# aluo-x/3D_SLN

Hardware: AMD Instinct MI355X
Metric: scene-graph VAE steps/sec + 256² diff-render fps, 1/2/4/8 MI355X (higher is better)
Workload: dtype f32; 1 GPU; BASELINE configs[1]: batch=64 scene graphs x (32 objects, 64 triples) per GPU, Sg2ScVAE train step at train.py defaults (embedding_dim=64, 5+5 GraphTripleConv, BatchNorm); O=2048, T=4096, hipgraph=True, distinct_batches_cycled=4, eps=N(0,1) drawn on the device inside the step, parallelism=dp1

## Files before the change

### 3d_sln_amd/_lib.py

```python
from __future__ import annotations

import ctypes as C
import os

HERE = os.path.dirname(os.path.abspath(__file__))
LIB_PATH = os.path.join(HERE, "libsln_hip.so")

SLN_E = {-1: "SLN_E_BADARG", -2: "SLN_E_UNSUPPORTED", -3: "SLN_E_STATE", -4: "SLN_E_NOGPU", -5: "SLN_E_NOMEM", -6: "SLN_E_CAPTURE"}

c_f32p = C.c_void_p
c_i64p = C.c_void_p


class SlnError(RuntimeError):
    pass


class SlnVaeConfig(C.Structure):
    _fields_ = [(n, C.c_int) for n in (
        "embedding_dim", "gconv_num_layers", "recurrent", "batch_norm", "decoder_cat", "use_ae",
        "box_dim", "n_angle", "num_objs", "num_preds", "num_attrs", "no_attr")]


class SlnVaeUnit(C.Structure):
# ... 143 lines not shown


class SlnDraw3D(C.Structure):
    _fields_ = [(n, C.c_void_p) for n in ("faces_xyz", "face_index", "depth", "face_label", "chosen", "K", "light_cam", "albedo")] + \
               [(n, C.c_int32) for n in ("R", "V", "F", "S", "k", "shadows")] + \
               [(n, C.c_float) for n in ("ambient", "intensity", "min_dist", "bias")] + [("background", C.c_float * 3)]


SIGNATURES = {
    "sln_version": (C.c_int, []),
    "sln_build_arch": (C.c_char_p, []),
    "sln_device_ok": (C.c_int, []),
    "sln_vae_num_units": (C.c_int, [C.POINTER(SlnVaeConfig)]),
    "sln_vae_create": (C.c_int, [C.POINTER(SlnVaeConfig), C.POINTER(C.c_void_p)]),
    "sln_vae_destroy": (None, [C.c_void_p]),
    "sln_vae_workspace_bytes": (C.c_int64, [C.c_void_p, C.c_int, C.c_int]),
    "sln_vae_bind": (C.c_int, [C.c_void_p, C.POINTER(SlnVaeTensors), C.c_void_p, C.c_int64, C.c_int, C.c_int]),
    "sln_vae_set_batch": (C.c_int, [C.c_void_p, C.POINTER(SlnVaeBatch), C.c_void_p]),
    "sln_vae_check_batch": (C.c_int, [C.c_void_p, C.c_void_p]),
    "sln_vae_encoder": (C.c_int, [C.c_void_p, c_f32p, c_f32p, C.c_int, C.c_void_p]),
    "sln_vae_decoder": (C.c_int, [C.c_void_p, c_f32p, c_f32p, c_f32p, C.c_int, C.c_void_p]),
    "sln_vae_forward": (C.c_int, [C.c_void_p, c_f32p, c_f32p, c_f32p, c_f32p, c_f32p, c_f32p, C.c_int, C.c_void_p]),
    "sln_vae_loss": (C.c_int, [C.c_void_p, c_f32p, c_f32p, c_f32p, c_f32p, C.c_float, c_f32p, C.c_int, C.c_void_p]),
    "sln_vae_decoder_backward": (C.c_int, [C.c_void_p, c_f32p, c_f32p, c_f32p, C.c_void_p]),
    "sln_vae_encoder_backward": (C.c_int, [C.c_void_p, c_f32p, c_f32p, C.c_void_p]),
    "sln_vae_backward": (C.c_int, [C.c_void_p, C.c_void_p]),
    "sln_vae_params_changed": (C.c_int, [C.c_void_p]),
    "sln_vae_zero_grad": (C.c_int, [C.c_void_p, C.c_void_p]),
    "sln_vae_adam_step": (C.c_int, [C.c_void_p, C.c_float, C.c_void_p]),
    "sln_vae_adam_reset": (C.c_int, [C.c_void_p, C.c_int64, C.c_void_p]),
    "sln_vae_adam_get_step": (C.c_int, [C.c_void_p, C.POINTER(C.c_int64), C.c_void_p]),
    "sln_vae_set_grad_guard": (C.c_int, [C.c_void_p, c_f32p]),
    "sln_vae_seed": (C.c_int, [C.c_void_p, C.c_uint64, C.c_uint64, C.c_void_p]),
    "sln_vae_last_eps": (C.c_int, [C.c_void_p, c_f32p, C.c_void_p]),
    "sln_vae_randn": (C.c_int, [C.c_void_p, c_f32p, C.c_int64, C.c_void_p]),
    "sln_layout_heatmap": (C.c_int, [c_f32p, C.c_int64, C.c_int, C.c_int, C.c_int, C.c_int, c_f32p, C.c_void_p]),
    "sln_vae_set_training": (C.c_int, [C.c_void_p, C.c_int]),
    "sln_vae_set_gemm_precision": (C.c_int, [C.c_void_p, C.c_int]),
    "sln_vae_train_step": (C.c_int, [C.c_void_p, c_f32p, C.c_float, C.c_float, c_f32p, C.c_int, C.c_int, C.c_void_p]),
    "sln_vae_group_create": (C.c_int, [C.POINTER(C.c_void_p), C.c_int, C.POINTER(SlnVaeGroupIO), C.POINTER(C.c_void_p)]),
    "sln_vae_group_decoder": (C.c_int, [C.c_void_p, C.c_void_p]),
    "sln_vae_group_decoder_backward": (C.c_int, [C.c_void_p, C.c_void_p]),
    "sln_vae_group_launches": (C.c_int, [C.c_void_p, C.POINTER(C.c_int), C.POINTER(C.c_int), C.POINTER(C.c_int)]),
    "sln_vae_group_transposes": (C.c_int64, [C.c_void_p]),
    "sln_vae_group_fused_params": (C.c_int, [C.c_void_p, C.POINTER(C.c_void_p), C.POINTER(C.c_int64), C.c_int]),
    "sln_vae_group_destroy": (None, [C.c_void_p]),
    "sln_debug_side_stream": (C.c_int, [C.c_void_p, C.POINTER(C.c_int), C.POINTER(C.c_int)]),
    "sln_side_stream_prepare": (C.c_int, [C.c_void_p]),
    "sln_side_stream_forget": (C.c_int, [C.c_void_p]),
    "sln_prof_enable": (C.c_int, [C.c_int]),
    "sln_set_deterministic": (C.c_int, [C.c_int]),
    "sln_get_deterministic": (C.c_int, []),
    "sln_debug_tn_plan": (C.c_int, [C.c_void_p, C.c_void_p, C.c_void_p, C.c_int, C.c_void_p, C.c_void_p, C.c_int]),
    "sln_prof_read": (C.c_int, [C.c_void_p, C.c_void_p, C.c_void_p, C.c_int]),
    "sln_vae_tap": (C.c_int64, [C.c_void_p, C.c_int, C.c_int, c_f32p, C.c_void_p]),
    "sln_gconv_workspace_bytes": (C.c_int64, [C.c_int, C.c_int, C.c_int, C.c_int, C.c_int, C.c_int]),
    "sln_gconv_forward": (C.c_int, [C.c_int, C.c_int, C.c_int, C.c_int, C.c_int, C.c_int, C.POINTER(SlnVaeUnit), c_f32p, c_f32p,
                                    C.c_void_p, C.c_int, C.c_int, C.c_int, C.c_void_p, C.c_int64, c_f32p, c_f32p, C.c_void_p]),
    "sln_gconv_net_create": (C.c_int, [C.c_int, C.c_int, C.c_int, C.c_int, C.c_int, C.c_int, C.POINTER(C.c_void_p)]),
    "sln_gconv_net_set_edges": (C.c_int, [C.c_void_p, C.c_void_p, C.c_int, C.c_int, C.c_void_p]),
    "sln_gconv_net_forward": (C.c_int, [C.c_void_p, c_f32p, c_f32p, c_f32p, c_f32p, C.c_int, C.c_void_p]),
    "sln_gconv_net_backward": (C.c_int, [C.c_void_p, c_f32p, c_f32p, c_f32p, c_f32p, C.c_void_p]),
    "sln_linear_forward": (C.c_int, [c_f32p, C.c_int, C.c_int, c_f32p, c_f32p, c_f32p, C.c_int, C.c_void_p,
                                     C.c_int, C.c_void_p]),
    "sln_linear_wgrad": (C.c_int, [c_f32p, c_f32p, C.c_int, C.c_int, C.c_int, c_f32p, c_f32p, C.c_void_p]),
    "sln_debug_gemm_nt": (C.c_int, [C.POINTER(SlnDbgGemmNT), C.c_int, C.POINTER(C.c_int), C.c_void_p]),
    "sln_debug_gemm_tn": (C.c_int, [C.POINTER(SlnDbgGemmTN), C.c_int, C.c_int, C.c_void_p]),
    "sln_debug_gemm_nt_route": (C.c_int, [C.POINTER(SlnDbgGemmNT), C.POINTER(SlnDbgNTRoute)]),
    "sln_debug_gemm_nt_half": (C.c_int, [C.POINTER(SlnDbgGemmNT), C.c_int, C.c_void_p]),
    "sln_debug_gemm_nt_half_takes": (C.c_int, [C.POINTER(SlnDbgGemmNT)]),
    "sln_debug_gemm_sizes": (C.c_int, [C.POINTER(C.c_int), C.c_int]),
    "sln_debug_vae_csr": (C.c_int, [c_i64p, C.c_int, C.c_int, C.c_int, C.POINTER(SlnDbgCsr), C.c_void_p, C.c_void_p]),
    "sln_debug_vae_edge": (C.c_int, [C.POINTER(SlnDbgEdge), C.c_int, C.c_int, C.POINTER(C.c_int), C.c_void_p]),
    "sln_debug_vae_loss": (C.c_int, [C.POINTER(SlnDbgLoss), C.c_void_p]),
    "sln_debug_vae_tables": (C.c_int, [C.c_int, C.c_void_p, C.c_int, C.c_int, C.c_float, C.c_int, C.c_int, C.c_int, C.c_void_p]),
    "sln_debug_vae_embed": (C.c_int, [C.POINTER(SlnDbgEmbed), C.c_int, C.c_int, C.POINTER(C.c_int), C.c_void_p]),
    "sln_debug_vae_opt": (C.c_int, [C.POINTER(SlnDbgOpt), C.c_void_p]),
    "sln_debug_vae_sizes": (C.c_int, [C.POINTER(C.c_int), C.c_int]),
    "sln_debug_vae_leaf_launches": (C.c_int64, [C.c_void_p]),
    "sln_debug_vae_half_launches": (C.c_int64, [C.c_void_p]),
    "sln_project_faces": (C.c_int, [c_f32p, C.c_void_p, c_f32p, c_f32p, c_f32p, C.c_int, C.c_int, C.c_int, C.c_float, C.c_float, c_f32p, C.c_void_p]),
    "sln_project_faces_backward": (C.c_int, [c_f32p, C.c_void_p, c_f32p, c_f32p, c_f32p, C.c_int, C.c_int, C.c_int, C.c_float, C.c_float, c_f32p,
                                             c_f32p, C.c_void_p]),
    "sln_raster_workspace_bytes": (C.c_int64, [C.c_int, C.c_int]),
    "sln_raster_forward": (C.c_int, [c_f32p, C.c_int, C.c_int, C.c_int, C.c_float, C.c_float, C.c_void_p, C.c_void_p,
                                     c_f32p, c_f32p, C.c_void_p]),
    "sln_raster_forward_dual": (C.c_int, [c_f32p, C.c_int, C.c_int, C.c_int, C.c_float, C.c_float, C.c_float, C.c_void_p,
                                          C.c_void_p, c_f32p, c_f32p, C.c_void_p, c_f32p, c_f32p, C.c_void_p]),
    "sln_raster_texture_sample": (C.c_int, [c_f32p, c_f32p, C.c_void_p, c_f32p, c_f32p, C.c_int, C.c_int, C.c_int, C.c_int,
                                            C.c_float, c_f32p, C.c_void_p]),
    "sln_raster_backward_depth": (C.c_int, [c_f32p, C.c_void_p, c_f32p, c_f32p, c_f32p, C.c_int, C.c_int, C.c_int, c_f32p,
                                            C.c_void_p]),
    "sln_raster_backward_rgb": (C.c_int, [c_f32p, C.c_void_p, c_f32p, c_f32p, C.c_int, C.c_int, C.c_int, C.c_int, C.c_float,
                                          c_f32p, C.c_void_p]),
    "sln_raster_texture_sample_chw": (C.c_int, [c_f32p, c_f32p, C.c_void_p, c_f32p, c_f32p, C.c_int, C.c_int, C.c_int, C.c_int, C.c_int,
                                                C.c_float, C.c_float, c_f32p, C.c_void_p]),
    "sln_raster_backward_rgb_multi": (C.c_int, [c_f32p, C.c_void_p, C.c_void_p, C.c_void_p, C.c_int, C.c_int, C.c_int, C.c_int, C.c_float,
                                                C.c_void_p, c_f32p, C.c_void_p]),
    "sln_scene_workspace_bytes": (C.c_int64, [C.c_int, C.c_int, C.c_int]),
    "sln_scene_forward": (C.c_int, [c_f32p, C.c_void_p, C.c_int, C.c_int, C.c_int, C.c_int, C.c_void_p, C.c_void_p,
                                    C.c_float, C.c_float, C.c_float, C.c_float, C.c_void_p, c_f32p, C.c_void_p]),
    "sln_scene_forward_live": (C.c_int, [c_f32p, C.c_void_p, C.c_int, C.c_int, C.c_int, C.c_int, C.c_void_p, C.c_void_p,
                                         C.c_float, C.c_float, C.c_float, C.c_float, C.c_void_p, c_f32p, C.c_void_p, C.c_void_p, C.c_void_p]),
    "sln_spade_prepare": (C.c_int, [C.c_void_p]),
    "sln_spade_release": (C.c_int, [C.c_void_p, C.c_int]),
    "sln_spade_conv": (C.c_int, [c_f32p, C.c_int, C.c_int, C.c_int, C.c_int, c_f32p, c_f32p, C.c_int, C.c_int, C.c_int, C.c_int,
                                 C.c_float, c_f32p, C.c_void_p]),
    "sln_spade_modulate": (C.c_int, [c_f32p, C.c_int, C.c_int, C.c_int, C.c_int, c_f32p, c_f32p, C.c_int, C.c_int, c_f32p, c_f32p,
                                     C.c_int, C.c_float, c_f32p, C.c_void_p]),
    "sln_layernorm_stats": (C.c_int, [c_f32p, C.c_int, C.c_int64, C.c_float, C.c_void_p, c_f32p, C.c_void_p]),
    "sln_spade_apply": (C.c_int, [c_f32p, c_f32p, C.c_int, C.c_int, C.c_int, C.c_int, C.c_int, c_f32p, C.c_int, C.c_float, c_f32p, C.c_void_p]),
    "sln_spade_apply_up": (C.c_int, [c_f32p, C.c_int, c_f32p, C.c_int, C.c_int, C.c_int, C.c_int, C.c_int, c_f32p, C.c_int, C.c_float, c_f32p,
                                     C.c_void_p]),
    "sln_resize": (C.c_int, [c_f32p, C.c_int, C.c_int, C.c_int, C.c_int, C.c_int, C.c_int, c_f32p, C.c_void_p]),
    "sln_spade_depth_concat": (C.c_int, [c_f32p, C.c_int, C.c_int, C.c_int, C.c_int, c_f32p, c_f32p, C.c_int, c_f32p, C.c_int, C.c_void_p]),
    "sln_se_scale_add": (C.c_int, [c_f32p, c_f32p, C.c_int, C.c_int, C.c_int64, c_f32p, c_f32p, c_f32p, c_f32p, C.c_void_p]),
    "sln_spade_conv_sums": (C.c_int, [c_f32p, C.c_int, C.c_int, C.c_int, C.c_int, c_f32p, c_f32p, C.c_int, C.c_int, C.c_int, C.c_int,
                                      C.c_float, c_f32p, C.c_void_p, C.c_void_p, C.c_void_p]),
    "sln_spade_modulate_up": (C.c_int, [c_f32p, C.c_int, C.c_int, C.c_int, C.c_int, c_f32p, c_f32p, C.c_int, C.c_int, c_f32p, C.c_int,
                                        c_f32p, C.c_int, C.c_float, c_f32p, C.c_void_p]),
    "sln_layernorm_finalize": (C.c_int, [C.c_void_p, C.c_int, C.c_int64, C.c_int, C.c_float, c_f32p, C.c_void_p]),
    "sln_spade_conv_f16": (C.c_int, [c_f32p, C.c_int, C.c_int, C.c_int, C.c_int, C.c_void_p, C.c_void_p, c_f32p, C.c_int, C.c_int, C.c_int,
                                     C.c_int, C.c_float, c_f32p, C.c_void_p]),
    "sln_spade_conv_sums_f16": (C.c_int, [c_f32p, C.c_int, C.c_int, C.c_int, C.c_int, C.c_void_p, C.c_void_p, c_f32p, C.c_int, C.c_int,
                                          C.c_int, C.c_int, C.c_float, c_f32p, C.c_void_p, C.c_void_p, C.c_void_p]),
    "sln_spade_modulate_f16": (C.c_int, [c_f32p, C.c_int, C.c_int, C.c_int, C.c_int, C.c_void_p, C.c_void_p, c_f32p, C.c_int, C.c_int,
                                         c_f32p, c_f32p, C.c_int, C.c_float, c_f32p, C.c_void_p]),
    "sln_spade_modulate_up_f16": (C.c_int, [c_f32p, C.c_int, C.c_int, C.c_int, C.c_int, C.c_void_p, C.c_void_p, c_f32p, C.c_int, C.c_int,
                                            c_f32p, C.c_int, c_f32p, C.c_int, C.c_float, c_f32p, C.c_void_p]),
    "sln_block_tail": (C.c_int, [c_f32p, C.c_int, c_f32p, C.c_int, C.c_int, C.c_int, C.c_int, C.c_void_p, c_f32p, c_f32p, c_f32p,
                                 C.c_int, c_f32p, C.c_void_p, C.c_int, C.c_float, c_f32p, C.c_void_p]),
    "sln_upsample2x": (C.c_int, [c_f32p, C.c_int, C.c_int, C.c_int, C.c_int, c_f32p, C.c_void_p]),
    "sln_conv_img_tanh": (C.c_int, [c_f32p, C.c_int, C.c_int, C.c_int, C.c_int, c_f32p, c_f32p, C.c_int, c_f32p, C.c_void_p]),
# ... 120 lines not shown
```

### 3d_sln_amd/csrc/gemm_bodies.h

```cpp
#pragma once
#include "sln_common.h"
#include "sln_gemm.h"
#include "sln_prof.h"

#include <cstdlib>
#include <cstring>
#include <type_traits>
namespace {


#ifndef SLN_TRACE
#define SLN_TRACE(i)
#endif
#ifndef SLN_TRACEH
#define SLN_TRACEH(i)
#endif

#ifndef SLN_NT_SCHED
#define SLN_NT_SCHED 1
#endif
#ifndef SLN_TN_SCHED
#define SLN_TN_SCHED 1
#endif
#ifndef SLN_TN_ABL
// ... 1267 lines not shown
      for (int r = 0; r < 16; ++r) dst[r * 64] = tn_acc_read(acc[1][r]);
    } else {
#pragma unroll
      for (int r = 0; r < 16; ++r) dst[r * 64] = tn_acc_read(acc[0][r]);
    }
  }
  __syncthreads();
  {
    const float* src = red + ((wave ^ 2) * 16) * 64 + lane;
    const float sc = a.sgd_step != nullptr ? -a.sgd_step[0] : 1.f;
    const int k = k0 + 32 * wc + lrow;
    float* dcol = a.dW + min(k, a.Kin - 1);
    const bool kv = k < a.Kin;
    if (wr == 0) {
#pragma unroll
      for (int r = 0; r < 16; ++r) {
        const float v = (tn_acc_read(acc[0][r]) + src[r * 64]) * sc;
        const int n = n0 + 2 * ((r & 3) + 8 * (r >> 2) + 4 * lk);
        if (kv && n < a.Nout) sln_gatomic_add(dcol + (size_t)n * a.lddw, v);
      }
    } else {
#pragma unroll
      for (int r = 0; r < 16; ++r) {
        const float v = (src[r * 64] + tn_acc_read(acc[1][r])) * sc;
        const int n = n0 + 2 * ((r & 3) + 8 * (r >> 2) + 4 * lk) + 1;
        if (kv && n < a.Nout) sln_gatomic_add(dcol + (size_t)n * a.lddw, v);
      }
    }
  }

  if (a.db != nullptr && (bx % tiles_k) == 0) {
#pragma unroll
    for (int off = TPRA; off < 64; off <<= 1) {
      dbacc.x += __shfl_xor(dbacc.x, off, 64); dbacc.y += __shfl_xor(dbacc.y, off, 64);
      dbacc.z += __shfl_xor(dbacc.z, off, 64); dbacc.w += __shfl_xor(dbacc.w, off, 64);
    }
    __syncthreads();
    float4* dbs = reinterpret_cast<float4*>(red);
    if (lane < TPRA) dbs[wave * TPRA + lane] = dbacc;
    __syncthreads();
    if (tid < TPRA) {
      const float4 p0 = dbs[tid], p1 = dbs[TPRA + tid], p2 = dbs[2 * TPRA + tid], p3 = dbs[3 * TPRA + tid];
      const int n = n0 + 4 * tid;
      const float sb = a.sgd_step != nullptr ? -a.sgd_step[0] : 1.f;
      if (n + 0 < a.Nout) sln_gatomic_add(a.db + n + 0, (((p0.x + p1.x) + p2.x) + p3.x) * sb);
      if (n + 1 < a.Nout) sln_gatomic_add(a.db + n + 1, (((p0.y + p1.y) + p2.y) + p3.y) * sb);
      if (n + 2 < a.Nout) sln_gatomic_add(a.db + n + 2, (((p0.z + p1.z) + p2.z) + p3.z) * sb);
      if (n + 3 < a.Nout) sln_gatomic_add(a.db + n + 3, (((p0.w + p1.w) + p2.w) + p3.w) * sb);
    }
  }
}


inline bool tn_gathers(const GemmTNArgs& a) {
  bool g = false;
  for (int s = 0; s < a.X.nseg; ++s) g |= a.X.seg[s].which != 0;
  return g;
}

inline bool tn_supported(const GemmTNArgs& a) {
  for (int s = 0; s < a.G.nseg; ++s) if (a.G.seg[s].which != 0) return false;
  return true;
}

inline size_t nt_smem_bytes(int K, int BM, int BN, int WM) {
  const int kpad = (K + 31) & ~31;
  return (size_t)sln_crows(kpad + 4) * 16 + (size_t)2 * (BM + BN) * (BK + 4) * 4 + (size_t)BN * 16 + (size_t)WM * BN * 16;
}

inline size_t tn_smem_bytes(int BM, int BN) { return (size_t)(BM + BN) * 16 + (size_t)2 * BK * (BM + TN_PAD + BN + TN_PAD) * 4; }

inline int nt_heuristic_tile(const GemmNTArgs& a) {
  static const int forced = std::getenv("SLN_NT_TILE") ? std::atoi(std::getenv("SLN_NT_TILE")) : -1;
  (void)a;
  return forced >= 0 ? forced : 0;
}

inline bool nt_big_shape(const GemmNTArgs& a) {
  return (long)sln_cdiv(a.M, 128) * sln_cdiv(a.N, 64) >= 384;
}

inline bool nt_unaligned(const GemmNTArgs& a) {
  for (int s = 0; s + 1 < a.A.nseg; ++s) if (a.A.seg[s].len % BK) return true;
  return false;
}

inline int nt_amode(const GemmNTArgs& a) {
  bool x2 = false;
  for (int s = 0; s < a.A.nseg; ++s) x2 |= a.A.seg[s].x2 != nullptr;
  bool ident = !x2;
  for (int s = 0; s < a.A.nseg; ++s) ident = ident && a.A.seg[s].coef == SLN_COEF_IDENT;
  return x2 ? 1 : (ident ? 2 : 0);
}

inline bool tn_prepare(GemmTNArgs& a) {
  bool x2 = false;
  for (int s = 0; s < a.G.nseg; ++s) x2 |= a.G.seg[s].x2 != nullptr;
  if (a.rows_per_block <= 0) {
    static const int target = std::getenv("SLN_TN_TARGET") ? std::atoi(std::getenv("SLN_TN_TARGET")) : 768;
    static const int minrows = std::getenv("SLN_TN_MINROWS") ? std::atoi(std::getenv("SLN_TN_MINROWS")) : 256;
    const int tiles = sln_cdiv(a.Nout, 64) * sln_cdiv(a.Kin, 64);
    int chunks = sln_cdiv(target, tiles);
    int rpb = sln_cdiv(sln_cdiv(a.R, chunks), BK) * BK;
    a.rows_per_block = rpb < minrows ? minrows : rpb;
  }
  return x2;
// ... 4 lines not shown
```

### 3d_sln_amd/csrc/gemm_f32.hip

```cpp
#include <cstdio>
#include <cstdlib>
#include <algorithm>
#include <vector>
#include "gemm_bodies.h"
#include "vae_multi.h"
namespace {
constexpr bool nt_coef_helpers(int amode, int epi) { return amode != 2 || epi == EPI_MASK; }
template <int BM, int BN, int AMODE, int EPI>
constexpr bool nt_helpers() { return BM == 64 && BN == 64 && nt_coef_helpers(AMODE, EPI); }
template <int BM, int BN, int WM, int WN, int AMODE, int EPI, int MULTI>
__global__ __launch_bounds__((nt_helpers<BM, BN, AMODE, EPI>() ? 512 : 256)) void gemm_nt_kernel(const GemmNTArgs a) {
  extern __shared__ __attribute__((aligned(16))) char smem[];
  gemm_nt_body<BM, BN, WM, WN, AMODE, EPI, MULTI, nt_helpers<BM, BN, AMODE, EPI>()>(a, blockIdx.x, ((a.M + BM - 1) / BM) * ((a.N + BN - 1) / BN), smem);
}

template <int AMODE, int EPI>
constexpr bool nt_helpers2() { return nt_coef_helpers(AMODE, EPI); }
template <int J, int AMODE, int EPI>
__global__ __launch_bounds__((nt_helpers2<AMODE, EPI>() ? 512 : 256)) void gemm_nt16_kernel(const GemmNTArgs a) {
  extern __shared__ __attribute__((aligned(16))) char smem[];
  gemm_nt_body16<J, AMODE, EPI, nt_helpers2<AMODE, EPI>()>(a, blockIdx.x, ((a.M + 63) / 64) * ((a.N + 32 * J - 1) / (32 * J)), smem);
}

template <int AMODE, int EPI, int NSEG = 1>
// ... 67 lines not shown
  SLN_CHECK_LAUNCH();
  return 0;
}

template <int AMODE, int EPI>
int launch_nt_route(const GemmNTArgs& a, const NtRoute& rt, hipStream_t st) {
  switch (rt.body) {
    case NT_BODY_SMALL: return launch_nt_small<AMODE, EPI>(a, rt, st);
    case NT_BODY_SMALL3: return launch_nt_small<AMODE, EPI, 3>(a, rt, st);
    case NT_BODY_16J3: return launch_nt16<3, AMODE, EPI>(a, rt, st);
    case NT_BODY_16J5: return launch_nt16<5, AMODE, EPI>(a, rt, st);
    case NT_BODY_128x64: return launch_nt<128, 64, 2, 2, AMODE, EPI>(a, rt, st);
    case NT_BODY_128: return launch_nt<128, 128, 2, 2, AMODE, EPI>(a, rt, st);
    case NT_BODY_64: return launch_nt<64, 64, 2, 2, AMODE, EPI>(a, rt, st);
    default: return -1;
  }
}

NtRoute nt_route(const GemmNTArgs& a, int epi, int tile) {
  static const bool no_small = std::getenv("SLN_NO_SMALL_NT") != nullptr;
  NtRoute r;
  r.amode = nt_amode(a); r.multi = 0;
  if (tile < 0 && !no_small && nt_wants_small(a)) r.body = NT_BODY_SMALL;
  else if (tile < 0 && !no_small && nt_wants_small3(a)) { r.body = NT_BODY_SMALL3; r.multi = 1; }
  else {
    const int J16 = tile < 0 ? nt16_pick(a) : 0;
    if (J16 == 3) r.body = NT_BODY_16J3;
    else if (J16 == 5) r.body = NT_BODY_16J5;
    else {
      if (tile < 0) tile = nt_heuristic_tile(a);
      const bool unaligned = a.A.nseg > 1 && nt_unaligned(a);
      if (unaligned) tile = 0;
      r.body = tile == 1 ? NT_BODY_128x64 : (tile == 2 ? NT_BODY_128 : NT_BODY_64);
      r.multi = a.A.nseg > 1 ? (unaligned ? 2 : 1) : 0;
    }
  }
  const bool big = r.body == NT_BODY_128x64 || r.body == NT_BODY_128;
  r.threads = !big && nt_coef_helpers(r.amode, epi) ? 512 : 256;
  return r;
}

template <int BM, int BN, int WM, int WN, bool G_X2, bool XG>
__global__ __launch_bounds__(256) void gemm_tn_kernel(const GemmTNArgs a) {
  extern __shared__ __attribute__((aligned(16))) char smem[];
  gemm_tn_body<BM, BN, WM, WN, G_X2, XG>(a, blockIdx.x, blockIdx.y, smem);
}

template <bool G_X2, bool XG>
__global__ __launch_bounds__(256) void gemm_tn_multi_kernel(const GemmTNArgs* __restrict__ probs, const TnMultiMeta* __restrict__ meta) {
  extern __shared__ __attribute__((aligned(16))) char smem[];
  const TnMultiItem it = meta->item[blockIdx.x];
  if (it.prob < 0) return;
  gemm_tn_body<64, 64, 2, 2, G_X2, XG>(probs[it.prob], it.tile, it.chunk, smem);
}

template <int BM, int BN, int WM, int WN, bool G_X2>
int launch_tn(const GemmTNArgs& a, hipStream_t st) {
  const size_t smem = tn_smem_bytes(BM, BN);
  const int gx = sln_cdiv(a.Nout, BM) * sln_cdiv(a.Kin, BN);
  const int gy = sln_cdiv(a.R, a.rows_per_block);
  if (gx <= 0 || gy <= 0) return 0;
  if (!tn_supported(a)) return -1;
  if (tn_gathers(a)) hipLaunchKernelGGL((gemm_tn_kernel<BM, BN, WM, WN, G_X2, true>), dim3(gx, gy), dim3(256), smem, st, a);
  else hipLaunchKernelGGL((gemm_tn_kernel<BM, BN, WM, WN, G_X2, false>), dim3(gx, gy), dim3(256), smem, st, a);
  SLN_CHECK_LAUNCH();
  return 0;
}

}

template <int BM, int BN, int WM, int WN>
static int init_nt_tile() {
  hipError_t e = hipSuccess;
#define SLN_SET(X2, EPI)                                                                                          \
  if (e == hipSuccess)                                                                                            \
    e = hipFuncSetAttribute(reinterpret_cast<const void*>(&gemm_nt_kernel<BM, BN, WM, WN, X2, EPI, 0>),           \
                            hipFuncAttributeMaxDynamicSharedMemorySize, 160 * 1024);                              \
  if (e == hipSuccess)                                                                                            \
    e = hipFuncSetAttribute(reinterpret_cast<const void*>(&gemm_nt_kernel<BM, BN, WM, WN, X2, EPI, 1>),           \
                            hipFuncAttributeMaxDynamicSharedMemorySize, 160 * 1024);                              \
  if (e == hipSuccess && BM == 64 && BN == 64)                                                                    \
    e = hipFuncSetAttribute(reinterpret_cast<const void*>(&gemm_nt_kernel<64, 64, WM, WN, X2, EPI, 2>),           \
                            hipFuncAttributeMaxDynamicSharedMemorySize, 160 * 1024);
  SLN_SET(0, EPI_PLAIN) SLN_SET(0, EPI_STATS) SLN_SET(0, EPI_MASK)
  SLN_SET(1, EPI_PLAIN) SLN_SET(1, EPI_STATS) SLN_SET(1, EPI_MASK)
  SLN_SET(2, EPI_PLAIN) SLN_SET(2, EPI_STATS) SLN_SET(2, EPI_MASK)
#undef SLN_SET
  return (int)e;
}

int sln_gemm_group_init();
int sln_gemm_init() {
  static bool done = false;
  if (done) return 0;
  int r = init_nt_tile<64, 64, 2, 2>();
#define SLN_SET_S(AM, EPI)                                                                                        \
  if (!r) r = (int)hipFuncSetAttribute(reinterpret_cast<const void*>(&gemm_nt_small_kernel<AM, EPI, 1>),         \
                                       hipFuncAttributeMaxDynamicSharedMemorySize, 160 * 1024);                  \
  if (!r) r = (int)hipFuncSetAttribute(reinterpret_cast<const void*>(&gemm_nt_small_kernel<AM, EPI, 3>),         \
                                       hipFuncAttributeMaxDynamicSharedMemorySize, 160 * 1024);
  SLN_SET_S(0, EPI_PLAIN) SLN_SET_S(0, EPI_STATS) SLN_SET_S(0, EPI_MASK) SLN_SET_S(1, EPI_PLAIN) SLN_SET_S(1, EPI_STATS)
  SLN_SET_S(1, EPI_MASK) SLN_SET_S(2, EPI_PLAIN) SLN_SET_S(2, EPI_STATS) SLN_SET_S(2, EPI_MASK)
#undef SLN_SET_S
#define SLN_SET_16(J, AM, EPI)                                                                                    \
  if (!r) r = (int)hipFuncSetAttribute(reinterpret_cast<const void*>(&gemm_nt16_kernel<J, AM, EPI>),             \
                                       hipFuncAttributeMaxDynamicSharedMemorySize, 160 * 1024);
#define SLN_SET_16J(J)                                                                                            \
  SLN_SET_16(J, 0, EPI_PLAIN) SLN_SET_16(J, 0, EPI_STATS) SLN_SET_16(J, 0, EPI_MASK) SLN_SET_16(J, 1, EPI_PLAIN) SLN_SET_16(J, 1, EPI_STATS) \
  SLN_SET_16(J, 1, EPI_MASK) SLN_SET_16(J, 2, EPI_PLAIN) SLN_SET_16(J, 2, EPI_STATS) SLN_SET_16(J, 2, EPI_MASK)
  SLN_SET_16J(3) SLN_SET_16J(5)
#undef SLN_SET_16J
#undef SLN_SET_16
  if (!r) r = init_nt_tile<128, 64, 2, 2>();
  if (!r) r = init_nt_tile<128, 128, 2, 2>();
#define SLN_SET_TN(X2, XG)                                                                                        \
  if (!r) r = (int)hipFuncSetAttribute(reinterpret_cast<const void*>(&gemm_tn_kernel<64, 64, 2, 2, X2, XG>),     \
                                       hipFuncAttributeMaxDynamicSharedMemorySize, 160 * 1024);
  SLN_SET_TN(true, true) SLN_SET_TN(true, false) SLN_SET_TN(false, true) SLN_SET_TN(false, false)
#undef SLN_SET_TN
#define SLN_SET_TNM(X2, XG)                                                                                       \
  if (!r) r = (int)hipFuncSetAttribute(reinterpret_cast<const void*>(&gemm_tn_multi_kernel<X2, XG>),             \
                                       hipFuncAttributeMaxDynamicSharedMemorySize, 160 * 1024);
  SLN_SET_TNM(true, true) SLN_SET_TNM(true, false) SLN_SET_TNM(false, true) SLN_SET_TNM(false, false)
#undef SLN_SET_TNM
  if (!r) r = sln_gemm_group_init();
  done = r == 0;
  return r;
}




int sln_launch_gemm_nt(const GemmNTArgs& a, int epi, int tile, hipStream_t st) {
  SlnProfScope prof(SLN_FAM_GEMM_NT, 2.0 * a.M * a.N * a.K, st);
  const NtRoute rt = nt_route(a, epi, tile);
  static const bool nt_log = std::getenv("SLN_NT_LOG") != nullptr;
  if (nt_log) std::fprintf(stderr, "NTLOG M=%d N=%d K=%d amode=%d epi=%d nseg=%d\n", a.M, a.N, a.K, rt.amode, epi, a.A.nseg);
#define SLN_DISPATCH(AM)                                                              \
  if (rt.amode == AM) {                                                               \
    if (epi == EPI_MASK) return launch_nt_route<AM, EPI_MASK>(a, rt, st);             \
    if (epi == EPI_STATS) return launch_nt_route<AM, EPI_STATS>(a, rt, st);           \
    return launch_nt_route<AM, EPI_PLAIN>(a, rt, st);                                 \
  }
  SLN_DISPATCH(0) SLN_DISPATCH(1) SLN_DISPATCH(2)
#undef SLN_DISPATCH
  return -1;
}

int sln_plan_nt_small(const GemmNTArgs& a, int epi, int* tiles) {
  static const bool no_small = std::getenv("SLN_NO_SMALL_NT") != nullptr;
  if (no_small || a.M <= 0 || a.N <= 0) return -1;
  int nseg = 0;
  const int amode = nt_amode(a);
  if (amode == 1 || epi == EPI_STATS) return -1;
  if (nt_wants_small(a)) nseg = 1;
  else if (nt_wants_small3(a)) nseg = 3;
  if (nseg) { *tiles = sln_cdiv(a.M, 32) * sln_cdiv(a.N, 32); return amode * 16 + epi * 4 + nseg; }
  if (nt_big_shape(a)) return -1;
  *tiles = sln_cdiv(a.M, 64) * sln_cdiv(a.N, 64);
  return 1000 + amode * 16 + epi * 4 + (a.A.nseg > 1 ? (nt_unaligned(a) ? 2 : 1) : 0);
}

template <int AMODE, int EPI, int NSEG>
static int launch_nt_small_multi(const GemmNTArgs* tab, const int* tiles, int R, int max_tiles, size_t smem, hipStream_t st) {
  static bool raised = false;
  if (smem > 48 * 1024 && !raised) {
    hipError_t e = hipFuncSetAttribute(reinterpret_cast<const void*>(&gemm_nt_small_multi_kernel<AMODE, EPI, NSEG>),
                                       hipFuncAttributeMaxDynamicSharedMemorySize, 160 * 1024);
    if (e != hipSuccess) return (int)e;
    raised = true;
  }
  hipLaunchKernelGGL((gemm_nt_small_multi_kernel<AMODE, EPI, NSEG>), dim3(max_tiles, R), dim3(nt_helpers2<AMODE, EPI>() ? 512 : 256), smem, st, tab, tiles);
  SLN_CHECK_LAUNCH();
  return 0;
}

template <int AMODE, int EPI, int MULTI>
static int launch_nt64_multi(const GemmNTArgs* tab, const int* tiles, int R, int max_tiles, size_t smem, hipStream_t st) {
  static bool raised = false;
  if (smem > 48 * 1024 && !raised) {
    hipError_t e = hipFuncSetAttribute(reinterpret_cast<const void*>(&gemm_nt64_multi_kernel<AMODE, EPI, MULTI>),
                                       hipFuncAttributeMaxDynamicSharedMemorySize, 160 * 1024);
    if (e != hipSuccess) return (int)e;
    raised = true;
  }
  hipLaunchKernelGGL((gemm_nt64_multi_kernel<AMODE, EPI, MULTI>), dim3(max_tiles, R), dim3(nt_helpers<64, 64, AMODE, EPI>() ? 512 : 256), smem, st, tab, tiles);
  SLN_CHECK_LAUNCH();
  return 0;
}

int sln_launch_gemm_nt_small_multi(const GemmNTArgs* tab, const int* tiles_dev, int R, int key, int max_tiles, int max_K, double flops,
                                   hipStream_t st) {
  if (R <= 0 || max_tiles <= 0) return 0;
  SlnProfScope prof(SLN_FAM_GEMM_NT, flops, st);
  if (key >= 1000) {
    const size_t smem64 = nt_smem_bytes(max_K, 64, 64, 2);
    const int am = (key - 1000) / 16, ep = ((key - 1000) / 4) % 4, mu = (key - 1000) % 4;
#define SLN_NT64M(AM, EP, MU) if (am == AM && ep == EP && mu == MU) return launch_nt64_multi<AM, EP, MU>(tab, tiles_dev, R, max_tiles, smem64, st);
    SLN_NT64M(0, EPI_PLAIN, 0) SLN_NT64M(0, EPI_PLAIN, 1) SLN_NT64M(0, EPI_PLAIN, 2) SLN_NT64M(0, EPI_MASK, 0) SLN_NT64M(0, EPI_MASK, 1) SLN_NT64M(0, EPI_MASK, 2)
    SLN_NT64M(2, EPI_PLAIN, 0) SLN_NT64M(2, EPI_PLAIN, 1) SLN_NT64M(2, EPI_PLAIN, 2) SLN_NT64M(2, EPI_MASK, 0) SLN_NT64M(2, EPI_MASK, 1) SLN_NT64M(2, EPI_MASK, 2)
#undef SLN_NT64M
    return -1;
  }
  const size_t smem = nt_small_smem_bytes(max_K);
  const int amode = key / 16, epi = (key / 4) % 4, nseg = key % 4;
#define SLN_NTM(AM, EP, NS) if (amode == AM && epi == EP && nseg == NS) return launch_nt_small_multi<AM, EP, NS>(tab, tiles_dev, R, max_tiles, smem, st);
  SLN_NTM(0, EPI_PLAIN, 1) SLN_NTM(0, EPI_PLAIN, 3) SLN_NTM(0, EPI_MASK, 1) SLN_NTM(0, EPI_MASK, 3)
  SLN_NTM(2, EPI_PLAIN, 1) SLN_NTM(2, EPI_PLAIN, 3) SLN_NTM(2, EPI_MASK, 1) SLN_NTM(2, EPI_MASK, 3)
#undef SLN_NTM
  return -1;
}

int sln_launch_gemm_tn(const GemmTNArgs& a0, hipStream_t st) {
  SlnProfScope prof(SLN_FAM_GEMM_TN, 2.0 * a0.R * a0.Nout * a0.Kin, st);
  GemmTNArgs a = a0;
  const bool x2 = tn_prepare(a);
  if (x2) return launch_tn<64, 64, 2, 2, true>(a, st);
  return launch_tn<64, 64, 2, 2, false>(a, st);
}

int sln_tn_multi_plan(GemmTNArgs* probs, int n, TnMultiMeta* meta, int* blocks, bool* x2, bool* xg, double* flops) {
  if (n < 1 || n > SLN_TN_MULTI_MAX) return -1;
  static const int target0 = std::getenv("SLN_TN_MULTI_ROWS") ? std::atoi(std::getenv("SLN_TN_MULTI_ROWS")) : 768;
  static const bool no_xcd = std::getenv("SLN_TN_NO_XCD") != nullptr;
  bool any_x2 = false, any_xg = false;
  double work = 0.0;
  for (int i = 0; i < n; ++i) {
    const GemmTNArgs& a = probs[i];
    if (a.R <= 0 || a.Nout <= 0 || a.Kin <= 0 || !tn_supported(a)) return -1;
    for (int s = 0; s < a.G.nseg; ++s) any_x2 |= a.G.seg[s].x2 != nullptr;
    any_xg |= tn_gathers(a);
    work += 2.0 * a.R * a.Nout * a.Kin;
  }
  struct Group { int prob, chunk, tiles; long cost; };
  std::vector<Group> groups;
  int per_xcd[8];
  std::vector<int> owner;
  for (long target = g_sln_deterministic ? (1L << 30) : (target0 > 0 ? target0 : 1024);; target *= 2) {
    groups.clear();
    for (int i = 0; i < n; ++i) {
      GemmTNArgs& a = probs[i];
      const int chunks = sln_cdiv(a.R, (int)(target > a.R ? a.R : target));
      a.rows_per_block = sln_cdiv(sln_cdiv(a.R, chunks), BK) * BK;
      const int tiles = sln_cdiv(a.Nout, 64) * sln_cdiv(a.Kin, 64), nch = sln_cdiv(a.R, a.rows_per_block);
      for (int c = 0; c < nch; ++c) {
        const int rows = (c + 1) * a.rows_per_block <= a.R ? a.rows_per_block : a.R - c * a.rows_per_block;
        groups.push_back(Group{i, c, tiles, (long)tiles * rows});
      }
    }
    std::stable_sort(groups.begin(), groups.end(), [](const Group& x, const Group& y) { return x.cost > y.cost; });
    long load[8] = {0, 0, 0, 0, 0, 0, 0, 0};
    for (int x = 0; x < 8; ++x) per_xcd[x] = 0;
    owner.assign(groups.size(), 0);
    for (size_t g = 0; g < groups.size(); ++g) {
      int best = 0;
      if (no_xcd) best = (int)(g % 8);
      else for (int x = 1; x < 8; ++x) if (load[x] < load[best]) best = x;
      owner[g] = best; load[best] += groups[g].cost; per_xcd[best] += groups[g].tiles;
    }
    int mx = 0;
    for (int x = 0; x < 8; ++x) mx = per_xcd[x] > mx ? per_xcd[x] : mx;
    if (8 * mx <= SLN_TN_MULTI_ITEMS) break;
    if (target > (1L << 30)) return -1;
  }
  if (any_xg) {
    const int* any = nullptr;
    for (int i = 0; i < n; ++i) { if (probs[i].X.idx_a) any = probs[i].X.idx_a; else if (probs[i].X.idx_b) any = probs[i].X.idx_b; }
    for (int i = 0; i < n; ++i) if (!probs[i].X.idx_a && !probs[i].X.idx_b) probs[i].X.idx_a = any;
  }
  int mx = 0;
  for (int x = 0; x < 8; ++x) mx = per_xcd[x] > mx ? per_xcd[x] : mx;
  std::memset(meta, 0, sizeof(*meta));
  meta->nprob = n; meta->nblocks = 8 * mx;
  for (int b = 0; b < 8 * mx; ++b) meta->item[b].prob = -1;
  int fill[8] = {0, 0, 0, 0, 0, 0, 0, 0};
  for (size_t g = 0; g < groups.size(); ++g) {
    const int x = owner[g];
    for (int t = 0; t < groups[g].tiles; ++t) {
      TnMultiItem& it = meta->item[8 * (fill[x]++) + x];
      it.prob = groups[g].prob; it.tile = t; it.chunk = groups[g].chunk;
    }
  }
  *blocks = 8 * mx; *x2 = any_x2; *xg = any_xg; *flops = work;
  return 0;
}

int sln_launch_gemm_tn_multi(const GemmTNArgs* dev_probs, const TnMultiMeta* dev_meta, int blocks, bool x2, bool xg, double flops,
                             hipStream_t st) {
  if (blocks <= 0) return 0;
  SlnProfScope prof(SLN_FAM_GEMM_TN, flops, st);
  const size_t smem = tn_smem_bytes(64, 64);
  if (smem > 48 * 1024) { int r = sln_gemm_init(); if (r) return r; }
  if (x2 && xg) hipLaunchKernelGGL((gemm_tn_multi_kernel<true, true>), dim3(blocks), dim3(256), smem, st, dev_probs, dev_meta);
  else if (x2) hipLaunchKernelGGL((gemm_tn_multi_kernel<true, false>), dim3(blocks), dim3(256), smem, st, dev_probs, dev_meta);
  else if (xg) hipLaunchKernelGGL((gemm_tn_multi_kernel<false, true>), dim3(blocks), dim3(256), smem, st, dev_probs, dev_meta);
  else hipLaunchKernelGGL((gemm_tn_multi_kernel<false, false>), dim3(blocks), dim3(256), smem, st, dev_probs, dev_meta);
  SLN_CHECK_LAUNCH();
  return 0;
}

extern "C" int sln_debug_tn_plan(const int* R, const int* Nout, const int* Kin, int n, int* rows_per_block, int* items, int max_items) {
  if (!R || !Nout || !Kin || !rows_per_block || !items || n < 1 || n > SLN_TN_MULTI_MAX) return -1;
  static thread_local GemmTNArgs probs[SLN_TN_MULTI_MAX];
  static thread_local TnMultiMeta meta;
  std::memset(probs, 0, sizeof(GemmTNArgs) * (size_t)n);
  for (int i = 0; i < n; ++i) {
    probs[i].R = R[i]; probs[i].Nout = Nout[i]; probs[i].Kin = Kin[i];
    probs[i].G.nseg = 1; probs[i].X.nseg = 1; probs[i].lddw = i;
  }
  int blocks = 0; bool x2 = false, xg = false; double flops = 0.0;
  const int r = sln_tn_multi_plan(probs, n, &meta, &blocks, &x2, &xg, &flops);
  if (r) return r;
  if (blocks > max_items) return -2;
  for (int i = 0; i < n; ++i) rows_per_block[probs[i].lddw] = probs[i].rows_per_block;
  for (int b = 0; b < blocks; ++b) {
    const TnMultiItem& it = meta.item[b];
    items[3 * b] = it.prob < 0 ? -1 : probs[it.prob].lddw; items[3 * b + 1] = it.tile; items[3 * b + 2] = it.chunk;
  }
  return blocks;
}

#include "sln_debug.h"

bool sln_dbg_bn(const SlnDbgBn& d, int coef, BnView& v) {
  std::memset(&v, 0, sizeof(v));
  v.sums = d.sums; v.gsums = d.gsums; v.gamma = d.gamma; v.beta = d.beta; v.rmean = d.rmean; v.rvar = d.rvar;
  v.cstride = d.cstride; v.mode = d.mode; v.n_rows = d.n_rows; v.eps = d.eps;
  v.rn = 1.0 / (double)(d.n_rows > 0.f ? d.n_rows : 1.f);
  if (coef == SLN_COEF_IDENT || d.mode == SLN_BN_NONE) return d.mode >= SLN_BN_NONE && d.mode <= SLN_BN_EVAL;
  const bool bwd = coef == SLN_COEF_BWD;
  if (d.mode == SLN_BN_TRAIN) return d.gamma && d.sums && d.cstride > 0 && d.n_rows >= 1.f && (bwd ? d.gsums != nullptr : d.beta != nullptr);
  if (d.mode == SLN_BN_EVAL) return d.gamma && d.rvar && (bwd || (d.beta && d.rmean));
  return false;
}

namespace {

bool dbg_operand(const SlnDbgOperand& d, int rows, int cols, bool gather_ok, bool x2_ok, Operand& op) {
  std::memset(&op, 0, sizeof(op));
  if (d.nseg < 1 || d.nseg > 3 || rows <= 0) return false;
  int tot = 0;
  for (int s = 0; s < d.nseg; ++s) {
    const SlnDbgSeg& g = d.seg[s];
    Seg& o = op.seg[s];
    if (!g.x1 || g.len <= 0 || (g.len & 3)) return false;
    if ((g.ld1 & 3) || (g.c1 & 3) || g.c1 < 0 || g.ld1 < g.c1 + g.len) return false;
    if (g.coef < SLN_COEF_IDENT || g.coef > SLN_COEF_BWD || g.which < 0 || g.which > 2) return false;
    if (g.which && (!gather_ok || !(g.which == 1 ? d.idx_a : d.idx_b))) return false;
    if (g.x2) {
      if (!x2_ok || g.coef != SLN_COEF_BWD || (g.ld2 & 3) || (g.c2 & 3) || g.c2 < 0 || g.ld2 < g.c2 + g.len) return false;
    } else if (g.coef == SLN_COEF_BWD && g.bn.mode == SLN_BN_TRAIN) return false;
    if (g.coef == SLN_COEF_BWD && !x2_ok) return false;
    o.x1 = g.x1; o.x2 = g.x2; o.ld1 = g.ld1; o.ld2 = g.ld2; o.c1 = g.c1; o.c2 = g.c2; o.len = g.len; o.which = g.which; o.coef = g.coef;
    if (!sln_dbg_bn(g.bn, g.coef, o.bn)) return false;
    tot += g.len;
  }
  if (tot != cols) return false;
  op.idx_a = d.idx_a; op.idx_b = d.idx_b; op.nseg = d.nseg; op.rows = rows; op.cols = cols;
  return true;
}

bool dbg_nt(const SlnDbgGemmNT& d, GemmNTArgs& a) {
  std::memset(&a, 0, sizeof(a));
  if (d.M <= 0 || d.N <= 0 || d.K <= 0 || d.epi < EPI_PLAIN || d.epi > EPI_MASK || d.tile < -1 || d.tile > 2) return false;
  if (!dbg_operand(d.A, d.M, d.K, true, true, a.A)) return false;
  if (!d.W || !d.Y || (d.ldw & 3) || d.ldw < d.K || d.ycol0 < 0 || d.ldy < d.ycol0 + d.N) return false;
  if (d.addend && (d.addcol0 < 0 || d.ldadd < d.addcol0 + d.N)) return false;
  if ((d.epi == EPI_STATS && d.osums) || (d.epi == EPI_MASK && d.ogsums)) { if (d.ocstride < d.N) return false; }
  if (d.epi == EPI_MASK) {
    if (!d.xprev || d.xcol0 < 0 || d.ldx < d.xcol0 + d.N || !sln_dbg_bn(d.obn, SLN_COEF_FWD, a.obn)) return false;
  } else if (!sln_dbg_bn(d.obn, SLN_COEF_IDENT, a.obn)) return false;
  a.W = d.W; a.bias = d.bias; a.Y = d.Y; a.ldy = d.ldy; a.ycol0 = d.ycol0; a.M = d.M; a.N = d.N; a.K = d.K; a.ldw = d.ldw;
  a.addend = d.addend; a.ldadd = d.ldadd; a.addcol0 = d.addcol0; a.osums = d.osums; a.ocstride = d.ocstride;
  a.ldx = d.ldx; a.xcol0 = d.xcol0; a.xprev = d.xprev; a.ogsums = d.ogsums;
  return true;
}

bool dbg_tn(const SlnDbgGemmTN& d, GemmTNArgs& a) {
  std::memset(&a, 0, sizeof(a));
  if (d.R <= 0 || d.Nout <= 0 || d.Kin <= 0 || !d.dW || d.lddw < d.Kin) return false;
  if (!dbg_operand(d.G, d.R, d.Nout, false, true, a.G)) return false;
  if (!dbg_operand(d.X, d.R, d.Kin, true, false, a.X)) return false;
  a.dW = d.dW; a.db = d.db; a.lddw = d.lddw; a.R = d.R; a.Nout = d.Nout; a.Kin = d.Kin;
  a.rows_per_block = d.rows_per_block; a.sgd_step = d.sgd_step;
  return true;
}

}

extern "C" int sln_debug_gemm_sizes(int* out, int max) {
  const int sz[6] = {(int)sizeof(SlnDbgBn), (int)sizeof(SlnDbgSeg), (int)sizeof(SlnDbgOperand), (int)sizeof(SlnDbgGemmNT),
                     (int)sizeof(SlnDbgGemmTN), (int)sizeof(SlnDbgNTRoute)};
  for (int i = 0; out && i < 6 && i < max; ++i) out[i] = sz[i];
  return 6;
}

extern "C" int sln_debug_gemm_nt_route(const SlnDbgGemmNT* desc, SlnDbgNTRoute* out) {
  GemmNTArgs a;
  if (!desc || !out || !dbg_nt(*desc, a)) return SLN_E_BADARG;
  const NtRoute rt = nt_route(a, desc->epi, desc->tile);
  out->body = rt.body; out->multi = rt.multi; out->amode = rt.amode; out->threads = rt.threads;
  return 0;
}

extern "C" int sln_debug_gemm_nt(const SlnDbgGemmNT* desc, int n, int* grouped, void* stream) {
  if (!desc || n < 1 || n > 2) return SLN_E_BADARG;
  GemmNTArgs nt[2]; int epi[2] = {0, 0};
  for (int i = 0; i < n; ++i) { if (!dbg_nt(desc[i], nt[i])) return SLN_E_BADARG; epi[i] = desc[i].epi; }
  hipStream_t st = (hipStream_t)stream;
  if (grouped) *grouped = 0;
  if (n == 2) {
    const int r = sln_launch_gemm_group(nt, epi, 2, st);
    if (r != 1) { if (grouped && !r) *grouped = 1; return r; }
  }
  for (int i = 0; i < n; ++i) { const int r = sln_launch_gemm_nt(nt[i], epi[i], desc[i].tile, st); if (r) return r; }
  return 0;
}

extern "C" int sln_debug_gemm_nt_half_takes(const SlnDbgGemmNT* desc) {
  GemmNTArgs a;
  if (!desc || !dbg_nt(*desc, a)) return SLN_E_BADARG;
  return sln_nt_half_takes(a, desc->epi) ? 1 : 0;
}

extern "C" int sln_debug_gemm_nt_half(const SlnDbgGemmNT* desc, int terms, void* stream) {
  GemmNTArgs a;
  if (!desc || (terms != 1 && terms != 3) || !dbg_nt(*desc, a)) return SLN_E_BADARG;
  if (!sln_nt_half_takes(a, desc->epi)) return SLN_E_UNSUPPORTED;
  return sln_launch_gemm_nt_half(a, terms, (hipStream_t)stream);
}

extern "C" int sln_debug_gemm_tn(const SlnDbgGemmTN* desc, int n, int multi, void* stream) {
  if (!desc || n < 1 || n > SLN_TN_MULTI_MAX || (!multi && n != 1)) return SLN_E_BADARG;
  std::vector<GemmTNArgs> probs((size_t)n);
  for (int i = 0; i < n; ++i) if (!dbg_tn(desc[i], probs[(size_t)i])) return SLN_E_BADARG;
  hipStream_t st = (hipStream_t)stream;
  if (!multi) return sln_launch_gemm_tn(probs[0], st);
  if (sln_capturing(st)) return SLN_E_CAPTURE;
  std::vector<TnMultiMeta> meta(1);
  int blocks = 0; bool x2 = false, xg = false; double flops = 0.0;
  if (sln_tn_multi_plan(probs.data(), n, meta.data(), &blocks, &x2, &xg, &flops)) return SLN_E_BADARG;
  GemmTNArgs* dprobs = nullptr; TnMultiMeta* dmeta = nullptr;
  const size_t pbytes = sizeof(GemmTNArgs) * (size_t)n;
  int r = (int)hipMalloc((void**)&dprobs, pbytes);
  if (!r) r = (int)hipMalloc((void**)&dmeta, sizeof(TnMultiMeta));
  if (!r) r = (int)hipMemcpy(dprobs, probs.data(), pbytes, hipMemcpyHostToDevice);
  if (!r) r = (int)hipMemcpy(dmeta, meta.data(), sizeof(TnMultiMeta), hipMemcpyHostToDevice);
  if (!r) r = sln_launch_gemm_tn_multi(dprobs, dmeta, blocks, x2, xg, flops, st);
  const int rs = (int)hipStreamSynchronize(st);
  if (!r) r = rs;
  if (dprobs) (void)hipFree(dprobs);
  if (dmeta) (void)hipFree(dmeta);
  return r;
}
```

### 3d_sln_amd/csrc/sln_debug.h

```cpp
#pragma once
#include "sln_common.h"
#include "sln_hip.h"

bool sln_dbg_bn(const SlnDbgBn& d, int coef, BnView& v);
long sln_vae_engine_leaf_launches(const SlnVae* h);
long sln_vae_engine_half_launches(const SlnVae* h);
```

### 3d_sln_amd/csrc/sln_gemm.h

```cpp
#pragma once
#include "sln_common.h"

enum { EPI_PLAIN = 0, EPI_STATS = 1, EPI_MASK = 2 };

struct GemmNTArgs {
  Operand A;
  const float* W;
  const float* bias;
  float* Y;
  int ldy, ycol0;
  int M, N, K, ldw;
  const float* addend;
  int ldadd, addcol0;
  double* osums;
  int ocstride;
  int ldx, xcol0;
  const float* xprev;
  double* ogsums;
  BnView obn;
};

struct GemmTNArgs {
  Operand G;
  Operand X;
  float* dW;
  float* db;
  int lddw;
  int R, Nout, Kin;
  int rows_per_block;
  const float* sgd_step;
};

int sln_launch_gemm_nt(const GemmNTArgs& a, int epi, int tile, hipStream_t st);
int sln_launch_gemm_tn(const GemmTNArgs& a, hipStream_t st);
bool sln_nt_half_takes(const GemmNTArgs& a, int epi);
int sln_launch_gemm_nt_half(const GemmNTArgs& a, int terms, hipStream_t st);
int sln_launch_gemm_group(const GemmNTArgs* nt, const int* epi, int n_nt, hipStream_t st);
enum { SLN_TN_MULTI_MAX = 64, SLN_TN_MULTI_ITEMS = 4096 };
struct TnMultiItem { int prob, tile, chunk, pad_; };
struct TnMultiMeta { int nprob, nblocks; TnMultiItem item[SLN_TN_MULTI_ITEMS]; };
int sln_tn_multi_plan(GemmTNArgs* probs, int n, TnMultiMeta* meta, int* blocks, bool* x2, bool* xg, double* flops);
int sln_launch_gemm_tn_multi(const GemmTNArgs* dev_probs, const TnMultiMeta* dev_meta, int blocks, bool x2, bool xg, double flops,
                             hipStream_t st);
int sln_gemm_init();
```

### 3d_sln_amd/csrc/vae_debug.hip

```cpp
#include <cstdint>
#include <cstring>
#include <vector>
#include "sln_debug.h"
#include "vae_multi.h"

namespace {

bool dbg_csr(const SlnDbgCsr& d, GraphCsr& g) {
  std::memset(&g, 0, sizeof(g));
  if (d.T < 0 || d.O < 1 || !d.deg || !d.invdeg || !d.rowptr || !d.cursor) return false;
  if (d.T > 0 && (!d.s || !d.p || !d.o || !d.ent)) return false;
  g.s = d.s; g.p = d.p; g.o = d.o; g.deg = d.deg; g.invdeg = d.invdeg; g.rowptr = d.rowptr; g.cursor = d.cursor; g.ent = d.ent;
  g.T = d.T; g.O = d.O;
  return true;
}

bool dbg_fwd_bn(const SlnDbgBn& d, int cols, BnView& v) {
  if (!sln_dbg_bn(d, SLN_COEF_FWD, v)) return false;
  return d.mode != SLN_BN_TRAIN || d.cstride >= cols;
}

enum { E_SCATTER_FWD = 0, E_SCATTER_BWD = 1, E_GATHER_BWD = 2, E_MASK_GSTATS = 3, E_BN_RELU = 4, E_ADD2 = 5 };

bool dbg_edge_ok(const SlnDbgEdge& d, GraphCsr& g, BnView& bn) {
// ... 309 lines not shown
      if (rows < 1 || (s.rmean && (!s.sums || !s.rvar))) return SLN_E_BADARG;
    } else if (s.dgamma && (!s.gsums || !s.dbeta)) return SLN_E_BADARG;
    BnTableEntry& t = h[(size_t)i];
    std::memset(&t, 0, sizeof(t));
    t.sums = s.sums; t.gsums = s.gsums; t.cstride = s.cstride; t.C = s.C; t.rows = s.rows;
    t.rmean = s.rmean; t.rvar = s.rvar; t.nbt = s.nbt; t.dgamma = s.dgamma; t.dbeta = s.dbeta;
  }
  DevTable<BnTableEntry> tab;
  int r = tab.upload(h);
  if (!r) r = kind == 0 ? sln_launch_bn_running_update(tab.p, n, width, momentum, independent, st, rows_t, rows_o)
                        : sln_launch_bn_param_grads(tab.p, n, width, independent, st);
  return tab.finish(r, st);
}

extern "C" int sln_debug_vae_opt(SlnDbgOpt* d, void* stream) {
  if (!d || d->calls < 1 || d->calls > 8 || d->kind < 0 || d->kind > 2) return SLN_E_BADARG;
  if (d->kind == 0 && (!d->grads || !d->m || !d->v || d->step < 0)) return SLN_E_BADARG;
  if (d->kind == 2 ? (d->params && d->n < 1) : (!d->params || d->n < 1)) return SLN_E_BADARG;
  hipStream_t st = (hipStream_t)stream;
  StepPrologue pro; std::memset(&pro, 0, sizeof(pro));
  if (d->kind == 2) {
    const SlnDbgEmbed* e = d->pro;
    if (!e || !dbg_enc(*e, pro.enc) || e->T < 0 || e->zero_bytes < 0 || e->zero_bytes % 16 || (reinterpret_cast<uintptr_t>(e->zero_ptr) & 15)) return SLN_E_BADARG;
    if (e->T > 0 && (!e->idx || !e->src || !e->dst || e->n < 1 || !e->src2 || !e->dst2 || e->n2 < 1)) return SLN_E_BADARG;
    pro.eps = d->params; pro.n_eps = (long)d->n;
    pro.pidx = static_cast<const int*>(e->idx); pro.T = e->T;
    pro.pemb_ec = e->src; pro.n_ec = e->n; pro.p0e = static_cast<float*>(e->dst);
    pro.pemb_dc = e->src2; pro.n_dc = e->n2; pro.p0d = static_cast<float*>(e->dst2);
    pro.zero_ptr = e->zero_ptr; pro.zero_bytes = (long)e->zero_bytes;
  }
  if (sln_capturing(st)) return SLN_E_CAPTURE;
  std::vector<AdamScalars> h(1);
  std::memset(h.data(), 0, sizeof(AdamScalars));
  h[0].step = d->step; h[0].lr = d->lr; h[0].beta1 = d->beta1; h[0].beta2 = d->beta2; h[0].eps = d->eps;
  h[0].rng_seed = d->seed; h[0].rng_offset = d->offset;
  DevTable<AdamScalars> sc;
  int r = sc.upload(h);
  pro.scalars = sc.p;
  for (int k = 0; k < d->calls && !r; ++k)
    r = d->kind == 0   ? sln_launch_adam(d->params, d->grads, d->m, d->v, (long)d->n, sc.p, d->total_loss, st)
        : d->kind == 1 ? sln_launch_randn(d->params, (long)d->n, sc.p, st)
                       : sln_launch_step_prologue(pro, st);
  const int rs = (int)hipStreamSynchronize(st);
  if (!r) r = rs;
  if (!r) r = (int)hipMemcpy(h.data(), sc.p, sizeof(AdamScalars), hipMemcpyDeviceToHost);
  if (sc.p) (void)hipFree(sc.p);
  if (r) return r;
  d->out_step = h[0].step; d->out_offset = h[0].rng_offset; d->out_bc1 = h[0].bc1; d->out_bc2 = h[0].bc2; d->out_skip = h[0].skip;
  if (h[0].adam_done != 0 || h[0].rng_done != 0) return SLN_E_STATE;
  return 0;
}

extern "C" int64_t sln_debug_vae_leaf_launches(const SlnVae* h) { return h ? (int64_t)sln_vae_engine_leaf_launches(h) : (int64_t)SLN_E_BADARG; }
extern "C" int64_t sln_debug_vae_half_launches(const SlnVae* h) { return h ? (int64_t)sln_vae_engine_half_launches(h) : (int64_t)SLN_E_BADARG; }
```

### 3d_sln_amd/csrc/vae_engine.hip

```cpp
#include <cstddef>
#include <new>
#include <type_traits>
#include <utility>
#include <vector>
#include <cstring>
#include <cstdlib>

#include "../../include/sln_hip.h"
#include "sln_gemm.h"
#include "vae_kernels.h"
#include "vae_multi.h"
#include "sln_prof.h"

namespace {

enum { SK_DEC_ASSEMBLE = 0, SK_EMBED_GATHER, SK_NT, SK_SCATTER_FWD, SK_TN, SK_TN_FLUSH, SK_MASK_GSTATS, SK_ADD2, SK_EMBED_BWD,
       SK_SCATTER_BWD, SK_GATHER_BWD, SK_DEC_ASSEMBLE_BWD, SK_COPY2D };
struct RecStep {
  int kind = -1, epi = 0, idx64 = 0;
  GemmNTArgs nt; GemmTNArgs tn;
  MScatterFwd sf; MScatterBwd sb; MGatherBwd gb; MMaskGstats mg; MDecAssemble da; DecAssembleBwd dab; MEmbedGather eg; MEmbedBwd eb; MAdd2 a2;
};
struct Recorder { std::vector<RecStep> steps; };

// ... 23 lines not shown
  float *g1 = nullptr, *g2 = nullptr, *g3 = nullptr, *g4 = nullptr;
  int bn[4] = {-1, -1, -1, -1};
  int u0 = 0;
  int D = 0;
  int Do = 0;
  bool first = false, last = false;
  int net = 0;
};

struct Bump {
  char* base; size_t off = 0; bool dry;
  explicit Bump(void* b) : base(static_cast<char*>(b)), dry(b == nullptr) {}
  template <typename T> T* take(size_t n) {
    off = (off + 255) & ~size_t(255);
    T* p = dry ? nullptr : reinterpret_cast<T*>(base + off);
    off += n * sizeof(T);
    return p;
  }
};

}

struct SlnVae {
  SlnVaeConfig cfg;
  int E, H, L, nmod, n_obj_e, n_attr_e, n_box_e, n_angle_e, Dec, Ddc;
  std::vector<Unit> units;
  SlnVaeTensors t;
  bool bound = false;
  int maxO = 0, maxT = 0, O = 0, T = 0;
  SlnVaeBatch batch;
  bool batch_set = false;

  std::vector<Layer> layers;
  std::vector<BnInst> bns;
  int bn_head[6] = {-1, -1, -1, -1, -1, -1};
  int n_bn_enc = 0;

  GraphCsr g;
  int* attrs32 = nullptr; int* err_flag = nullptr;
  double* stats_base = nullptr; size_t stats_doubles = 0, enc_stats_doubles = 0;
  double* gstats_base = nullptr;
  char* zero_begin = nullptr; size_t zero_bytes = 0; bool bulk_zeroed = false;
  bool step_training = true;
  int64_t* st_objs = nullptr; int64_t* st_angles = nullptr; int64_t* st_attrs = nullptr; float* st_boxes = nullptr;
  BnTableEntry* bn_table_dev = nullptr;
  TransposeEntry* tr_table_dev = nullptr; int n_tr = 0, tr_max_tiles = 0;
  AdamScalars* scalars = nullptr; double* loss_acc = nullptr; float* losses = nullptr;
  float *X0e = nullptr, *P0e = nullptr, *X0d = nullptr, *P0d = nullptr;
  float *hbA1 = nullptr, *hbA2 = nullptr, *haA1 = nullptr, *haA2 = nullptr;
  float *mu = nullptr, *logvar = nullptr, *z = nullptr, *eps_buf = nullptr;
  float *bnA1 = nullptr, *anA1 = nullptr, *boxes_pred = nullptr, *logits = nullptr, *angles_pred = nullptr;
  float *dbp = nullptr, *dlogits = nullptr, *g_bn = nullptr, *g_an = nullptr, *d_bx = nullptr, *d_ax = nullptr;
  float *dM = nullptr, *dG[3] = {nullptr, nullptr, nullptr};
  float *dX0 = nullptr, *dz = nullptr, *dmu = nullptr, *dlv = nullptr;
  float *g_h2 = nullptr, *g_h1 = nullptr, *d_xb = nullptr, *d_xa = nullptr, *tmp_d = nullptr;
  float *g_h2b = nullptr, *g_h1b = nullptr, *tmp_db = nullptr;
  int dbp_ld = 8;

  bool enc_training = false, dec_training = false, have_enc = false, have_dec = false, have_loss_grads = false;
  const float* z_src = nullptr;
  bool z_from_latent = false;
  bool wt_fresh = false;
  float host_kl = 0.f, host_lr = 0.f; int64_t host_step = 0; bool host_scalars_valid = false;
  float* grad_guard = nullptr;
  bool draw_eps = false;
  unsigned long long host_seed[2] = {0, 0};

  struct TnGroup {
    GemmTNArgs probs[SLN_TN_MULTI_MAX]; TnMultiMeta meta; int n = 0, blocks = 0; bool x2 = false, xg = false; double flops = 0.0;
    bool dirty = true; GemmTNArgs* dev_probs = nullptr; TnMultiMeta* dev_meta = nullptr;
  };
  int tn_slots = 32;
  std::vector<GemmTNArgs> tn_kind_scratch;
  bool capturing = false, tn_upload_pending = false;
  int det_seen = 0;
  bool tn_per_layer = false;
  int tn_slot_next[3] = {0, 0, 0};
  std::vector<GemmTNArgs> deferred;
  TnGroup* tn_groups_store = nullptr;
  TnGroup& tn_group(int set, int slot, int k) { return tn_groups_store[((size_t)set * tn_slots + slot) * 2 + k]; }
  int upload_group(TnGroup& g) {
    hipError_t e = hipMemcpy(g.dev_probs, g.probs, sizeof(GemmTNArgs) * (size_t)g.n, hipMemcpyHostToDevice);
    if (e == hipSuccess) e = hipMemcpy(g.dev_meta, &g.meta, sizeof(TnMultiMeta), hipMemcpyHostToDevice);
    g.dirty = e != hipSuccess;
    return (int)e;
  }
  bool bn_table_live = false;
  struct TnStage { char* host = nullptr; hipEvent_t done = nullptr; };
  enum { TN_STAGE_SLOTS = 16 };
  TnStage tn_stage[TN_STAGE_SLOTS];
  int tn_stage_next = 0;
  int stage_upload(void* dev0, const void* src0, size_t n0, void* dev1, const void* src1, size_t n1, hipStream_t st) {
    hipStreamCaptureStatus cs = hipStreamCaptureStatusNone;
    if (hipStreamIsCapturing(st, &cs) != hipSuccess || cs != hipStreamCaptureStatusNone) return SLN_E_CAPTURE;
    const size_t cap0 = sizeof(GemmTNArgs) * (size_t)SLN_TN_MULTI_MAX, cap = cap0 + sizeof(TnMultiMeta);
    if (n0 > cap0 || n1 > cap - cap0) return SLN_E_BADARG;
    TnStage& sl = tn_stage[tn_stage_next];
    tn_stage_next = (tn_stage_next + 1) % TN_STAGE_SLOTS;
    hipError_t e = hipSuccess;
    if (!sl.host) {
      void* hp = nullptr;
      if (hipHostMalloc(&hp, cap, hipHostMallocDefault) != hipSuccess) return SLN_E_NOMEM;
      sl.host = static_cast<char*>(hp);
      if (hipEventCreateWithFlags(&sl.done, hipEventDisableTiming) != hipSuccess) { (void)hipHostFree(hp); sl.host = nullptr; return SLN_E_NOMEM; }
    } else {
      e = hipEventSynchronize(sl.done);
    }
    if (e == hipSuccess && n0) { std::memcpy(sl.host, src0, n0); e = hipMemcpyAsync(dev0, sl.host, n0, hipMemcpyHostToDevice, st); }
    if (e == hipSuccess && n1) { std::memcpy(sl.host + cap0, src1, n1); e = hipMemcpyAsync(dev1, sl.host + cap0, n1, hipMemcpyHostToDevice, st); }
    if (e == hipSuccess) e = hipEventRecord(sl.done, st);
    return (int)e;
  }
  int upload_group_async(TnGroup& g, hipStream_t st) {
    const int r = stage_upload(g.dev_probs, g.probs, sizeof(GemmTNArgs) * (size_t)g.n, g.dev_meta, &g.meta,
                               offsetof(TnMultiMeta, item) + sizeof(TnMultiItem) * (size_t)g.meta.nblocks, st);
    if (r == 0) g.dirty = false;
    return r;
  }
  int upload_pending_tables() {
    for (int w = 0; w < tn_slots; ++w)
      for (int k = 0; k < 2; ++k) {
        TnGroup& g = tn_group(0, w, k);
        if (g.n > 0 && g.dirty) { int r = upload_group(g); if (r) return r; }
      }
    tn_upload_pending = false;
    return 0;
  }
  hipStream_t tn_eager_stream = nullptr;
  int flush_deferred(int which, hipStream_t st) {
    if (rec) { rec_push(SK_TN_FLUSH); return 0; }
    if (deferred.empty()) return 0;
    const int set = capturing ? 0 : 1;
    if (set == 1 && tn_eager_stream != st) {
      hipStreamCaptureStatus cs = hipStreamCaptureStatusNone, cs_old = hipStreamCaptureStatusNone;
      const bool st_capt = hipStreamIsCapturing(st, &cs) != hipSuccess || cs != hipStreamCaptureStatusNone;
      if (!st_capt) {
        if (tn_eager_stream != nullptr && hipStreamIsCapturing(tn_eager_stream, &cs_old) == hipSuccess && cs_old == hipStreamCaptureStatusNone)
          (void)hipStreamSynchronize(tn_eager_stream);
        tn_eager_stream = st;
      }
    }
    static thread_local TnGroup tmp;
    std::vector<GemmTNArgs>& kind = tn_kind_scratch;
    for (int k = 0; k < 2; ++k) {
      kind.clear();
      for (const GemmTNArgs& t : deferred) {
        bool gathers = false;
        for (int s2 = 0; s2 < t.X.nseg; ++s2) gathers |= t.X.seg[s2].which != 0;
        if ((int)gathers == k) kind.push_back(t);
      }
      size_t next = 0;
      while (next < kind.size()) {
        int want = 0; long tiles = 0;
        for (size_t i = next; i < kind.size() && want < SLN_TN_MULTI_MAX; ++i) {
          const long tl = (long)sln_cdiv(kind[i].Nout, 64) * sln_cdiv(kind[i].Kin, 64);
          if (want > 0 && tiles + tl > SLN_TN_MULTI_ITEMS / 2) break;
          tiles += tl; ++want;
        }
        int r = -1;
        const bool have_slot = tn_slot_next[which] < tn_slots / 3;
        for (; have_slot && want >= 1; want /= 2) {
          tmp.n = want;
          for (int i = 0; i < want; ++i) tmp.probs[i] = kind[next + i];
          r = sln_tn_multi_plan(tmp.probs, tmp.n, &tmp.meta, &tmp.blocks, &tmp.x2, &tmp.xg, &tmp.flops);
          if (r == 0) break;
        }
        if (r != 0) {
          GemmTNArgs one = kind[next++];
          if (g_sln_deterministic) one.rows_per_block = sln_cdiv(one.R, 32) * 32;
          r = sln_launch_gemm_tn(one, st);
          if (r) { deferred.clear(); return r; }
          continue;
        }
        next += (size_t)tmp.n;
        const int slot = which * (tn_slots / 3) + tn_slot_next[which]++;
        TnGroup& g = tn_group(set, slot, k);
        if (g.n != tmp.n || std::memcmp(g.probs, tmp.probs, sizeof(GemmTNArgs) * (size_t)tmp.n) != 0 ||
            std::memcmp(&g.meta, &tmp.meta, sizeof(TnMultiMeta)) != 0) {
          std::memcpy(g.probs, tmp.probs, sizeof(GemmTNArgs) * (size_t)tmp.n);
          g.meta = tmp.meta; g.n = tmp.n; g.blocks = tmp.blocks; g.x2 = tmp.x2; g.xg = tmp.xg; g.flops = tmp.flops;
          g.dirty = true;
        }
        if (g.dirty) {
          if (capturing) tn_upload_pending = true;
          else {
            r = upload_group_async(g, st);
            if (r) { deferred.clear(); return r; }
          }
        }
        r = sln_launch_gemm_tn_multi(g.dev_probs, g.dev_meta, g.blocks, g.x2, g.xg, g.flops, st);
        if (r) { deferred.clear(); return r; }
      }
// ... 260 lines not shown
  Bump b(base);
  const size_t Om = (size_t)mo, Tm = (size_t)mt;
  g.s = b.take<int>(Tm); g.p = b.take<int>(Tm); g.o = b.take<int>(Tm);
  g.deg = b.take<int>(Om); g.invdeg = b.take<float>(Om); g.rowptr = b.take<int>(Om + 1);
  g.cursor = b.take<int>(Om); g.ent = b.take<int>(2 * Tm);
  attrs32 = b.take<int>(Om); err_flag = b.take<int>(4);
  st_objs = b.take<int64_t>(Om); st_angles = b.take<int64_t>(Om); st_attrs = b.take<int64_t>(Om); st_boxes = b.take<float>(Om * 6);
  scalars = b.take<AdamScalars>(1); losses = b.take<float>(4);
  size_t nd = 0, nd_enc = 0;
  for (size_t i = 0; i < bns.size(); ++i) { if ((int)i == n_bn_enc) nd_enc = nd; nd += 2 * (size_t)bns[i].C; }
  if ((int)bns.size() == n_bn_enc) nd_enc = nd;
  stats_doubles = nd; enc_stats_doubles = nd_enc;
  loss_acc = b.take<double>(4); stats_base = b.take<double>(nd); gstats_base = b.take<double>(nd);
  zero_begin = reinterpret_cast<char*>(loss_acc);
  zero_bytes = (size_t)(reinterpret_cast<char*>(gstats_base + nd) - zero_begin);
  size_t o = 0;
  for (auto& bi : bns) { bi.sums = stats_base ? stats_base + o : nullptr; bi.gsums = gstats_base ? gstats_base + o : nullptr; o += 2 * (size_t)bi.C; }
  bn_table_dev = b.take<BnTableEntry>(bns.size() + 1);
  tr_table_dev = b.take<TransposeEntry>(units.size() + 1);
  for (auto& u : units) { u.wt_ld = rup(u.out, 4); u.wt = b.take<float>((size_t)u.in * u.wt_ld); }
  const size_t W = 2 * (size_t)E;
  X0e = b.take<float>(Om * Dec); P0e = b.take<float>(Tm * Dec);
  X0d = b.take<float>(Om * Ddc); P0d = b.take<float>(Tm * Ddc);
  for (auto& ly : layers) {
    const size_t D = ly.Do;
    ly.A1 = b.take<float>(Tm * H); ly.A2 = b.take<float>(Tm * (2 * H + D)); ly.M = b.take<float>(Om * H);
    ly.A3 = b.take<float>(Om * H); ly.A4 = b.take<float>(Om * D);
  }
  hbA1 = b.take<float>(Om * H); hbA2 = b.take<float>(Om * W); haA1 = b.take<float>(Om * H); haA2 = b.take<float>(Om * W);
  mu = b.take<float>(Om * E); logvar = b.take<float>(Om * E); z = b.take<float>(Om * E); eps_buf = b.take<float>(Om * E);
  bnA1 = b.take<float>(Om * H); anA1 = b.take<float>(Om * H);
  boxes_pred = b.take<float>(Om * cfg.box_dim); logits = b.take<float>(Om * cfg.n_angle);
  angles_pred = b.take<float>(Om * cfg.n_angle);
  dbp_ld = rup(cfg.box_dim, 4);
  dbp = b.take<float>(Om * dbp_ld); dlogits = b.take<float>(Om * cfg.n_angle);
  g_bn = b.take<float>(Om * H); g_an = b.take<float>(Om * H);
  d_bx = b.take<float>(Om * (W + n_attr_e)); d_ax = b.take<float>(Om * W);
  const size_t Dm = (size_t)(Dec > Ddc ? Dec : Ddc);
  dM = b.take<float>(Om * H);
  for (auto& ly : layers) {
    const size_t D = ly.Do;
    ly.g4 = b.take<float>(Om * D); ly.g3 = b.take<float>(Om * H); ly.g2 = b.take<float>(Tm * (2 * H + D)); ly.g1 = b.take<float>(Tm * H);
  }
  for (int set = 0; set < 2; ++set)
    for (int w = 0; w < tn_slots; ++w)
      for (int k = 0; k < 2; ++k) {
        GemmTNArgs* dp = b.take<GemmTNArgs>(SLN_TN_MULTI_MAX);
        TnMultiMeta* dm = b.take<TnMultiMeta>(1);
        if (!b.dry && tn_groups_store) {
          TnGroup& tg = tn_group(set, w, k);
          tg.dev_probs = dp; tg.dev_meta = dm; tg.dirty = true; tg.n = 0;
        }
      }
  dG[0] = b.take<float>(Tm * 3 * Dm); dG[1] = b.take<float>(Tm * 3 * Dm);
  dG[2] = (gconv_only || !leaf_merge || no_merge || n_attr_e == 0 || !cfg.decoder_cat) ? nullptr : b.take<float>(Tm * 3 * (size_t)Ddc);
  dX0 = b.take<float>(Om * Dm); dz = b.take<float>(Om * E); dmu = b.take<float>(Om * E); dlv = b.take<float>(Om * E);
  g_h2 = b.take<float>(Om * W); g_h1 = b.take<float>(Om * H); d_xb = b.take<float>(Om * W); d_xa = b.take<float>(Om * W);
  tmp_d = b.take<float>(Om * W);
  g_h2b = b.take<float>(Om * W); g_h1b = b.take<float>(Om * H); tmp_db = b.take<float>(Om * W);
  return (b.off + 255) & ~size_t(255);
}

int SlnVae::refresh_transposes(hipStream_t st) {
  if (wt_fresh) return 0;
  RET_IF(sln_launch_transpose_table(tr_table_dev, n_tr, tr_max_tiles, st));
  wt_fresh = true;
  return 0;
}

VaeLeaf SlnVae::leaf_args() const {
  VaeLeaf v; std::memset(&v, 0, sizeof(v));
  EncAssembleBwd& eb = v.enc;
  eb.objs = batch.objs; eb.attrs = batch.attributes; eb.angles = batch.angles; eb.boxes = batch.boxes; eb.dx0 = dX0;
  eb.O = O; eb.n_obj = n_obj_e; eb.n_attr = n_attr_e; eb.n_box = n_box_e; eb.n_angle = n_angle_e; eb.box_dim = cfg.box_dim;
  eb.d_obj_emb = t.d_obj_emb_ec; eb.d_attr_emb = t.d_attr_emb_ec; eb.d_angle_emb = t.d_angle_emb;
  eb.d_wb = t.d_box_emb_w; eb.d_bb = t.d_box_emb_b;
  eb.rows_obj = cfg.num_objs; eb.rows_attr = cfg.num_attrs; eb.rows_angle = cfg.n_angle;
  v.pidx = g.p; v.pred_rows = T; v.pred_table_rows = cfg.num_preds;
  v.d_pdc = dG[2]; v.ld_pdc = 3 * Ddc; v.col0_pdc = Ddc; v.n_pdc = Ddc; v.d_pred_dc = t.d_pred_emb_dc;
  v.d_pec = dG[0]; v.ld_pec = 3 * Dec; v.col0_pec = Dec; v.n_pec = Dec; v.d_pred_ec = t.d_pred_emb_ec;
  v.attr_idx = batch.attributes; v.d_attr = d_bx; v.ld_attr = 2 * E + n_attr_e; v.col0_attr = 2 * E; v.n_attr_dc = n_attr_e;
  v.attr_table_rows = cfg.num_attrs; v.d_attr_dc = t.d_attr_emb_dc;
  int maxc = 0;
  for (auto& bi : bns) maxc = bi.C > maxc ? bi.C : maxc;
  v.bn_tab = bn_table_dev; v.bn_n = (int)bns.size(); v.bn_max_c = maxc; v.bn_independent = cfg.recurrent ? 0 : 1;
  v.bn_update = step_training ? 1 : 0; v.bn_momentum = kBnMomentum;
  return v;
}

int SlnVae::run_bn_updates(int first, int count, hipStream_t st) {
  if (count <= 0) return 0;
  int maxc = 0;
  for (int i = first; i < first + count; ++i) maxc = bns[i].C > maxc ? bns[i].C : maxc;
  return sln_launch_bn_running_update(bn_table_dev + first, count, maxc, kBnMomentum, cfg.recurrent ? 0 : 1, st, T, O);
}

int SlnVae::gconv_forward(int gi, bool training, hipStream_t st) {
  Layer& ly = layers[gi];
  const int Do = ly.Do;
  RET_IF(linear_fwd(layer_input(gi, training), ly.u0 + 0, ly.A1, H, 0, T, ly.bn[0], training, st));
  RET_IF(linear_fwd(op1(seg_act(ly.A1, H, 0, H, ly.bn[0], 0, training), T), ly.u0 + 1, ly.A2, 2 * H + Do, 0, T, ly.bn[1],
                    training, st));
  RET_IF(k_scatter_fwd(ly.A2, 2 * H + Do, H, Do, view(ly.bn[1], 0, training), g, O, ly.M, st));
  RET_IF(linear_fwd(op1(seg_ident(ly.M, H, 0, H, 0), O), ly.u0 + 2, ly.A3, H, 0, O, ly.bn[2], training, st));
  RET_IF(linear_fwd(op1(seg_act(ly.A3, H, 0, H, ly.bn[2], 0, training), O), ly.u0 + 3, ly.A4, Do, 0, O, ly.bn[3], training,
                    st));
  return 0;
}

int SlnVae::gconv_backward(int gi, const float* dP, int lddp, int dpcol0, int slot, bool tr, hipStream_t st) {
  Layer& ly = layers[gi];
  const int D = ly.D, Do = ly.Do, C2 = 2 * H + Do;
  float *g1 = ly.g1, *g2 = ly.g2, *g3 = ly.g3, *g4 = ly.g4;
  Operand G4 = op1(seg_bwd(g4, Do, ly.A4, Do, Do, ly.bn[3], tr), O);
  RET_IF(linear_wgrad(G4, op1(seg_act(ly.A3, H, 0, H, ly.bn[2], 0, tr), O), ly.u0 + 3, O));
  RET_IF(linear_dgrad(G4, ly.u0 + 3, g3, H, O, ly.A3, H, ly.bn[2], true, nullptr, 0, tr, st));
  Operand G3 = op1(seg_bwd(g3, H, ly.A3, H, H, ly.bn[2], tr), O);
  RET_IF(linear_wgrad(G3, op1(seg_ident(ly.M, H, 0, H, 0), O), ly.u0 + 2, O));
  RET_IF(linear_dgrad(G3, ly.u0 + 2, dM, H, O, nullptr, 0, -1, false, nullptr, 0, tr, st));
  BnView v2 = view(ly.bn[1], 0, tr);
  RET_IF(k_scatter_bwd(dM, dP, lddp, dpcol0, ly.A2, C2, H, Do, v2, g, T, g2,
                       v2.mode != SLN_BN_NONE ? bns[ly.bn[1]].gsums : nullptr, C2, st));
  Operand G2 = op1(seg_bwd(g2, C2, ly.A2, C2, C2, ly.bn[1], tr), T);
  RET_IF(linear_wgrad(G2, op1(seg_act(ly.A1, H, 0, H, ly.bn[0], 0, tr), T), ly.u0 + 1, T));
  RET_IF(linear_dgrad(G2, ly.u0 + 1, g1, H, T, ly.A1, H, ly.bn[0], true, nullptr, 0, tr, st));
  Operand G1 = op1(seg_bwd(g1, H, ly.A1, H, H, ly.bn[0], tr), T);
  RET_IF(linear_wgrad(G1, layer_input(gi, tr), ly.u0 + 0, T));
  RET_IF(linear_dgrad(G1, ly.u0 + 0, dG[slot], 3 * D, T, nullptr, 0, -1, false, nullptr, 0, tr, st));
  if (tn_per_layer || (g_sln_deterministic && cfg.recurrent) || rec) RET_IF(flush_deferred(ly.net == 0 ? 1 : 0, st));
  return 0;
}

int SlnVae::encoder_forward(bool training, hipStream_t st) {
  if (training && enc_stats_doubles && !bulk_zeroed) RET_IF(sln_zero_async(stats_base, enc_stats_doubles * sizeof(double), st));
  EncAssemble ea; std::memset(&ea, 0, sizeof(ea));
  ea.objs = batch.objs; ea.attrs = batch.attributes; ea.angles = batch.angles; ea.boxes = batch.boxes;
  ea.obj_emb = t.obj_emb_ec; ea.attr_emb = t.attr_emb_ec; ea.angle_emb = t.angle_emb; ea.wb = t.box_emb_w; ea.bb = t.box_emb_b;
  ea.O = O; ea.n_obj = n_obj_e; ea.n_attr = n_attr_e; ea.n_box = n_box_e; ea.n_angle = n_angle_e; ea.box_dim = cfg.box_dim;
  ea.x0 = X0e;
// ... 75 lines not shown
  a.from_logits = (it_fused_loss && ap == angles_pred) ? 1 : 0;
  RET_IF(sln_launch_loss(a, st));
  have_loss_grads = with_grads;
  return 0;
}

int SlnVae::decoder_backward(hipStream_t st) {
  const bool tr = dec_training;
  tn_slot_next[0] = 0;
  const size_t dec_doubles = stats_doubles - enc_stats_doubles;
  if (dec_doubles && !bulk_zeroed && !rec) RET_IF(sln_zero_async(gstats_base + enc_stats_doubles, dec_doubles * sizeof(double), st));
  if (!rec) RET_IF(refresh_transposes(st));
  const int last = 2 * L - 1;
  const Layer& ll = layers[last];
  const int W = Ddc, Wh = 2 * E, WA = Wh + n_attr_e;
  Operand Gb = op1(seg_ident(dbp, dbp_ld, 0, dbp_ld, 0), O); Gb.cols = dbp_ld;
  Operand Ga = op1(seg_ident(dlogits, cfg.n_angle, 0, cfg.n_angle, 0), O);
  begin_group();
  {
    Operand Gw = Gb; Gw.seg[0].len = cfg.box_dim; Gw.cols = cfg.box_dim;
    RET_IF(linear_wgrad(Gw, op1(seg_act(bnA1, H, 0, H, bn_head[4], 0, tr), O), unit_boxnet(1), O));
  }
  RET_IF(linear_dgrad(Gb, unit_boxnet(1), g_bn, H, O, bnA1, H, bn_head[4], true, nullptr, 0, tr, st));
  RET_IF(linear_wgrad(Ga, op1(seg_act(anA1, H, 0, H, bn_head[5], 0, tr), O), unit_anglenet(1), O));
  RET_IF(linear_dgrad(Ga, unit_anglenet(1), g_an, H, O, anA1, H, bn_head[5], true, nullptr, 0, tr, st));
  RET_IF(end_group(st));
  Operand G0 = op1(seg_bwd(g_bn, H, bnA1, H, H, bn_head[4], tr), O);
  const Operand XA = head_input(true, tr);
  Operand Ga0 = op1(seg_bwd(g_an, H, anA1, H, H, bn_head[5], tr), O);
  begin_group();
  RET_IF(linear_wgrad(G0, XA, unit_boxnet(0), O));
  RET_IF(linear_dgrad(G0, unit_boxnet(0), d_bx, WA, O, nullptr, 0, -1, false, nullptr, 0, tr, st));
  RET_IF(linear_wgrad(Ga0, head_input(false, tr), unit_anglenet(0), O));
  RET_IF(linear_dgrad(Ga0, unit_anglenet(0), d_ax, Wh, O, nullptr, 0, -1, false, nullptr, 0, tr, st));
  RET_IF(end_group(st));
  {
    BnView v = view(ll.bn[3], 0, tr);
    RET_IF(k_mask_gstats(d_bx, WA, d_ax, Wh, ll.A4, W, v, O, W, ll.g4, W,
                         v.mode != SLN_BN_NONE ? bns[ll.bn[3]].gsums : nullptr, W, st));
  }
  if (!cfg.decoder_cat) RET_IF(k_add2(d_bx + W, WA, d_ax + W, Wh, O, E, dz, E, st));
  if (n_attr_e > 0 && !it_leaf) RET_IF(k_embed_bwd(batch.attributes, 1, d_bx, WA, Wh, O, n_attr_e, cfg.num_attrs, t.d_attr_emb_dc, st));
  for (int l = L - 1; l >= 0; --l) {
    const int gi = L + l, slot = (it_leaf && l == 0) ? 2 : (l & 1);
    const float* dP = (l == L - 1) ? nullptr : dG[(l & 1) ^ 1];
    RET_IF(gconv_backward(gi, dP, 3 * W, W, slot, tr, st));
    if (l > 0) {
      const Layer& pv = layers[gi - 1];
      BnView v = view(pv.bn[3], 0, tr);
      RET_IF(k_gather_bwd(dG[slot], 3 * W, W, g, O, nullptr, 0, pv.A4, W, v, 1, pv.g4, W,
                          v.mode != SLN_BN_NONE ? bns[pv.bn[3]].gsums : nullptr, W, st));
    } else {
      BnView none = view(-1, 0, tr);
      RET_IF(k_gather_bwd(dG[slot], 3 * W, W, g, O, nullptr, 0, nullptr, 0, none, 0, dX0, W, nullptr, 0, st));
      if (!it_leaf) RET_IF(k_embed_bwd(g.p, 0, dG[slot], 3 * W, W, T, W, cfg.num_preds, t.d_pred_emb_dc, st));
    }
  }
  DecAssembleBwd db; std::memset(&db, 0, sizeof(db));
  db.objs = batch.objs; db.attrs = batch.attributes; db.dx0 = dX0; db.O = O; db.n_obj = n_obj_e; db.n_attr = n_attr_e; db.n_z = E;
  db.d_obj_emb = t.d_obj_emb_dc; db.d_attr_emb = t.d_attr_emb_dc; db.dz = dz; db.z_in_x0 = cfg.decoder_cat ? 1 : 0;
  db.rows_obj = cfg.num_objs; db.rows_attr = cfg.num_attrs;
  RET_IF(k_dec_assemble_bwd(db, st));
  const int nb = (int)bns.size() - n_bn_enc;
  if (nb > 0 && !it_merge_bn && !rec) {
    int maxc = 0;
    for (int i = n_bn_enc; i < (int)bns.size(); ++i) maxc = bns[i].C > maxc ? bns[i].C : maxc;
    RET_IF(sln_launch_bn_param_grads(bn_table_dev + n_bn_enc, nb, maxc, cfg.recurrent ? 0 : 1, st));
  }
  if (!it_one_flush) RET_IF(flush_deferred(0, st));
  return 0;
}

int SlnVae::encoder_backward(hipStream_t st) {
  const bool tr = enc_training;
  tn_slot_next[1] = tn_slot_next[2] = 0;
  if (enc_stats_doubles && !bulk_zeroed) RET_IF(sln_zero_async(gstats_base, enc_stats_doubles * sizeof(double), st));
  RET_IF(refresh_transposes(st));
  const int last = L - 1, W = 2 * E;
  const Layer& ll = layers[last];
  const Operand XL = layer_output(last, tr);
  float* d_x[2] = {d_xb, d_xa};
  float* hA1v[2] = {hbA1, haA1}; float* hA2v[2] = {hbA2, haA2};
  float* tmpv[2] = {tmp_d, tmp_db}; float* gh2v[2] = {g_h2, g_h2b}; float* gh1v[2] = {g_h1, g_h1b};
  const int c0v[2] = {0, n_box_e}, nv[2] = {n_box_e, n_angle_e};
  begin_group();
  for (int br = 0; br < 2; ++br) {
    const Operand Hh = op1(seg_act(hA2v[br], W, 0, W, bn_head[br * 2 + 1], 0, tr), O);
    Operand Gm = op1(seg_ident(dmu, E, c0v[br], nv[br], 0), O);
    RET_IF(linear_wgrad(Gm, Hh, br * 4 + 2, O));
    RET_IF(linear_dgrad(Gm, br * 4 + 2, tmpv[br], W, O, nullptr, 0, -1, false, nullptr, 0, tr, st));
  }
  RET_IF(end_group(st));
  begin_group();
  for (int br = 0; br < 2; ++br) {
    const int b1 = bn_head[br * 2 + 1];
    const Operand Hh = op1(seg_act(hA2v[br], W, 0, W, b1, 0, tr), O);
    Operand Gv = op1(seg_ident(dlv, E, c0v[br], nv[br], 0), O);
    RET_IF(linear_wgrad(Gv, Hh, br * 4 + 3, O));
    RET_IF(linear_dgrad(Gv, br * 4 + 3, gh2v[br], W, O, hA2v[br], W, b1, true, tmpv[br], W, tr, st));
  }
  RET_IF(end_group(st));
  begin_group();
  for (int br = 0; br < 2; ++br) {
    const int b0 = bn_head[br * 2], b1 = bn_head[br * 2 + 1];
    Operand G2 = op1(seg_bwd(gh2v[br], W, hA2v[br], W, W, b1, tr), O);
    RET_IF(linear_wgrad(G2, op1(seg_act(hA1v[br], H, 0, H, b0, 0, tr), O), br * 4 + 1, O));
    RET_IF(linear_dgrad(G2, br * 4 + 1, gh1v[br], H, O, hA1v[br], H, b0, true, nullptr, 0, tr, st));
  }
  RET_IF(end_group(st));
  begin_group();
  for (int br = 0; br < 2; ++br) {
    const int b0 = bn_head[br * 2];
    Operand G1 = op1(seg_bwd(gh1v[br], H, hA1v[br], H, H, b0, tr), O);
    RET_IF(linear_wgrad(G1, XL, br * 4 + 0, O));
    RET_IF(linear_dgrad(G1, br * 4 + 0, d_x[br], W, O, nullptr, 0, -1, false, nullptr, 0, tr, st));
  }
  RET_IF(end_group(st));
  {
    BnView v = view(ll.bn[3], 0, tr);
    RET_IF(sln_launch_mask_gstats(d_xb, W, d_xa, W, ll.A4, W, v, O, W, ll.g4, W,
                                  v.mode != SLN_BN_NONE ? bns[ll.bn[3]].gsums : nullptr, W, st));
  }
  for (int l = L - 1; l >= 0; --l) {
    const int gi = l, slot = l & 1;
    const float* dP = (l == L - 1) ? nullptr : dG[slot ^ 1];
    RET_IF(gconv_backward(gi, dP, 3 * W, W, slot, tr, st));
    if (l > 0) {
      const Layer& pv = layers[gi - 1];
      BnView v = view(pv.bn[3], 0, tr);
      RET_IF(sln_launch_gather_bwd(dG[slot], 3 * W, W, g, O, nullptr, 0, pv.A4, W, v, 1, pv.g4, W,
                                   v.mode != SLN_BN_NONE ? bns[pv.bn[3]].gsums : nullptr, W, st));
    } else {
      BnView none = view(-1, 0, tr);
      RET_IF(sln_launch_gather_bwd(dG[slot], 3 * W, W, g, O, nullptr, 0, nullptr, 0, none, 0, dX0, W, nullptr, 0, st));
      if (!it_leaf) RET_IF(sln_launch_embed_bwd_i32(g.p, dG[slot], 3 * W, W, T, W, cfg.num_preds, t.d_pred_emb_ec, st));
    }
  }
  if (it_leaf) {
    RET_IF(sln_launch_vae_leaf(leaf_args(), st));
    ++leaf_launches;
    RET_IF(flush_deferred(it_one_flush ? 2 : 1, st));
    return 0;
  }
  EncAssembleBwd eb; std::memset(&eb, 0, sizeof(eb));
  eb.objs = batch.objs; eb.attrs = batch.attributes; eb.angles = batch.angles; eb.boxes = batch.boxes; eb.dx0 = dX0;
  eb.O = O; eb.n_obj = n_obj_e; eb.n_attr = n_attr_e; eb.n_box = n_box_e; eb.n_angle = n_angle_e; eb.box_dim = cfg.box_dim;
  eb.d_obj_emb = t.d_obj_emb_ec; eb.d_attr_emb = t.d_attr_emb_ec; eb.d_angle_emb = t.d_angle_emb;
  eb.d_wb = t.d_box_emb_w; eb.d_bb = t.d_box_emb_b;
  eb.rows_obj = cfg.num_objs; eb.rows_attr = cfg.num_attrs; eb.rows_angle = cfg.n_angle;
  RET_IF(sln_launch_enc_assemble_bwd(eb, st));
  if (it_merge_bn && !bns.empty()) {
    int maxc = 0;
    for (auto& bi : bns) maxc = bi.C > maxc ? bi.C : maxc;
    RET_IF(sln_launch_bn_param_grads(bn_table_dev, (int)bns.size(), maxc, cfg.recurrent ? 0 : 1, st));
  } else if (n_bn_enc > 0) {
    int maxc = 0;
    for (int i = 0; i < n_bn_enc; ++i) maxc = bns[i].C > maxc ? bns[i].C : maxc;
    RET_IF(sln_launch_bn_param_grads(bn_table_dev, n_bn_enc, maxc, cfg.recurrent ? 0 : 1, st));
  }
  RET_IF(flush_deferred(it_one_flush ? 2 : 1, st));
  return 0;
}

int SlnVae::train_iteration(const float* eps, int mode, hipStream_t st) {
  int r = 0;
  if (mode != TRAIN_ENCODER_BWD) {
    HIP_RET(hipMemsetAsync(t.flat_grads, 0, sizeof(float) * (size_t)t.n_flat, st));
    const bool no_merge = this->no_merge;
    it_prologue = it_fused_loss = !no_merge;
    it_zero_in_prologue = it_prologue && (reinterpret_cast<uintptr_t>(zero_begin) & 15) == 0 && (zero_bytes & 15) == 0;
    if (!it_zero_in_prologue) HIP_RET(hipMemsetAsync(zero_begin, 0, zero_bytes, st));
    bulk_zeroed = true;
    it_merge_bn = !no_merge && (mode == TRAIN_BACKWARD || mode == TRAIN_FULL);
    it_one_flush = one_flush && !tn_per_layer && (mode == TRAIN_BACKWARD || mode == TRAIN_FULL);
    it_leaf = it_merge_bn && dG[2] != nullptr && T > 0 && sln_vae_leaf_fits(leaf_args()) != 0;
    it_wt_prologue = it_prologue && leaf_merge && (mode == TRAIN_BACKWARD || mode == TRAIN_FULL);
    if (!it_prologue && draw_eps) r = sln_launch_randn(eps_buf, (long)O * E, scalars, st);
    in_iteration = true;
    if (!r) r = encoder_forward(step_training, st);
    if (!r) r = decoder_forward(nullptr, eps, step_training, st);
    in_iteration = false;
    if (!r) r = loss(boxes_pred, angles_pred, mu, logvar, true, st);
    if (!r && grad_guard && mode != TRAIN_FULL)
      r = (int)hipMemcpyAsync(grad_guard, losses + 3, sizeof(float), hipMemcpyDeviceToDevice, st);
    if (!r) r = decoder_backward(st);
    if (!r) r = sln_launch_latent_bwd(mu, logvar, eps, dz, &scalars->kl_weight, O, E, cfg.use_ae, dmu, dlv, st);
  }
  if (mode != TRAIN_UPTO_DECODER) {
    bulk_zeroed = true;
    if (!r) r = encoder_backward(st);
  }
  bulk_zeroed = false;
  it_prologue = it_fused_loss = it_merge_bn = it_zero_in_prologue = it_one_flush = it_leaf = it_wt_prologue = false;
  RET_IF(r);
  if (mode == TRAIN_FULL) {
    RET_IF(sln_launch_adam(t.flat_params, t.flat_grads, t.adam_m, t.adam_v, (long)t.n_flat, scalars, losses + 3, st));
    wt_fresh = false;
  }
  return 0;
}

long sln_vae_engine_leaf_launches(const SlnVae* h) { return h->leaf_launches; }
long sln_vae_engine_half_launches(const SlnVae* h) { return h->half_launches; }

extern "C" {

int sln_version(void) { return 1; }
const char* sln_build_arch(void) { return "gfx950"; }
int sln_device_ok(void) {
  int n = 0;
  if (hipGetDeviceCount(&n) != hipSuccess || n <= 0) return SLN_E_NOGPU;
  hipDeviceProp_t p;
  int dev = 0;
  if (hipGetDevice(&dev) != hipSuccess || hipGetDeviceProperties(&p, dev) != hipSuccess) return SLN_E_NOGPU;
  return std::strncmp(p.gcnArchName, "gfx950", 6) == 0 ? 0 : SLN_E_NOGPU;
}

static int cfg_check(const SlnVaeConfig* c) {
  if (!c) return SLN_E_BADARG;
  if (c->embedding_dim <= 0 || c->embedding_dim % 16 != 0) return SLN_E_UNSUPPORTED;
  if (c->gconv_num_layers < 1) return SLN_E_UNSUPPORTED;
  if (c->box_dim != 6 && c->box_dim != 4) return SLN_E_UNSUPPORTED;
  if (c->n_angle % 4 != 0 || c->n_angle <= 0) return SLN_E_UNSUPPORTED;
  return 0;
}

int sln_vae_num_units(const SlnVaeConfig* c) {
  if (cfg_check(c) != 0) return cfg_check(c);
  const int nmod = c->recurrent ? 1 : c->gconv_num_layers;
  return 8 + 2 * nmod * 4 + 4;
}

static int read_engine_options(SlnVae* h) {
  auto is = [](const char* name, char c) { const char* v = std::getenv(name); return v && v[0] == c; };
  h->use_group = !is("SLN_NO_GROUP", '1');
  h->no_merge = is("SLN_NO_MERGE", '1');
  h->tn_per_layer = is("SLN_TN_PER_LAYER", '1');
  h->one_flush = !is("SLN_TN_ONE_FLUSH", '0');
  h->leaf_merge = !is("SLN_LEAF_MERGE", '0');
  h->tn_slots = 3 * (2 * h->L + 8 > 16 ? 2 * h->L + 8 : 16);
  h->tn_groups_store = new (std::nothrow) SlnVae::TnGroup[2 * (size_t)h->tn_slots * 2];
  return h->tn_groups_store ? 0 : SLN_E_BADARG;
}

int sln_vae_create(const SlnVaeConfig* c, SlnVae** out) {
  if (!out) return SLN_E_BADARG;
  int r = cfg_check(c);
  if (r != 0) return r;
  SlnVae* h = new (std::nothrow) SlnVae();
  if (!h) return SLN_E_BADARG;
  h->cfg = *c;
  const int E = c->embedding_dim;
  h->E = E; h->H = 4 * E; h->L = c->gconv_num_layers; h->nmod = c->recurrent ? 1 : h->L;
  h->n_obj_e = c->no_attr ? E : E * 3 / 4; h->n_attr_e = c->no_attr ? 0 : E / 4; h->n_box_e = E * 3 / 4; h->n_angle_e = E / 4;
  h->Dec = 2 * E; h->Ddc = c->decoder_cat ? 2 * E : E;
  const int H = h->H, W = 2 * E, n = sln_vae_num_units(c);
  h->units.resize(n);
  auto set = [&](int i, int out_, int in_, bool bn) { h->units[i].out = out_; h->units[i].in = in_; h->units[i].bn = bn && c->batch_norm; };
  set(0, H, W, true); set(1, W, H, true); set(2, h->n_box_e, W, false); set(3, h->n_box_e, W, false);
  set(4, H, W, true); set(5, W, H, true); set(6, h->n_angle_e, W, false); set(7, h->n_angle_e, W, false);
  for (int net = 0; net < 2; ++net)
    for (int m = 0; m < h->nmod; ++m) {
      const int u = 8 + (net * h->nmod + m) * 4, D = net == 0 ? h->Dec : h->Ddc;
      set(u + 0, H, 3 * D, true); set(u + 1, 2 * H + D, H, true); set(u + 2, H, H, true); set(u + 3, D, H, true);
    }
  set(h->unit_boxnet(0), H, W + h->n_attr_e, true); set(h->unit_boxnet(1), c->box_dim, H, false);
  set(h->unit_anglenet(0), H, W, true); set(h->unit_anglenet(1), c->n_angle, H, false);
  h->layers.resize(2 * h->L);
  for (int net = 0; net < 2; ++net) {
    for (int l = 0; l < h->L; ++l) {
      Layer& ly = h->layers[net * h->L + l];
      ly.net = net; ly.first = l == 0; ly.last = l == h->L - 1; ly.D = net == 0 ? h->Dec : h->Ddc; ly.Do = ly.D; ly.u0 = h->unit_of(net, l, 0);
      const int Cs[4] = {H, 2 * H + ly.D, H, ly.D};
      for (int k = 0; k < 4; ++k) {
        if (!h->units[ly.u0 + k].bn) continue;
        BnInst b; b.unit = ly.u0 + k; b.C = Cs[k]; b.rows = b.rows_code = k < 2 ? -1 : -2;
        ly.bn[k] = (int)h->bns.size(); h->bns.push_back(b);
      }
    }
    auto head = [&](int slot, int unit, int C) {
      if (!h->units[unit].bn) return;
      BnInst b; b.unit = unit; b.C = C; b.rows = b.rows_code = -2;
      h->bn_head[slot] = (int)h->bns.size(); h->bns.push_back(b);
    };
    if (net == 0) { head(0, 0, H); head(1, 1, W); head(2, 4, H); head(3, 5, W); h->n_bn_enc = (int)h->bns.size(); }
    else { head(4, h->unit_boxnet(0), H); head(5, h->unit_anglenet(0), H); }
  }
  if (!c->batch_norm) h->n_bn_enc = 0;
  if (read_engine_options(h) != 0) { delete h; return SLN_E_BADARG; }
  *out = h;
  return 0;
}

void sln_vae_destroy(SlnVae* h) {
  if (!h) return;
  h->drop_graphs();
  delete[] h->tn_groups_store;
  for (auto& sl : h->tn_stage) {
    if (sl.done) { (void)hipEventSynchronize(sl.done); (void)hipEventDestroy(sl.done); }
    if (sl.host) (void)hipHostFree(sl.host);
  }
  delete h;
}

int64_t sln_vae_workspace_bytes(const SlnVae* h, int max_objs, int max_triples) {
  if (!h || max_objs <= 0 || max_triples < 0) return SLN_E_BADARG;
  SlnVae tmp = *h;
  for (int i = 0; i < 4; ++i) tmp.graph_exec[i] = nullptr;
  return (int64_t)tmp.carve(nullptr, max_objs, max_triples < 1 ? 1 : max_triples);
}

int sln_vae_bind(SlnVae* h, const SlnVaeTensors* t, void* workspace, int64_t workspace_bytes, int max_objs, int max_triples) {
  if (!h || !t || !workspace || !t->units_host) return SLN_E_BADARG;
  if (max_triples < 1) max_triples = 1;
  const int64_t need = sln_vae_workspace_bytes(h, max_objs, max_triples);
  if (need < 0 || workspace_bytes < need) return SLN_E_BADARG;
  h->t = *t;
  for (size_t i = 0; i < h->units.size(); ++i) {
    h->units[i].p = t->units_host[i];
    if (!h->units[i].p.weight || !h->units[i].p.bias) return SLN_E_BADARG;
    if (h->units[i].bn && (!h->units[i].p.bn_weight || !h->units[i].p.bn_bias || !h->units[i].p.bn_running_mean ||
                           !h->units[i].p.bn_running_var)) return SLN_E_BADARG;
  }
  h->carve(workspace, max_objs, max_triples);
  h->maxO = max_objs; h->maxT = max_triples;
  std::vector<TransposeEntry> tr;
  int maxt = 0;
  for (auto& u : h->units) {
    TransposeEntry e; e.src = u.p.weight; e.dst = u.wt; e.rows = u.out; e.cols = u.in; e.dst_ld = u.wt_ld; e.pad_ = 0;
    tr.push_back(e);
    const int tiles = sln_cdiv(u.out, 32) * sln_cdiv(u.in, 32);
    maxt = tiles > maxt ? tiles : maxt;
  }
  h->n_tr = (int)tr.size(); h->tr_max_tiles = maxt;
  HIP_RET(hipMemcpy(h->tr_table_dev, tr.data(), sizeof(TransposeEntry) * tr.size(), hipMemcpyHostToDevice));
  AdamScalars sc; std::memset(&sc, 0, sizeof(sc));
  sc.step = 0; sc.lr = 1e-4f; sc.beta1 = 0.9f; sc.beta2 = 0.999f; sc.eps = 1e-8f; sc.kl_weight = 0.1f; sc.bc1 = 1.f; sc.bc2 = 1.f;
  sc.rng_seed = h->host_seed[0]; sc.rng_offset = h->host_seed[1];
  HIP_RET(hipMemcpy(h->scalars, &sc, sizeof(sc), hipMemcpyHostToDevice));
  RET_IF(sln_gemm_init());
  h->host_scalars_valid = false;
  h->bound = true; h->batch_set = false; h->wt_fresh = false; h->have_enc = h->have_dec = false; h->bn_table_live = false;
  h->drop_graphs();
  return 0;
}

static int upload_bn_table(SlnVae* h) {
  std::vector<BnTableEntry> tab(h->bns.size());
  for (size_t i = 0; i < h->bns.size(); ++i) {
    BnInst& b = h->bns[i];
// ... 903 lines not shown
```

### 3d_sln_amd/csrc/vae_kernels.h

```cpp
#pragma once
#include "sln_common.h"

struct GraphCsr {
  int* s;
  int* p;
  int* o;
  int* deg;
  float* invdeg;
  int* rowptr;
  int* cursor;
  int* ent;
  int T, O;
};
int sln_launch_graph_prep(const int64_t* triples, int T, int O, int num_preds, GraphCsr g, int* err_flag, hipStream_t st,
                          int edges_only = 0, int deg_is_zero = 0);
int sln_launch_bn_relu_apply(const float* x, int ld, int col0, int cols, int rows, BnView bn, float* out, int ldo, hipStream_t st);
struct StageBatch {
  const int64_t* objs; const int64_t* attrs; const int64_t* angles; const float* boxes;
  int64_t* st_objs; int64_t* st_attrs; int64_t* st_angles; float* st_boxes;
  int* attrs32; int* deg; int* err;
  int O, box_dim, n_objs, n_attrs, n_angle;
};
int sln_launch_stage_batch(const StageBatch& a, hipStream_t st);
int sln_launch_validate_ids(const int64_t* objs, const int64_t* attrs, const int64_t* angles, int O, int n_objs, int n_attrs,
// ... 22 lines not shown
  float* x0;
};
int sln_launch_enc_assemble(EncAssemble a, hipStream_t st);
struct EncAssembleBwd {
  const int64_t* objs; const int64_t* attrs; const int64_t* angles; const float* boxes;
  const float* dx0; int O, n_obj, n_attr, n_box, n_angle, box_dim;
  float* d_obj_emb; float* d_attr_emb; float* d_angle_emb; float* d_wb; float* d_bb;
  int rows_obj, rows_attr, rows_angle;
};
int sln_launch_enc_assemble_bwd(EncAssembleBwd a, hipStream_t st);

struct DecAssemble {
  const int64_t* objs; const int64_t* attrs;
  const float* obj_emb; const float* attr_emb; const float* mu; const float* logvar; const float* eps;
  const float* z_in;
  int O, n_obj, n_attr, n_z, use_ae;
  float* z; float* x0;
  int z_in_x0;
};
int sln_launch_dec_assemble(DecAssemble a, hipStream_t st);
struct DecAssembleBwd {
  const int64_t* objs; const int64_t* attrs; const float* dx0; int O, n_obj, n_attr, n_z;
  float* d_obj_emb; float* d_attr_emb; float* dz;
  int z_in_x0;
  int rows_obj, rows_attr;
};
int sln_launch_dec_assemble_bwd(DecAssembleBwd a, hipStream_t st);

int sln_launch_embed_gather_i32(const int* idx, const float* emb, int rows, int n, float* out, hipStream_t st);
int sln_launch_embed_bwd_i32(const int* idx, const float* d, int ld, int col0, int rows, int n, int table_rows,
                             float* d_emb, hipStream_t st);
int sln_launch_embed_bwd_i64(const int64_t* idx, const float* d, int ld, int col0, int rows, int n, int table_rows,
                             float* d_emb, hipStream_t st);

struct LossArgs {
  const float* boxes; const float* boxes_pred; int box_dim;
  const int64_t* angles; const float* logits; float* angles_pred; int n_angle;
  const float* mu; const float* logvar; int n_z; int use_ae;
  const float* kl_weight;
  int O;
  double* acc;
  float* losses;
  float* d_boxes_pred; float* d_logits;
  int ld_dbp;
  int acc_prezeroed;
  int from_logits;
};
int sln_launch_log_softmax_bwd(const float* logprob, const float* d_logprob, float* d_logits, int O, int n, hipStream_t st);
int sln_launch_i64_to_i32(const int64_t* src, int* dst, int n, hipStream_t st);
int sln_launch_log_softmax(const float* logits, float* out, int O, int n, hipStream_t st);
int sln_launch_loss(LossArgs a, hipStream_t st);
int sln_launch_latent_bwd(const float* mu, const float* logvar, const float* eps, const float* dz,
                          const float* kl_weight, int O, int n_z, int use_ae, float* dmu, float* dlogvar,
                          hipStream_t st);

struct BnTableEntry {
  const double* sums; const double* gsums; int cstride; int C; int rows;
  float* rmean; float* rvar; int64_t* nbt; float* dgamma; float* dbeta;
};
int sln_launch_bn_running_update(const BnTableEntry* table, int n, int max_c, float momentum, int independent,
                                 hipStream_t st, int rows_t = 0, int rows_o = 0);
int sln_launch_bn_param_grads(const BnTableEntry* table, int n, int max_c, int independent, hipStream_t st);

struct TransposeEntry { const float* src; float* dst; int rows; int cols; int dst_ld; int pad_; };
int sln_launch_transpose_table(const TransposeEntry* table, int n, int max_tiles, hipStream_t st);

struct AdamScalars {
  int64_t step; float lr, beta1, beta2, eps; float kl_weight; float bc1, bc2; int skip, pad_;
  unsigned long long rng_seed, rng_offset; unsigned int rng_done, adam_done;
};
int sln_launch_adam(float* params, const float* grads, float* m, float* v, long n, AdamScalars* scalars, const float* total_loss,
                    hipStream_t st);

int sln_launch_randn(float* eps, long n, AdamScalars* scalars, hipStream_t st);

struct StepPrologue {
  float* eps; long n_eps; AdamScalars* scalars;
  EncAssemble enc;
  const int* pidx; int T;
  const float* pemb_ec; int n_ec; float* p0e;
  const float* pemb_dc; int n_dc; float* p0d;
  void* zero_ptr; long zero_bytes;
  const TransposeEntry* tr_tab; int n_tr, tr_max_tiles;
};
int sln_launch_step_prologue(const StepPrologue& a, hipStream_t st);

struct VaeLeaf {
  EncAssembleBwd enc;
  const int* pidx; int pred_rows, pred_table_rows;
  const float* d_pdc; int ld_pdc, col0_pdc, n_pdc; float* d_pred_dc;
  const float* d_pec; int ld_pec, col0_pec, n_pec; float* d_pred_ec;
  const int64_t* attr_idx; const float* d_attr; int ld_attr, col0_attr, n_attr_dc, attr_table_rows; float* d_attr_dc;
  const BnTableEntry* bn_tab; int bn_n, bn_max_c, bn_independent;
  int bn_update; float bn_momentum;
};
int sln_vae_leaf_fits(const VaeLeaf& a);
int sln_launch_vae_leaf(const VaeLeaf& a, hipStream_t st);
int sln_launch_layout_heatmap(const float* boxes, long n_trials, int O, int cs, int clip, float* counts, hipStream_t st);
```

### 3d_sln_amd/csrc/vae_kernels.hip

```cpp
#include <cstring>
#include "vae_kernels.h"
#include "sln_prof.h"

namespace {

constexpr int CB = 64;
constexpr int RL = 4;
constexpr int BOX_ROWS = 64;
constexpr int RB = 32;

__device__ __forceinline__ void commit_col_stats(float s1, float s2, bool valid, double* out, int cstride, int col) {
  __shared__ float red[2][RL][CB];
  red[0][threadIdx.y][threadIdx.x] = s1;
  red[1][threadIdx.y][threadIdx.x] = s2;
  __syncthreads();
  if (threadIdx.y == 0 && valid && out != nullptr) {
    float a = 0.f, b = 0.f;
#pragma unroll
    for (int i = 0; i < RL; ++i) { a += red[0][i][threadIdx.x]; b += red[1][i][threadIdx.x]; }
    atomicAdd(out + col, sln_qd((double)a, SLN_Q_BWD));
    atomicAdd(out + cstride + col, sln_qd((double)b, SLN_Q_BWD));
  }
}

__global__ void prep_split_kernel(const int64_t* __restrict__ tri, int T, int O, int num_preds, GraphCsr g, int* err, int stride,
                                  int poff, int ooff) {
  const int t = blockIdx.x * blockDim.x + threadIdx.x;
  if (t >= T) return;
  const int64_t s = tri[stride * t], p = poff >= 0 ? tri[stride * t + poff] : 0, o = tri[stride * t + ooff];
  if (s < 0 || s >= O || o < 0 || o >= O || p < 0 || p >= num_preds) {
    if (err) atomicOr(err, 1);
    g.s[t] = 0; g.p[t] = 0; g.o[t] = 0;
    atomicAdd(g.deg, 2);
    return;
  }
  g.s[t] = (int)s; g.p[t] = (int)p; g.o[t] = (int)o;
  atomicAdd(g.deg + (int)s, 1);
  atomicAdd(g.deg + (int)o, 1);
}

__global__ __launch_bounds__(1024) void csr_scan_kernel(GraphCsr g, int O) {
  __shared__ int part[1024];
  __shared__ int carry;
  if (threadIdx.x == 0) carry = 0;
  __syncthreads();
  for (int base = 0; base < O; base += 1024) {
    const int i = base + threadIdx.x;
    const int d = i < O ? g.deg[i] : 0;
    part[threadIdx.x] = d;
    __syncthreads();
    for (int off = 1; off < 1024; off <<= 1) {
      int v = threadIdx.x >= off ? part[threadIdx.x - off] : 0;
      __syncthreads();
      part[threadIdx.x] += v;
      __syncthreads();
// ... 582 lines not shown
  } else {
    for (long i = i0; i < (long)a.O * a.n_angle; i += stride) {
      const int r = (int)(i / a.n_angle), k = (int)(i % a.n_angle);
      const int tgt = (int)a.angles[r];
      const float lp = a.angles_pred[i];
      if (k == tgt) nll -= (double)lp;
      if (a.d_logits) a.d_logits[i] = (expf(lp) - (k == tgt ? 1.f : 0.f)) * go;
    }
  }
  if (!a.use_ae) {
    float s = 0.f;
    const long nkl = (long)a.O * a.n_z;
    for (long i = i0; i < nkl; i += 4 * stride) {
      float m[4], lv[4];
#pragma unroll
      for (int u = 0; u < 4; ++u) { const long j = min(i + u * stride, nkl - 1); m[u] = a.mu[j]; lv[u] = a.logvar[j]; }
#pragma unroll
      for (int u = 0; u < 4; ++u) {
        const float term = 1.f + lv[u] - m[u] * m[u] - expf(lv[u]);
        s += (i + u * stride < nkl) ? term : 0.f;
      }
    }
    kl = s;
  }
  __shared__ double red[3][256];
  red[0][threadIdx.x] = l1; red[1][threadIdx.x] = nll; red[2][threadIdx.x] = kl;
  __syncthreads();
  for (int off = 128; off > 0; off >>= 1) {
    if (threadIdx.x < off)
      for (int k = 0; k < 3; ++k) red[k][threadIdx.x] += red[k][threadIdx.x + off];
    __syncthreads();
  }
  if (threadIdx.x < 3) atomicAdd(a.acc + threadIdx.x, sln_qd(red[threadIdx.x][0], SLN_Q_LOSS));
  __threadfence();
  __syncthreads();
  if (threadIdx.x == 0) {
    const unsigned int t = atomicAdd(reinterpret_cast<unsigned int*>(a.acc + 3), 1u);
    if (t == gridDim.x - 1) {
      __threadfence();
      const double s0 = atomicAdd(a.acc + 0, 0.0), s1 = atomicAdd(a.acc + 1, 0.0), s2 = atomicAdd(a.acc + 2, 0.0);
      const double O = (double)a.O;
      const float lb = (float)(s0 / (O * a.box_dim));
      const float la = (float)(s1 / O);
      float lk = 0.f;
      if (!a.use_ae) lk = (float)(-0.5 * s2 / O) * a.kl_weight[0];
      a.losses[0] = lb; a.losses[1] = la; a.losses[2] = lk; a.losses[3] = lb + la + lk;
    }
  }
}

__global__ void latent_bwd_kernel(const float* __restrict__ mu, const float* __restrict__ lv,
                                  const float* __restrict__ eps, const float* __restrict__ dz,
                                  const float* __restrict__ klw, int O, int nz, int use_ae, float* __restrict__ dmu,
                                  float* __restrict__ dlv) {
  const long i = (long)blockIdx.x * blockDim.x + threadIdx.x;
  if (i >= (long)O * nz) return;
  const float g = dz[i];
  if (use_ae) { dmu[i] = g; dlv[i] = 0.f; return; }
  const float w = klw[0] / (float)O;
  const float l = lv[i];
  dmu[i] = fmaf(w, mu[i], g);
  dlv[i] = w * 0.5f * (expf(l) - 1.f) + g * eps[i] * 0.5f * expf(0.5f * l);
}

__device__ __forceinline__ void bn_running_update_body(const BnTableEntry* __restrict__ tab, int n, float mom, int per_entry, int rows_t, int rows_o,
                                                       const int c, const int ey) {
  const int e0 = per_entry ? ey : 0, e1 = per_entry ? ey + 1 : n;
  for (int e = e0; e < e1; ++e) {
    const BnTableEntry t = tab[e];
    if (c == 0 && t.nbt) t.nbt[0] += 1;
    if (c >= t.C || t.rmean == nullptr) continue;
    const int rows = t.rows == -1 ? rows_t : (t.rows == -2 ? rows_o : t.rows);
    const double N = (double)rows;
    const double m = t.sums[c] / N;
    double v = t.sums[t.cstride + c] / N - m * m;
    v = v < 0.0 ? 0.0 : v;
    const double vu = rows > 1 ? v * N / (N - 1.0) : v;
    t.rmean[c] = (1.f - mom) * t.rmean[c] + mom * (float)m;
    t.rvar[c] = (1.f - mom) * t.rvar[c] + mom * (float)vu;
  }
}

__global__ void bn_running_update_kernel(const BnTableEntry* __restrict__ tab, int n, float mom, int per_entry, int rows_t, int rows_o) {
  bn_running_update_body(tab, n, mom, per_entry, rows_t, rows_o, (int)(blockIdx.x * blockDim.x + threadIdx.x), (int)blockIdx.y);
}

__device__ __forceinline__ void bn_param_grads_body(const BnTableEntry* __restrict__ tab, int n, int per_entry, const int c, const int ey) {
  const int e0 = per_entry ? ey : 0, e1 = per_entry ? ey + 1 : n;
  for (int e = e0; e < e1; ++e) {
    const BnTableEntry t = tab[e];
    if (c >= t.C || t.dgamma == nullptr) continue;
    t.dbeta[c] += (float)t.gsums[c];
    t.dgamma[c] += (float)t.gsums[t.cstride + c];
  }
}
__global__ void bn_param_grads_kernel(const BnTableEntry* __restrict__ tab, int n, int per_entry) {
  bn_param_grads_body(tab, n, per_entry, (int)(blockIdx.x * blockDim.x + threadIdx.x), (int)blockIdx.y);
}

__device__ __forceinline__ void transpose_tile_body(const TransposeEntry& t, const int tile_id, float (*tile)[33]) {
  const int tr = (t.rows + 31) / 32, tc = (t.cols + 31) / 32;
  if (tile_id >= tr * tc) return;
  const int r0 = (tile_id / tc) * 32, c0 = (tile_id % tc) * 32;
  const int tx = threadIdx.x & 31, ty = threadIdx.x >> 5;
  for (int i = ty; i < 32; i += 8) {
    const int r = r0 + i, c = c0 + tx;
    tile[i][tx] = (r < t.rows && c < t.cols) ? t.src[(size_t)r * t.cols + c] : 0.f;
  }
  __syncthreads();
  for (int i = ty; i < 32; i += 8) {
// ... 444 lines not shown
    const int rpb = embed_rows_per_block();
    hipLaunchKernelGGL(embed_bwd_lds_kernel<int64_t>, dim3(sln_cdiv(rows, rpb)), dim3(256), sizeof(float) * table_rows * n, st,
                       idx, d, ld, col0, rows, n, table_rows, rpb, d_emb);
    SLN_CHECK_LAUNCH();
    return 0;
  }
  hipLaunchKernelGGL(embed_bwd_kernel<int64_t>, dim3((unsigned)((tot + 255) / 256)), dim3(256), 0, st, idx, d, ld, col0,
                     rows, n, d_emb);
  SLN_CHECK_LAUNCH();
  return 0;
}

int sln_launch_embed_gather_i32(const int* idx, const float* emb, int rows, int n, float* out, hipStream_t st) {
  const long tot = (long)rows * n;
  if (tot <= 0) return 0;
  hipLaunchKernelGGL(embed_gather_kernel, dim3((unsigned)((tot + 255) / 256)), dim3(256), 0, st, idx, emb, rows, n, out);
  SLN_CHECK_LAUNCH();
  return 0;
}

int sln_launch_i64_to_i32(const int64_t* src, int* dst, int n, hipStream_t st) {
  if (n <= 0) return 0;
  hipLaunchKernelGGL(i64_to_i32_kernel, dim3(sln_cdiv(n, 256)), dim3(256), 0, st, src, dst, n);
  SLN_CHECK_LAUNCH();
  return 0;
}

int sln_launch_log_softmax_bwd(const float* logprob, const float* d_logprob, float* d_logits, int O, int n,
                               hipStream_t st) {
  if (O <= 0) return 0;
  hipLaunchKernelGGL(log_softmax_bwd_kernel, dim3(sln_cdiv(O, 128)), dim3(128), 0, st, logprob, d_logprob, d_logits, O, n);
  SLN_CHECK_LAUNCH();
  return 0;
}

int sln_launch_log_softmax(const float* logits, float* out, int O, int n, hipStream_t st) {
  if (O <= 0) return 0;
  hipLaunchKernelGGL(log_softmax_kernel, dim3(sln_cdiv(O, 128)), dim3(128), 0, st, logits, out, O, n);
  SLN_CHECK_LAUNCH();
  return 0;
}

int sln_launch_loss(LossArgs a, hipStream_t st) {
  if (!a.acc_prezeroed) {
    const int e = sln_zero_async(a.acc, sizeof(double) * 4, st);
    if (e != 0) return e;
  }
  hipLaunchKernelGGL(loss_kernel, dim3(LOSS_BLOCKS), dim3(256), 0, st, a);
  SLN_CHECK_LAUNCH();
  return 0;
}

int sln_launch_latent_bwd(const float* mu, const float* logvar, const float* eps, const float* dz, const float* kl_weight,
                          int O, int n_z, int use_ae, float* dmu, float* dlogvar, hipStream_t st) {
  const long n = (long)O * n_z;
  if (n <= 0) return 0;
  hipLaunchKernelGGL(latent_bwd_kernel, dim3((unsigned)((n + 255) / 256)), dim3(256), 0, st, mu, logvar, eps, dz,
                     kl_weight, O, n_z, use_ae, dmu, dlogvar);
  SLN_CHECK_LAUNCH();
  return 0;
}

int sln_launch_bn_running_update(const BnTableEntry* table, int n, int max_c, float momentum, int independent,
                                 hipStream_t st, int rows_t, int rows_o) {
  if (n <= 0) return 0;
  hipLaunchKernelGGL(bn_running_update_kernel, dim3(sln_cdiv(max_c, 256), independent ? n : 1), dim3(256), 0, st, table, n,
                     momentum, independent, rows_t, rows_o);
  SLN_CHECK_LAUNCH();
  return 0;
}

int sln_launch_bn_param_grads(const BnTableEntry* table, int n, int max_c, int independent, hipStream_t st) {
  if (n <= 0) return 0;
  hipLaunchKernelGGL(bn_param_grads_kernel, dim3(sln_cdiv(max_c, 256), independent ? n : 1), dim3(256), 0, st, table, n,
                     independent);
  SLN_CHECK_LAUNCH();
  return 0;
}

int sln_launch_transpose_table(const TransposeEntry* table, int n, int max_tiles, hipStream_t st) {
  if (n <= 0 || max_tiles <= 0) return 0;
  hipLaunchKernelGGL(transpose_table_kernel, dim3(max_tiles, n), dim3(256), 0, st, table);
  SLN_CHECK_LAUNCH();
  return 0;
}

int sln_launch_adam(float* params, const float* grads, float* m, float* v, long n, AdamScalars* scalars, const float* total_loss,
                    hipStream_t st) {
  SlnProfScope prof(SLN_FAM_OTHER, 28.0 * n, st);
  long blocks = (n + 4095) / 4096;
  if (blocks > 256) blocks = 256;
  if (blocks < 1) blocks = 1;
  const int vec = ((reinterpret_cast<uintptr_t>(params) | reinterpret_cast<uintptr_t>(grads) | reinterpret_cast<uintptr_t>(m) | reinterpret_cast<uintptr_t>(v)) & 15) == 0;
  hipLaunchKernelGGL(adam_kernel, dim3((unsigned)blocks), dim3(1024), 0, st, params, grads, m, v, n, vec, scalars, total_loss);
  SLN_CHECK_LAUNCH();
  return 0;
}

int sln_launch_randn(float* eps, long n, AdamScalars* scalars, hipStream_t st) {
  if (n <= 0) return 0;
  const long q = (n + 3) / 4;
  hipLaunchKernelGGL(randn_kernel, dim3((unsigned)((q + 255) / 256)), dim3(256), 0, st, eps, n, scalars);
  SLN_CHECK_LAUNCH();
  return 0;
}

int sln_launch_step_prologue(const StepPrologue& a, hipStream_t st) {
  auto blocks = [](long n) { return (unsigned int)((n + 255) / 256); };
  const unsigned int nr = a.eps ? blocks((a.n_eps + 3) / 4) : 0;
  const unsigned int ne = blocks((long)a.enc.O * (a.enc.n_obj + a.enc.n_attr + a.enc.n_box + a.enc.n_angle));
  const unsigned int n1 = blocks((long)a.T * a.n_ec), n2 = blocks((long)a.T * a.n_dc);
  const unsigned int nz = a.zero_ptr ? blocks(a.zero_bytes / 16) : 0;
  const unsigned int nt = (a.tr_tab && a.n_tr > 0 && a.tr_max_tiles > 0) ? (unsigned int)a.n_tr * (unsigned int)a.tr_max_tiles : 0;
  const unsigned int tot = nr + ne + n1 + n2 + nz + nt;
  if (tot == 0) return 0;
  hipLaunchKernelGGL(step_prologue_kernel, dim3(tot), dim3(256), 0, st, a, nr, nr + ne, nr + ne + n1, nr + ne + n1 + n2, nr + ne + n1 + n2 + nz);
  SLN_CHECK_LAUNCH();
  return 0;
}

struct LeafEmbedJob { const void* idx; const float* d; float* d_emb; int ld, col0, rows, n, table_rows, rpb; };
struct LeafArgs {
  AssembleBwdLds asmb;
  EncAssembleBwd box; int box_gx;
  LeafEmbedJob pdc, pec, attr;
  const BnTableEntry* bn_tab; int bn_n, bn_per_entry, bn_gx, rows_t, rows_o; float mom;
};
__global__ __launch_bounds__(256) void vae_leaf_kernel(unsigned int b0, unsigned int b1, unsigned int b2, unsigned int b3, unsigned int b4,
                                                       unsigned int b5, LeafArgs a) {
  extern __shared__ float tab[];
  const unsigned int b = blockIdx.x;
  if (b < b0) assemble_bwd_lds_body(a.asmb, (int)b);
  else if (b < b1) {
    const int q = (int)(b - b0);
    box_embed_bwd_body(a.box, (int)BOX_ROWS, q % a.box_gx, q / a.box_gx, (int)(threadIdx.x % CB), (int)(threadIdx.x / CB),
                       reinterpret_cast<float (*)[RL][CB]>(tab));
  } else if (b < b2)
    embed_bwd_lds_body<int>(static_cast<const int*>(a.pdc.idx), a.pdc.d, a.pdc.ld, a.pdc.col0, a.pdc.rows, a.pdc.n, a.pdc.table_rows, a.pdc.rpb,
                            a.pdc.d_emb, (int)(b - b1));
  else if (b < b3)
    embed_bwd_lds_body<int>(static_cast<const int*>(a.pec.idx), a.pec.d, a.pec.ld, a.pec.col0, a.pec.rows, a.pec.n, a.pec.table_rows, a.pec.rpb,
                            a.pec.d_emb, (int)(b - b2));
  else if (b < b4)
    embed_bwd_lds_body<int64_t>(static_cast<const int64_t*>(a.attr.idx), a.attr.d, a.attr.ld, a.attr.col0, a.attr.rows, a.attr.n,
                                a.attr.table_rows, a.attr.rpb, a.attr.d_emb, (int)(b - b3));
  else if (b < b5) {
    const int q = (int)(b - b4);
    bn_param_grads_body(a.bn_tab, a.bn_n, a.bn_per_entry, (q % a.bn_gx) * 256 + (int)threadIdx.x, q / a.bn_gx);
  } else {
    const int q = (int)(b - b5);
    bn_running_update_body(a.bn_tab, a.bn_n, a.mom, a.bn_per_entry, a.rows_t, a.rows_o, (q % a.bn_gx) * 256 + (int)threadIdx.x, q / a.bn_gx);
  }
}

int sln_vae_leaf_fits(const VaeLeaf& a) {
  if (g_sln_deterministic) return 0;
  const EncAssembleBwd& e = a.enc;
  if (e.O <= 0 || a.pred_rows <= 0) return 0;
  if (!(e.rows_obj > 0 && e.rows_angle > 0 && (e.n_attr == 0 || e.rows_attr > 0))) return 0;
  if ((long)e.rows_obj * e.n_obj + (long)e.rows_attr * e.n_attr + (long)e.rows_angle * e.n_angle > ASSEMBLE_LDS_MAX_FLOATS) return 0;
  if (a.pred_table_rows <= 0 || (long)a.pred_table_rows * a.n_pdc > EMBED_LDS_MAX_FLOATS || (long)a.pred_table_rows * a.n_pec > EMBED_LDS_MAX_FLOATS)
    return 0;
  if (a.n_attr_dc > 0 && (a.attr_table_rows <= 0 || (long)a.attr_table_rows * a.n_attr_dc > EMBED_LDS_MAX_FLOATS)) return 0;
  if (a.n_pdc <= 0 || a.n_pec <= 0 || e.n_box <= 0) return 0;
  return 1;
}

int sln_launch_vae_leaf(const VaeLeaf& v, hipStream_t st) {
  if (!sln_vae_leaf_fits(v)) return -1;
  LeafArgs a; std::memset(&a, 0, sizeof(a));
  const EncAssembleBwd& e = v.enc;
  AssembleBwdLds& l = a.asmb;
  l.dx0 = e.dx0; l.ld = e.n_obj + e.n_attr + e.n_box + e.n_angle; l.O = e.O;
  int k = 0;
  l.seg[k++] = EmbSeg{e.objs, e.d_obj_emb, e.n_obj, e.rows_obj, 0, 0};
  if (e.n_attr > 0) l.seg[k++] = EmbSeg{e.attrs, e.d_attr_emb, e.n_attr, e.rows_attr, e.n_obj, 0};
  l.seg[k++] = EmbSeg{e.angles, e.d_angle_emb, e.n_angle, e.rows_angle, e.n_obj + e.n_attr + e.n_box, 0};
  l.nseg = k;
  int off = 0;
  for (int s = 0; s < l.nseg; ++s) { l.seg[s].lds0 = off; off += l.seg[s].rows * l.seg[s].n; }
  l.lds_floats = off;
  l.rows_per_block = l.O <= 8192 ? 16 : 64;
  a.box = e; a.box_gx = sln_cdiv(e.n_box, CB);
  const int rpb = embed_rows_per_block();
  a.pdc = LeafEmbedJob{v.pidx, v.d_pdc, v.d_pred_dc, v.ld_pdc, v.col0_pdc, v.pred_rows, v.n_pdc, v.pred_table_rows, rpb};
  a.pec = LeafEmbedJob{v.pidx, v.d_pec, v.d_pred_ec, v.ld_pec, v.col0_pec, v.pred_rows, v.n_pec, v.pred_table_rows, rpb};
  if (v.n_attr_dc > 0) a.attr = LeafEmbedJob{v.attr_idx, v.d_attr, v.d_attr_dc, v.ld_attr, v.col0_attr, e.O, v.n_attr_dc, v.attr_table_rows, rpb};
  a.bn_tab = v.bn_tab; a.bn_n = v.bn_n; a.bn_per_entry = v.bn_independent ? 1 : 0; a.bn_gx = sln_cdiv(v.bn_max_c > 0 ? v.bn_max_c : 1, 256);
  a.rows_t = v.pred_rows; a.rows_o = e.O; a.mom = v.bn_momentum;
  const unsigned int n_bn = v.bn_n > 0 ? (unsigned int)a.bn_gx * (unsigned int)(a.bn_per_entry ? v.bn_n : 1) : 0;
  const unsigned int n_asm = (unsigned int)sln_cdiv(l.O, l.rows_per_block);
  const unsigned int n_box = (unsigned int)a.box_gx * (unsigned int)sln_cdiv(e.O, BOX_ROWS);
  const unsigned int n_pred = (unsigned int)sln_cdiv(v.pred_rows, rpb);
  const unsigned int n_attr = v.n_attr_dc > 0 ? (unsigned int)sln_cdiv(e.O, rpb) : 0;
  const unsigned int b0 = n_asm, b1 = b0 + n_box, b2 = b1 + n_pred, b3 = b2 + n_pred, b4 = b3 + n_attr, b5 = b4 + n_bn;
  const unsigned int tot = b5 + (v.bn_update ? n_bn : 0);
  size_t lds = sizeof(float) * 7 * RL * CB;
  auto grow = [&lds](long floats) { if (sizeof(float) * (size_t)floats > lds) lds = sizeof(float) * (size_t)floats; };
  grow(l.lds_floats); grow((long)v.pred_table_rows * v.n_pdc); grow((long)v.pred_table_rows * v.n_pec);
  if (v.n_attr_dc > 0) grow((long)v.attr_table_rows * v.n_attr_dc);
  hipLaunchKernelGGL(vae_leaf_kernel, dim3(tot), dim3(256), lds, st, b0, b1, b2, b3, b4, b5, a);
  SLN_CHECK_LAUNCH();
  return 0;
}

int sln_launch_add2(const float* a, int lda, const float* b, int ldb, int rows, int cols, float* out, int ldo, hipStream_t st) {
  const long n = (long)rows * cols;
  if (n <= 0) return 0;
  hipLaunchKernelGGL(add2_kernel, dim3((unsigned)((n + 255) / 256)), dim3(256), 0, st, a, lda, b, ldb, rows, cols, out, ldo);
  SLN_CHECK_LAUNCH();
  return 0;
}

#include "vae_multi.h"
namespace {

template <int XT, int YT>
__global__ __launch_bounds__(XT* YT) void scatter_avg_fwd_multi_kernel(const MScatterFwd* __restrict__ tab) {
  const MScatterFwd& a = tab[blockIdx.z];
  if ((int)blockIdx.x >= a.gx || (int)blockIdx.y >= a.gy) return;
  scatter_avg_fwd_v4_body<XT, YT>(a.A2, a.ld, a.H, a.D, a.bn, a.g, a.O, a.g.T, a.pooled);
}
template <int XT, int YT, int RPT, int NIT>
__global__ __launch_bounds__(XT* YT) void scatter_avg_bwd_multi_kernel(const MScatterBwd* __restrict__ tab) {
  const MScatterBwd& a = tab[blockIdx.z];
  if ((int)blockIdx.x >= a.gx || (int)blockIdx.y >= a.gy) return;
  scatter_avg_bwd_v4_body<XT, YT, RPT, NIT>(a.dM, a.dP, a.lddp, a.dpcol0, a.A2, a.ld, a.H, a.D, a.bn, a.g, a.T, a.g2, a.gsums, a.cstride);
}
template <int XT, int YT>
__global__ __launch_bounds__(XT* YT) void gather_bwd_multi_kernel(const MGatherBwd* __restrict__ tab) {
  const MGatherBwd& a = tab[blockIdx.z];
  if ((int)blockIdx.x >= a.gx || (int)blockIdx.y >= a.gy) return;
  gather_bwd_v4_body<XT, YT>(a.dG, a.ldg, a.D, a.g, a.O, a.g.T, a.add1, a.ldadd1, a.xprev, a.ldx, a.bn, a.masked, a.out, a.ldo, a.gsums, a.cstride);
}
__global__ __launch_bounds__(CB* RL) void mask_gstats_multi_kernel(const MMaskGstats* __restrict__ tab) {
  const MMaskGstats& a = tab[blockIdx.z];
  if ((int)blockIdx.x >= a.gx || (int)blockIdx.y >= a.gy) return;
  mask_gstats_body(a.d1, a.ld1, a.d2, a.ld2, a.xprev, a.ldx, a.bn, a.rows, a.cols, a.out, a.ldo, a.gsums, a.cstride);
}
__global__ void dec_assemble_multi_kernel(const MDecAssemble* __restrict__ tab) {
  const MDecAssemble& a = tab[blockIdx.z];
  if ((int)blockIdx.x >= a.gx) return;
  dec_assemble_body(a.a);
}
__global__ void dec_assemble_bwd_multi_kernel(const MDecAssembleBwd* __restrict__ tab) {
  const MDecAssembleBwd& a = tab[blockIdx.z];
  if ((int)blockIdx.x >= a.gx) return;
  dec_assemble_bwd_body(a.a);
}
struct MAsmLds { AssembleBwdLds a; int gx, pad_; };
static_assert(sizeof(MAsmLds) <= SLN_ASM_BLOB && sizeof(MDecAssembleBwd) <= SLN_ASM_BLOB, "SLN_ASM_BLOB too small");
__global__ __launch_bounds__(256) void assemble_bwd_lds_multi_kernel(const char* __restrict__ tab) {
  const MAsmLds& a = *reinterpret_cast<const MAsmLds*>(tab + (size_t)blockIdx.z * SLN_ASM_BLOB);
  if ((int)blockIdx.x >= a.gx) return;
// ... 231 lines not shown
```

### include/sln_hip.h

```cpp
#ifndef SLN_HIP_H
#define SLN_HIP_H

#include <stdint.h>

#ifdef __cplusplus
extern "C" {
#endif

#define SLN_E_BADARG (-1)
#define SLN_E_UNSUPPORTED (-2)
#define SLN_E_STATE (-3)
#define SLN_E_NOGPU (-4)
#define SLN_E_NOMEM (-5)
#define SLN_E_CAPTURE (-6)

int sln_version(void);
const char* sln_build_arch(void);
int sln_device_ok(void);


typedef struct SlnVaeConfig {
  int embedding_dim;
  int gconv_num_layers;
  int recurrent;
// ... 59 lines not shown
int sln_vae_loss(SlnVae* h, const float* boxes_pred, const float* angles_pred, const float* mu,
                 const float* logvar, float kl_weight, float* losses_out, int with_grads, void* stream);

int sln_vae_decoder_backward(SlnVae* h, const float* d_boxes_pred, const float* d_angles_pred, float* dz, void* stream);
int sln_vae_encoder_backward(SlnVae* h, const float* d_mu, const float* d_logvar, void* stream);
int sln_vae_backward(SlnVae* h, void* stream);

int sln_vae_params_changed(SlnVae* h);
int sln_vae_zero_grad(SlnVae* h, void* stream);
int sln_vae_adam_step(SlnVae* h, float lr, void* stream);
int sln_vae_adam_reset(SlnVae* h, int64_t step, void* stream);
int sln_vae_adam_get_step(SlnVae* h, int64_t* step_out, void* stream);
int sln_vae_set_grad_guard(SlnVae* h, float* slot);
int sln_vae_seed(SlnVae* h, uint64_t seed, uint64_t offset, void* stream);
int sln_vae_last_eps(SlnVae* h, float* eps_out, void* stream);
int sln_vae_randn(SlnVae* h, float* out, int64_t n, void* stream);
int sln_layout_heatmap(const float* boxes_pred, int64_t n_trials, int O, int box_dim, int container_size, int clip_coor, float* counts,
                       void* stream);

enum { SLN_TRAIN_BACKWARD = 0, SLN_TRAIN_FULL = 1, SLN_TRAIN_UPTO_DECODER = 2, SLN_TRAIN_ENCODER_BWD = 3 };
int sln_vae_set_training(SlnVae* h, int training);
int sln_vae_set_gemm_precision(SlnVae* h, int mode);
int sln_vae_train_step(SlnVae* h, const float* eps, float kl_weight, float lr, float* losses_out, int use_graph,
                       int with_adam, void* stream);

typedef struct SlnVaeGroup SlnVaeGroup;
typedef struct SlnVaeGroupIO {
  int rows_total;
  const int* row0_host;
  const float* z;
  float* boxes_pred;
  float* angles_pred;
  float* d_boxes_pred;
  float* d_angles_pred;
  float* dz;
  const float* sgd_step;
} SlnVaeGroupIO;
int sln_vae_group_create(SlnVae* const* engines, int R, const SlnVaeGroupIO* io, SlnVaeGroup** out);
int sln_vae_group_decoder(SlnVaeGroup* g, void* stream);
int sln_vae_group_decoder_backward(SlnVaeGroup* g, void* stream);
int sln_vae_group_fused_params(const SlnVaeGroup* g, const float** params, int64_t* numel, int max);
int sln_vae_group_launches(const SlnVaeGroup* g, int* fwd, int* bwd, int* single_room_fallbacks);
int64_t sln_vae_group_transposes(const SlnVaeGroup* g);
void sln_vae_group_destroy(SlnVaeGroup* g);

int sln_debug_side_stream(void* stream, int* index, int* overlapped);
int sln_side_stream_prepare(void* stream);
int sln_side_stream_forget(void* stream);

int sln_prof_enable(int enable);
int sln_set_deterministic(int on);
int sln_get_deterministic(void);
int sln_debug_tn_plan(const int* R, const int* Nout, const int* Kin, int n, int* rows_per_block, int* items, int max_items);
int sln_prof_read(double* ms_by_family, double* work_by_family, int64_t* launches_by_family, int n_families);

int64_t sln_vae_tap(SlnVae* h, int layer, int what, float* dst, void* stream);

int64_t sln_gconv_workspace_bytes(int D, int H, int Dout, int O, int T, int num_layers);
int sln_gconv_forward(int D, int H, int Dout, int num_layers, int n_modules, int batch_norm, const SlnVaeUnit* units_host,
                      const float* obj_vecs, const float* pred_vecs, const int64_t* edges, int O, int T, int training, void* workspace,
                      int64_t workspace_bytes, float* new_obj, float* new_pred, void* stream);

int sln_gconv_net_create(int D, int H, int Dout, int num_layers, int recurrent, int batch_norm, SlnVae** out);
int sln_gconv_net_set_edges(SlnVae* h, const int64_t* edges, int O, int T, void* stream);
int sln_gconv_net_forward(SlnVae* h, const float* obj_vecs, const float* pred_vecs, float* new_obj, float* new_pred, int training,
                          void* stream);
int sln_gconv_net_backward(SlnVae* h, const float* d_new_obj, const float* d_new_pred, float* d_obj_vecs, float* d_pred_vecs,
                           void* stream);

int sln_linear_forward(const float* x, int M, int K, const float* W, const float* bias, float* y, int N, double* sums,
                       int tile, void* stream);
int sln_linear_wgrad(const float* g, const float* x, int R, int N, int K, float* dW, float* db, void* stream);

typedef struct SlnDbgBn {
  const double* sums;
  const double* gsums;
  const float* gamma;
  const float* beta;
  const float* rmean;
  const float* rvar;
  int cstride;
  int mode;
  float n_rows;
  float eps;
} SlnDbgBn;
typedef struct SlnDbgSeg {
  const float* x1;
  const float* x2;
  int ld1, ld2, c1, c2, len, which, coef, pad_;
  SlnDbgBn bn;
} SlnDbgSeg;
typedef struct SlnDbgOperand {
  SlnDbgSeg seg[3];
  const int* idx_a;
  const int* idx_b;
  int nseg, pad_;
} SlnDbgOperand;
typedef struct SlnDbgGemmNT {
  SlnDbgOperand A;
  const float* W;
  const float* bias;
  float* Y;
  const float* addend;
  const float* xprev;
  double* osums;
  double* ogsums;
  SlnDbgBn obn;
  int M, N, K, ldw, ldy, ycol0, ldadd, addcol0, ocstride, ldx, xcol0, epi, tile, pad_;
} SlnDbgGemmNT;
typedef struct SlnDbgGemmTN {
  SlnDbgOperand G, X;
  float* dW;
  float* db;
  const float* sgd_step;
  int lddw, R, Nout, Kin, rows_per_block, pad_;
} SlnDbgGemmTN;
typedef struct SlnDbgNTRoute { int body, multi, amode, threads; } SlnDbgNTRoute;
int sln_debug_gemm_nt(const SlnDbgGemmNT* desc, int n, int* grouped, void* stream);
int sln_debug_gemm_tn(const SlnDbgGemmTN* desc, int n, int multi, void* stream);
int sln_debug_gemm_nt_route(const SlnDbgGemmNT* desc, SlnDbgNTRoute* out);
int sln_debug_gemm_nt_half(const SlnDbgGemmNT* desc, int terms, void* stream);
int sln_debug_gemm_nt_half_takes(const SlnDbgGemmNT* desc);
int sln_debug_gemm_sizes(int* out, int max);

typedef struct SlnDbgCsr {
  int* s; int* p; int* o; int* deg; float* invdeg; int* rowptr; int* cursor; int* ent;
  int T, O;
} SlnDbgCsr;
int sln_debug_vae_csr(const int64_t* triples, int num_preds, int edges_only, int deg_is_zero, const SlnDbgCsr* g, int* err, void* stream);
typedef struct SlnDbgEdge {
  SlnDbgCsr g;
  SlnDbgBn bn;
  const float* a; const float* b; const float* c;
  float* out;
  double* gsums;
  int kind, lda, ldb, ldc, ldo, H, D, rows, cols, col0, cstride, masked;
} SlnDbgEdge;
int sln_debug_vae_edge(const SlnDbgEdge* desc, int n, int multi, int* variant, void* stream);
typedef struct SlnDbgLoss {
  const float* boxes; const float* boxes_pred; const int64_t* angles; const float* logits; float* angles_pred;
  const float* mu; const float* logvar; const float* eps; const float* dz; const float* d_logprob; const float* kl_weight;
  double* acc; float* losses; float* d_boxes_pred; float* d_logits; float* dmu; float* dlogvar;
  int kind, O, box_dim, n_angle, n_z, use_ae, ld_dbp, acc_prezeroed, from_logits, pad_;
} SlnDbgLoss;
int sln_debug_vae_loss(const SlnDbgLoss* desc, void* stream);
typedef struct SlnDbgBnEntry {
  const double* sums; const double* gsums; float* rmean; float* rvar; int64_t* nbt; float* dgamma; float* dbeta;
  int cstride, C, rows, pad_;
} SlnDbgBnEntry;
typedef struct SlnDbgTranspose { const float* src; float* dst; int rows, cols, dst_ld, pad_; } SlnDbgTranspose;
int sln_debug_vae_tables(int kind, const void* entries_host, int n, int width, float momentum, int independent, int rows_t, int rows_o,
                         void* stream);
typedef struct SlnDbgEmbed {
  const int64_t* objs; const int64_t* attrs; const int64_t* angles; const float* boxes;
  const float* obj_emb; const float* attr_emb; const float* angle_emb; const float* wb; const float* bb;
  const float* mu; const float* logvar; const float* eps; const float* z_in; float* z;
  float* x0; const float* dx0;
  float* d_obj_emb; float* d_attr_emb; float* d_angle_emb; float* d_wb; float* d_bb; float* dz;
  const void* idx; const float* src; void* dst; const float* src2; void* dst2;
  int64_t* st_objs; int64_t* st_attrs; int64_t* st_angles; float* st_boxes; int* attrs32; int* deg; int* err;
  void* zero_ptr; int64_t zero_bytes;
  int kind, O, n_obj, n_attr, n_box, n_angle, box_dim, n_z, use_ae, z_in_x0, rows_obj, rows_attr, rows_angle, ld, col0, n, table_rows,
      T, n2, pad_;
} SlnDbgEmbed;
int sln_debug_vae_embed(const SlnDbgEmbed* desc, int n, int multi, int* variant, void* stream);
typedef struct SlnDbgOpt {
  float* params; const float* grads; float* m; float* v; const float* total_loss; const SlnDbgEmbed* pro;
  int64_t n, step;
  uint64_t seed, offset;
  float lr, beta1, beta2, eps;
  int kind, calls;
  int64_t out_step; uint64_t out_offset; float out_bc1, out_bc2; int out_skip, pad_;
} SlnDbgOpt;
int sln_debug_vae_opt(SlnDbgOpt* desc, void* stream);
int sln_debug_vae_sizes(int* out, int max);
int64_t sln_debug_vae_leaf_launches(const SlnVae* h);
int64_t sln_debug_vae_half_launches(const SlnVae* h);


int sln_project_faces(const float* vertices, const int32_t* faces, const float* K, const float* R, const float* t, int B, int V, int F,
                      float orig_size, float eps, float* faces_xyz, void* stream);
int sln_project_faces_backward(const float* vertices, const int32_t* faces, const float* K, const float* R, const float* t, int B, int V,
                               int F, float orig_size, float eps, const float* grad_faces_xyz, float* grad_vertices, void* stream);
int64_t sln_raster_workspace_bytes(int B, int F);
int sln_raster_forward(const float* faces, int B, int F, int image_size, float near, float far, void* workspace,
                       int32_t* face_index, float* weight, float* depth, void* stream);
int sln_raster_forward_dual(const float* faces, int B, int F, int image_size, float near_a, float near_b, float far,
                            void* workspace, int32_t* fi_a, float* w_a, float* d_a, int32_t* fi_b, float* w_b,
                            float* d_b, void* stream);
int sln_raster_texture_sample(const float* faces, const float* textures, const int32_t* face_index, const float* weight,
                              const float* depth, int B, int F, int image_size, int texture_size, float eps, float* rgb,
                              void* stream);
int sln_raster_backward_depth(const float* faces, const int32_t* face_index, const float* weight, const float* depth,
                              const float* grad_depth, int B, int F, int image_size, float* grad_faces, void* stream);
int sln_raster_backward_rgb(const float* faces, const int32_t* face_index, const float* rgb, const float* grad_rgb, int B,
                            int F, int image_size, int channels, float eps, float* grad_faces, void* stream);
int sln_raster_texture_sample_chw(const float* faces, const float* textures, const int32_t* face_index, const float* weight,
                                  const float* depth, int B, int F, int F_tex, int image_size, int texture_size, float eps, float scale,
                                  float* rgb_chw, void* stream);
int sln_raster_backward_rgb_multi(const float* faces, const int32_t* face_index, const float* const* rgb_chw,
                                  const float* const* grad_chw, int P, int B, int F, int image_size, float eps, void* mask_ws,
                                  float* grad_faces, void* stream);

int64_t sln_scene_workspace_bytes(int B, int F, int image_size);
int sln_scene_forward(const float* faces, const int32_t* face_class, int B, int F, int image_size, int num_classes,
                      const int32_t* class_channel, const int32_t* class_depth_channel, float near_depth, float near_rgb,
                      float far, float tex_eps, void* workspace, float* final_out, void* stream);
int sln_scene_forward_live(const float* faces, const int32_t* face_class, int B, int F, int image_size, int num_classes,
                           const int32_t* class_channel, const int32_t* class_depth_channel, float near_depth, float near_rgb,
                           float far, float tex_eps, void* workspace, float* final_out, unsigned char* live,
                           unsigned char* null_mask , void* stream);
int sln_scene_live_channels(void* workspace, int B, int F, int image_size, int num_classes, const int32_t* class_channel,
                            const int32_t* class_depth_channel, unsigned char* live, void* stream);
int sln_scene_backward(const float* faces, const int32_t* face_class, int B, int F, int image_size, int num_classes,
                       const int32_t* class_channel, const int32_t* class_depth_channel, float pix_eps, void* workspace,
                       const float* grad_final, float* grad_faces, void* stream);


typedef struct {
  int n, n_vis, Vm, Vs, F, reserved;
  const int32_t* vis; const float* model_v; const float* msize; const float* mcenter; const float* shell_v;
  const int32_t* faces; const int32_t* obj_face_ptr;
  float ext[3];
  float K[9], R[9], t[3];
  float orig_size, proj_eps, cull_eps;
} SlnPlacement;
int sln_place_forward(const SlnPlacement* P , const float* boxes, const float* angles, const float* size_target,
                      float* faces_out, float* sizes, float* size_loss, void* stream);
int sln_place_backward(const SlnPlacement* P, const float* boxes, const float* angles, const float* size_target, const float* grad_faces,
// ... 230 lines not shown
```

Baseline: 35560 graphs/s (scene-graph VAE fwd+loss+bwd+Adam).

## Fuse backward weight-grad GEMMs and leaf kernel into one mixed tail launch

Adds a mixed TN multi-GEMM plan that mixes gathered and non-gathered problems in one launch, with a per-item gather flag, and a combined vae_tail kernel. That kernel runs the weight-gradient GEMM tiles and then the leaf work: embedding scatter, BN param grads, and a new decoder-assembly backward. The aim is to cut kernel launches and the serialization between the backward tail stages of the VAE step. In exchange it brings larger metadata structures, a uniform LDS allocation at GEMM size for leaf blocks, and more planning complexity.

```diff
diff --git a/3d_sln_amd/_lib.py b/3d_sln_amd/_lib.py
--- a/3d_sln_amd/_lib.py
+++ b/3d_sln_amd/_lib.py
@@ -219,6 +219,7 @@
     "sln_set_deterministic": (C.c_int, [C.c_int]),
     "sln_get_deterministic": (C.c_int, []),
     "sln_debug_tn_plan": (C.c_int, [C.c_void_p, C.c_void_p, C.c_void_p, C.c_int, C.c_void_p, C.c_void_p, C.c_int]),
+    "sln_debug_tn_plan_mixed": (C.c_int, [C.c_void_p, C.c_void_p, C.c_void_p, C.c_void_p, C.c_int, C.c_void_p, C.c_void_p, C.c_int]),
     "sln_prof_read": (C.c_int, [C.c_void_p, C.c_void_p, C.c_void_p, C.c_int]),
     "sln_vae_tap": (C.c_int64, [C.c_void_p, C.c_int, C.c_int, c_f32p, C.c_void_p]),
     "sln_gconv_workspace_bytes": (C.c_int64, [C.c_int, C.c_int, C.c_int, C.c_int, C.c_int, C.c_int]),
@@ -233,6 +234,7 @@
     "sln_linear_wgrad": (C.c_int, [c_f32p, c_f32p, C.c_int, C.c_int, C.c_int, c_f32p, c_f32p, C.c_void_p]),
     "sln_debug_gemm_nt": (C.c_int, [C.POINTER(SlnDbgGemmNT), C.c_int, C.POINTER(C.c_int), C.c_void_p]),
     "sln_debug_gemm_tn": (C.c_int, [C.POINTER(SlnDbgGemmTN), C.c_int, C.c_int, C.c_void_p]),
+    "sln_debug_gemm_tn_mixed": (C.c_int, [C.POINTER(SlnDbgGemmTN), C.c_int, C.c_void_p]),
     "sln_debug_gemm_nt_route": (C.c_int, [C.POINTER(SlnDbgGemmNT), C.POINTER(SlnDbgNTRoute)]),
     "sln_debug_gemm_nt_half": (C.c_int, [C.POINTER(SlnDbgGemmNT), C.c_int, C.c_void_p]),
     "sln_debug_gemm_nt_half_takes": (C.c_int, [C.POINTER(SlnDbgGemmNT)]),
@@ -246,6 +248,7 @@
     "sln_debug_vae_sizes": (C.c_int, [C.POINTER(C.c_int), C.c_int]),
     "sln_debug_vae_leaf_launches": (C.c_int64, [C.c_void_p]),
     "sln_debug_vae_half_launches": (C.c_int64, [C.c_void_p]),
+    "sln_debug_vae_tail_launches": (C.c_int64, [C.c_void_p]),
     "sln_project_faces": (C.c_int, [c_f32p, C.c_void_p, c_f32p, c_f32p, c_f32p, C.c_int, C.c_int, C.c_int, C.c_float, C.c_float, c_f32p, C.c_void_p]),
     "sln_project_faces_backward": (C.c_int, [c_f32p, C.c_void_p, c_f32p, c_f32p, c_f32p, C.c_int, C.c_int, C.c_int, C.c_float, C.c_float, c_f32p,
                                              c_f32p, C.c_void_p]),
diff --git a/3d_sln_amd/csrc/gemm_bodies.h b/3d_sln_amd/csrc/gemm_bodies.h
--- a/3d_sln_amd/csrc/gemm_bodies.h
+++ b/3d_sln_amd/csrc/gemm_bodies.h
@@ -1343,6 +1343,13 @@
 }
 
 
+template <bool G_X2>
+__device__ __forceinline__ void gemm_tn_mixed_item(const GemmTNArgs* __restrict__ probs, const TnMultiItem it, char* smem) {
+  if (it.prob < 0) return;
+  if (it.xg) gemm_tn_body<64, 64, 2, 2, G_X2, true>(probs[it.prob], it.tile, it.chunk, smem);
+  else gemm_tn_body<64, 64, 2, 2, G_X2, false>(probs[it.prob], it.tile, it.chunk, smem);
+}
+
 inline bool tn_gathers(const GemmTNArgs& a) {
   bool g = false;
   for (int s = 0; s < a.X.nseg; ++s) g |= a.X.seg[s].which != 0;
diff --git a/3d_sln_amd/csrc/gemm_f32.hip b/3d_sln_amd/csrc/gemm_f32.hip
--- a/3d_sln_amd/csrc/gemm_f32.hip
+++ b/3d_sln_amd/csrc/gemm_f32.hip
@@ -143,6 +143,12 @@
   const TnMultiItem it = meta->item[blockIdx.x];
   if (it.prob < 0) return;
   gemm_tn_body<64, 64, 2, 2, G_X2, XG>(probs[it.prob], it.tile, it.chunk, smem);
+}
+
+template <bool G_X2>
+__global__ __launch_bounds__(256) void gemm_tn_mixed_kernel(const GemmTNArgs* __restrict__ probs, const TnMixedMeta* __restrict__ meta) {
+  extern __shared__ __attribute__((aligned(16))) char smem[];
+  gemm_tn_mixed_item<G_X2>(probs, meta->item[blockIdx.x], smem);
 }
 
 template <int BM, int BN, int WM, int WN, bool G_X2>
@@ -181,6 +187,7 @@
 }
 
 int sln_gemm_group_init();
+int sln_vae_tail_init();
 int sln_gemm_init() {
   static bool done = false;
   if (done) return 0;
@@ -214,7 +221,10 @@
                                        hipFuncAttributeMaxDynamicSharedMemorySize, 160 * 1024);
   SLN_SET_TNM(true, true) SLN_SET_TNM(true, false) SLN_SET_TNM(false, true) SLN_SET_TNM(false, false)
 #undef SLN_SET_TNM
+  if (!r) r = (int)hipFuncSetAttribute(reinterpret_cast<const void*>(&gemm_tn_mixed_kernel<true>), hipFuncAttributeMaxDynamicSharedMemorySize, 160 * 1024);
+  if (!r) r = (int)hipFuncSetAttribute(reinterpret_cast<const void*>(&gemm_tn_mixed_kernel<false>), hipFuncAttributeMaxDynamicSharedMemorySize, 160 * 1024);
   if (!r) r = sln_gemm_group_init();
+  if (!r) r = sln_vae_tail_init();
   done = r == 0;
   return r;
 }
@@ -310,8 +320,9 @@
   return launch_tn<64, 64, 2, 2, false>(a, st);
 }
 
-int sln_tn_multi_plan(GemmTNArgs* probs, int n, TnMultiMeta* meta, int* blocks, bool* x2, bool* xg, double* flops) {
-  if (n < 1 || n > SLN_TN_MULTI_MAX) return -1;
+static int tn_plan(GemmTNArgs* probs, int n, int max_probs, int max_items, bool mixed, int* nprob, int* nblocks, TnMultiItem* item,
+                   int* blocks, bool* x2, bool* xg, double* flops) {
+  if (n < 1 || n > max_probs) return -1;
   static const int target0 = std::getenv("SLN_TN_MULTI_ROWS") ? std::atoi(std::getenv("SLN_TN_MULTI_ROWS")) : 768;
   static const bool no_xcd = std::getenv("SLN_TN_NO_XCD") != nullptr;
   bool any_x2 = false, any_xg = false;
@@ -351,29 +362,39 @@
     }
     int mx = 0;
     for (int x = 0; x < 8; ++x) mx = per_xcd[x] > mx ? per_xcd[x] : mx;
-    if (8 * mx <= SLN_TN_MULTI_ITEMS) break;
-    if (target > (1L << 30)) return -1;
-  }
-  if (any_xg) {
+    if (8 * mx <= max_items) break;
+    if (mixed || target > (1L << 30)) return -1;
+  }
+  if (any_xg && !mixed) {
     const int* any = nullptr;
     for (int i = 0; i < n; ++i) { if (probs[i].X.idx_a) any = probs[i].X.idx_a; else if (probs[i].X.idx_b) any = probs[i].X.idx_b; }
     for (int i = 0; i < n; ++i) if (!probs[i].X.idx_a && !probs[i].X.idx_b) probs[i].X.idx_a = any;
   }
   int mx = 0;
   for (int x = 0; x < 8; ++x) mx = per_xcd[x] > mx ? per_xcd[x] : mx;
-  std::memset(meta, 0, sizeof(*meta));
-  meta->nprob = n; meta->nblocks = 8 * mx;
-  for (int b = 0; b < 8 * mx; ++b) meta->item[b].prob = -1;
+  *nprob = n; *nblocks = 8 * mx;
+  std::memset(item, 0, sizeof(TnMultiItem) * (size_t)(mixed ? 8 * mx : max_items));
+  for (int b = 0; b < 8 * mx; ++b) item[b].prob = -1;
   int fill[8] = {0, 0, 0, 0, 0, 0, 0, 0};
   for (size_t g = 0; g < groups.size(); ++g) {
     const int x = owner[g];
+    const int gathers = mixed && tn_gathers(probs[groups[g].prob]) ? 1 : 0;
     for (int t = 0; t < groups[g].tiles; ++t) {
-      TnMultiItem& it = meta->item[8 * (fill[x]++) + x];
-      it.prob = groups[g].prob; it.tile = t; it.chunk = groups[g].chunk;
+      TnMultiItem& it = item[8 * (fill[x]++) + x];
+      it.prob = groups[g].prob; it.tile = t; it.chunk = groups[g].chunk; it.xg = gathers;
     }
   }
   *blocks = 8 * mx; *x2 = any_x2; *xg = any_xg; *flops = work;
   return 0;
+}
+
+int sln_tn_multi_plan(GemmTNArgs* probs, int n, TnMultiMeta* meta, int* blocks, bool* x2, bool* xg, double* flops) {
+  return tn_plan(probs, n, SLN_TN_MULTI_MAX, SLN_TN_MULTI_ITEMS, false, &meta->nprob, &meta->nblocks, meta->item, blocks, x2, xg, flops);
+}
+
+int sln_tn_mixed_plan(GemmTNArgs* probs, int n, TnMixedMeta* meta, int* blocks, bool* x2, double* flops) {
+  bool xg = false;
+  return tn_plan(probs, n, SLN_TN_MIXED_MAX, SLN_TN_MIXED_ITEMS, true, &meta->nprob, &meta->nblocks, meta->item, blocks, x2, &xg, flops);
 }
 
 int sln_launch_gemm_tn_multi(const GemmTNArgs* dev_probs, const TnMultiMeta* dev_meta, int blocks, bool x2, bool xg, double flops,
@@ -390,6 +411,17 @@
   return 0;
 }
 
+int sln_launch_gemm_tn_mixed(const GemmTNArgs* dev_probs, const TnMixedMeta* dev_meta, int blocks, bool x2, double flops, hipStream_t st) {
+  if (blocks <= 0) return 0;
+  SlnProfScope prof(SLN_FAM_GEMM_TN, flops, st);
+  const size_t smem = tn_smem_bytes(64, 64);
+  if (smem > 48 * 1024) { int r = sln_gemm_init(); if (r) return r; }
+  if (x2) hipLaunchKernelGGL((gemm_tn_mixed_kernel<true>), dim3(blocks), dim3(256), smem, st, dev_probs, dev_meta);
+  else hipLaunchKernelGGL((gemm_tn_mixed_kernel<false>), dim3(blocks), dim3(256), smem, st, dev_probs, dev_meta);
+  SLN_CHECK_LAUNCH();
+  return 0;
+}
+
 extern "C" int sln_debug_tn_plan(const int* R, const int* Nout, const int* Kin, int n, int* rows_per_block, int* items, int max_items) {
   if (!R || !Nout || !Kin || !rows_per_block || !items || n < 1 || n > SLN_TN_MULTI_MAX) return -1;
   static thread_local GemmTNArgs probs[SLN_TN_MULTI_MAX];
@@ -407,6 +439,28 @@
   for (int b = 0; b < blocks; ++b) {
     const TnMultiItem& it = meta.item[b];
     items[3 * b] = it.prob < 0 ? -1 : probs[it.prob].lddw; items[3 * b + 1] = it.tile; items[3 * b + 2] = it.chunk;
+  }
+  return blocks;
+}
+
+extern "C" int sln_debug_tn_plan_mixed(const int* R, const int* Nout, const int* Kin, const int* gathers, int n, int* rows_per_block,
+                                       int* items, int max_items) {
+  if (!R || !Nout || !Kin || !gathers || !rows_per_block || !items || n < 1 || n > SLN_TN_MIXED_MAX) return -1;
+  std::vector<GemmTNArgs> probs((size_t)n);
+  std::vector<TnMixedMeta> meta(1);
+  std::memset(probs.data(), 0, sizeof(GemmTNArgs) * (size_t)n);
+  for (int i = 0; i < n; ++i) {
+    probs[i].R = R[i]; probs[i].Nout = Nout[i]; probs[i].Kin = Kin[i];
+    probs[i].G.nseg = 1; probs[i].X.nseg = 1; probs[i].X.seg[0].which = gathers[i] ? 1 : 0; probs[i].lddw = i;
+  }
+  int blocks = 0; bool x2 = false; double flops = 0.0;
+  const int r = sln_tn_mixed_plan(probs.data(), n, meta.data(), &blocks, &x2, &flops);
+  if (r) return r;
+  if (blocks > max_items) return -2;
+  for (int i = 0; i < n; ++i) rows_per_block[probs[i].lddw] = probs[i].rows_per_block;
+  for (int b = 0; b < blocks; ++b) {
+    const TnMultiItem& it = meta[0].item[b];
+    items[4 * b] = it.prob < 0 ? -1 : probs[it.prob].lddw; items[4 * b + 1] = it.tile; items[4 * b + 2] = it.chunk; items[4 * b + 3] = it.xg;
   }
   return blocks;
 }
@@ -427,19 +481,21 @@
 
 namespace {
 
-bool dbg_operand(const SlnDbgOperand& d, int rows, int cols, bool gather_ok, bool x2_ok, Operand& op) {
+bool dbg_operand(const SlnDbgOperand& d, int rows, int cols, bool gather_ok, bool x2_ok, Operand& op, bool ragged_ok = false) {
   std::memset(&op, 0, sizeof(op));
   if (d.nseg < 1 || d.nseg > 3 || rows <= 0) return false;
   int tot = 0;
   for (int s = 0; s < d.nseg; ++s) {
     const SlnDbgSeg& g = d.seg[s];
     Seg& o = op.seg[s];
-    if (!g.x1 || g.len <= 0 || (g.len & 3)) return false;
-    if ((g.ld1 & 3) || (g.c1 & 3) || g.c1 < 0 || g.ld1 < g.c1 + g.len) return false;
+    const bool ragged = ragged_ok && s == d.nseg - 1 && (g.len & 3);
+    const int len4 = (g.len + 3) & ~3;
+    if (!g.x1 || g.len <= 0 || ((g.len & 3) && !ragged)) return false;
+    if ((g.ld1 & 3) || (g.c1 & 3) || g.c1 < 0 || g.ld1 < g.c1 + len4) return false;
     if (g.coef < SLN_COEF_IDENT || g.coef > SLN_COEF_BWD || g.which < 0 || g.which > 2) return false;
     if (g.which && (!gather_ok || !(g.which == 1 ? d.idx_a : d.idx_b))) return false;
     if (g.x2) {
-      if (!x2_ok || g.coef != SLN_COEF_BWD || (g.ld2 & 3) || (g.c2 & 3) || g.c2 < 0 || g.ld2 < g.c2 + g.len) return false;
+      if (!x2_ok || g.coef != SLN_COEF_BWD || (g.ld2 & 3) || (g.c2 & 3) || g.c2 < 0 || g.ld2 < g.c2 + len4) return false;
     } else if (g.coef == SLN_COEF_BWD && g.bn.mode == SLN_BN_TRAIN) return false;
     if (g.coef == SLN_COEF_BWD && !x2_ok) return false;
     o.x1 = g.x1; o.x2 = g.x2; o.ld1 = g.ld1; o.ld2 = g.ld2; o.c1 = g.c1; o.c2 = g.c2; o.len = g.len; o.which = g.which; o.coef = g.coef;
@@ -467,11 +523,11 @@
   return true;
 }
 
-bool dbg_tn(const SlnDbgGemmTN& d, GemmTNArgs& a) {
+bool dbg_tn(const SlnDbgGemmTN& d, GemmTNArgs& a, bool ragged_ok = false) {
   std::memset(&a, 0, sizeof(a));
   if (d.R <= 0 || d.Nout <= 0 || d.Kin <= 0 || !d.dW || d.lddw < d.Kin) return false;
-  if (!dbg_operand(d.G, d.R, d.Nout, false, true, a.G)) return false;
-  if (!dbg_operand(d.X, d.R, d.Kin, true, false, a.X)) return false;
+  if (!dbg_operand(d.G, d.R, d.Nout, false, true, a.G, ragged_ok)) return false;
+  if (!dbg_operand(d.X, d.R, d.Kin, true, false, a.X, ragged_ok)) return false;
   a.dW = d.dW; a.db = d.db; a.lddw = d.lddw; a.R = d.R; a.Nout = d.Nout; a.Kin = d.Kin;
   a.rows_per_block = d.rows_per_block; a.sgd_step = d.sgd_step;
   return true;
@@ -544,3 +600,26 @@
   if (dmeta) (void)hipFree(dmeta);
   return r;
 }
+
+extern "C" int sln_debug_gemm_tn_mixed(const SlnDbgGemmTN* desc, int n, void* stream) {
+  if (!desc || n < 1 || n > SLN_TN_MIXED_MAX) return SLN_E_BADARG;
+  std::vector<GemmTNArgs> probs((size_t)n);
+  for (int i = 0; i < n; ++i) if (!dbg_tn(desc[i], probs[(size_t)i], true)) return SLN_E_BADARG;
+  hipStream_t st = (hipStream_t)stream;
+  if (sln_capturing(st)) return SLN_E_CAPTURE;
+  std::vector<TnMixedMeta> meta(1);
+  int blocks = 0; bool x2 = false; double flops = 0.0;
+  if (sln_tn_mixed_plan(probs.data(), n, meta.data(), &blocks, &x2, &flops)) return SLN_E_BADARG;
+  GemmTNArgs* dprobs = nullptr; TnMixedMeta* dmeta = nullptr;
+  const size_t pbytes = sizeof(GemmTNArgs) * (size_t)n, mbytes = offsetof(TnMixedMeta, item) + sizeof(TnMultiItem) * (size_t)blocks;
+  int r = (int)hipMalloc((void**)&dprobs, pbytes);
+  if (!r) r = (int)hipMalloc((void**)&dmeta, sizeof(TnMixedMeta));
+  if (!r) r = (int)hipMemcpy(dprobs, probs.data(), pbytes, hipMemcpyHostToDevice);
+  if (!r) r = (int)hipMemcpy(dmeta, meta.data(), mbytes, hipMemcpyHostToDevice);
+  if (!r) r = sln_launch_gemm_tn_mixed(dprobs, dmeta, blocks, x2, flops, st);
+  const int rs = (int)hipStreamSynchronize(st);
+  if (!r) r = rs;
+  if (dprobs) (void)hipFree(dprobs);
+  if (dmeta) (void)hipFree(dmeta);
+  return r;
+}
diff --git a/3d_sln_amd/csrc/sln_debug.h b/3d_sln_amd/csrc/sln_debug.h
--- a/3d_sln_amd/csrc/sln_debug.h
+++ b/3d_sln_amd/csrc/sln_debug.h
@@ -4,4 +4,5 @@
 
 bool sln_dbg_bn(const SlnDbgBn& d, int coef, BnView& v);
 long sln_vae_engine_leaf_launches(const SlnVae* h);
+long sln_vae_engine_tail_launches(const SlnVae* h);
 long sln_vae_engine_half_launches(const SlnVae* h);
diff --git a/3d_sln_amd/csrc/sln_gemm.h b/3d_sln_amd/csrc/sln_gemm.h
--- a/3d_sln_amd/csrc/sln_gemm.h
+++ b/3d_sln_amd/csrc/sln_gemm.h
@@ -37,9 +37,13 @@
 int sln_launch_gemm_nt_half(const GemmNTArgs& a, int terms, hipStream_t st);
 int sln_launch_gemm_group(const GemmNTArgs* nt, const int* epi, int n_nt, hipStream_t st);
 enum { SLN_TN_MULTI_MAX = 64, SLN_TN_MULTI_ITEMS = 4096 };
-struct TnMultiItem { int prob, tile, chunk, pad_; };
+struct TnMultiItem { int prob, tile, chunk, xg; };
 struct TnMultiMeta { int nprob, nblocks; TnMultiItem item[SLN_TN_MULTI_ITEMS]; };
+enum { SLN_TN_MIXED_MAX = 128, SLN_TN_MIXED_ITEMS = 16384 };
+struct TnMixedMeta { int nprob, nblocks; TnMultiItem item[SLN_TN_MIXED_ITEMS]; };
 int sln_tn_multi_plan(GemmTNArgs* probs, int n, TnMultiMeta* meta, int* blocks, bool* x2, bool* xg, double* flops);
 int sln_launch_gemm_tn_multi(const GemmTNArgs* dev_probs, const TnMultiMeta* dev_meta, int blocks, bool x2, bool xg, double flops,
                              hipStream_t st);
+int sln_tn_mixed_plan(GemmTNArgs* probs, int n, TnMixedMeta* meta, int* blocks, bool* x2, double* flops);
+int sln_launch_gemm_tn_mixed(const GemmTNArgs* dev_probs, const TnMixedMeta* dev_meta, int blocks, bool x2, double flops, hipStream_t st);
 int sln_gemm_init();
diff --git a/3d_sln_amd/csrc/vae_debug.hip b/3d_sln_amd/csrc/vae_debug.hip
--- a/3d_sln_amd/csrc/vae_debug.hip
+++ b/3d_sln_amd/csrc/vae_debug.hip
@@ -385,4 +385,5 @@
 }
 
 extern "C" int64_t sln_debug_vae_leaf_launches(const SlnVae* h) { return h ? (int64_t)sln_vae_engine_leaf_launches(h) : (int64_t)SLN_E_BADARG; }
+extern "C" int64_t sln_debug_vae_tail_launches(const SlnVae* h) { return h ? (int64_t)sln_vae_engine_tail_launches(h) : (int64_t)SLN_E_BADARG; }
 extern "C" int64_t sln_debug_vae_half_launches(const SlnVae* h) { return h ? (int64_t)sln_vae_engine_half_launches(h) : (int64_t)SLN_E_BADARG; }
diff --git a/3d_sln_amd/csrc/vae_engine.hip b/3d_sln_amd/csrc/vae_engine.hip
--- a/3d_sln_amd/csrc/vae_engine.hip
+++ b/3d_sln_amd/csrc/vae_engine.hip
@@ -99,6 +99,7 @@
   float *bnA1 = nullptr, *anA1 = nullptr, *boxes_pred = nullptr, *logits = nullptr, *angles_pred = nullptr;
   float *dbp = nullptr, *dlogits = nullptr, *g_bn = nullptr, *g_an = nullptr, *d_bx = nullptr, *d_ax = nullptr;
   float *dM = nullptr, *dG[3] = {nullptr, nullptr, nullptr};
+  float* dX0_dc = nullptr;
   float *dX0 = nullptr, *dz = nullptr, *dmu = nullptr, *dlv = nullptr;
   float *g_h2 = nullptr, *g_h1 = nullptr, *d_xb = nullptr, *d_xa = nullptr, *tmp_d = nullptr;
   float *g_h2b = nullptr, *g_h1b = nullptr, *tmp_db = nullptr;
@@ -140,7 +141,8 @@
   int stage_upload(void* dev0, const void* src0, size_t n0, void* dev1, const void* src1, size_t n1, hipStream_t st) {
     hipStreamCaptureStatus cs = hipStreamCaptureStatusNone;
     if (hipStreamIsCapturing(st, &cs) != hipSuccess || cs != hipStreamCaptureStatusNone) return SLN_E_CAPTURE;
-    const size_t cap0 = sizeof(GemmTNArgs) * (size_t)SLN_TN_MULTI_MAX, cap = cap0 + sizeof(TnMultiMeta);
+    const size_t cap0 = sizeof(GemmTNArgs) * (size_t)(tn_mixed_store ? SLN_TN_MIXED_MAX : SLN_TN_MULTI_MAX);
+    const size_t cap = cap0 + (tn_mixed_store ? sizeof(TnMixedMeta) : sizeof(TnMultiMeta));
     if (n0 > cap0 || n1 > cap - cap0) return SLN_E_BADARG;
     TnStage& sl = tn_stage[tn_stage_next];
     tn_stage_next = (tn_stage_next + 1) % TN_STAGE_SLOTS;
@@ -170,12 +172,70 @@
         TnGroup& g = tn_group(0, w, k);
         if (g.n > 0 && g.dirty) { int r = upload_group(g); if (r) return r; }
       }
+    if (tn_mixed_store && tn_mixed_store[0].n > 0 && tn_mixed_store[0].dirty) { int r = upload_mixed(tn_mixed_store[0]); if (r) return r; }
     tn_upload_pending = false;
     return 0;
   }
+  struct TnMixedGroup {
+    GemmTNArgs probs[SLN_TN_MIXED_MAX]; TnMixedMeta meta; int n = 0, blocks = 0; bool x2 = false; double flops = 0.0;
+    bool dirty = true; GemmTNArgs* dev_probs = nullptr; TnMixedMeta* dev_meta = nullptr;
+  };
+  TnMixedGroup* tn_mixed_store = nullptr;
+  bool tail_merge = true;
+  bool it_tail = false;
+  bool tail_dec = true;
+  bool it_dec_leaf = false;
+  bool tail_leaf = true;
+  long tail_launches = 0;
+  static size_t mixed_meta_bytes(const TnMixedMeta& m) { return offsetof(TnMixedMeta, item) + sizeof(TnMultiItem) * (size_t)m.nblocks; }
+  int upload_mixed(TnMixedGroup& g) {
+    hipError_t e = hipMemcpy(g.dev_probs, g.probs, sizeof(GemmTNArgs) * (size_t)g.n, hipMemcpyHostToDevice);
+    if (e == hipSuccess) e = hipMemcpy(g.dev_meta, &g.meta, mixed_meta_bytes(g.meta), hipMemcpyHostToDevice);
+    g.dirty = e != hipSuccess;
+    return (int)e;
+  }
+  enum { TN_MIXED_NO_FIT = 1 << 20 };
+  int flush_mixed(int set, const VaeLeaf* leaf, hipStream_t st) {
+    if (!tn_mixed_store || !tn_mixed_store[set].dev_probs) return TN_MIXED_NO_FIT;
+    TnMixedGroup& tmp = tn_mixed_store[2];
+    int n = 0;
+    for (const GemmTNArgs& t : deferred) {
+      if (t.R <= 0) continue;
+      if (n == SLN_TN_MIXED_MAX) return TN_MIXED_NO_FIT;
+      tmp.probs[n++] = t;
+    }
+    if (n == 0) return leaf ? TN_MIXED_NO_FIT : 0;
+    tmp.n = n;
+    if (sln_tn_mixed_plan(tmp.probs, n, &tmp.meta, &tmp.blocks, &tmp.x2, &tmp.flops) != 0) return TN_MIXED_NO_FIT;
+    TnMixedGroup& g = tn_mixed_store[set];
+    if (g.n != n || g.meta.nblocks != tmp.meta.nblocks || std::memcmp(g.probs, tmp.probs, sizeof(GemmTNArgs) * (size_t)n) != 0 ||
+        std::memcmp(&g.meta, &tmp.meta, mixed_meta_bytes(tmp.meta)) != 0) {
+      std::memcpy(g.probs, tmp.probs, sizeof(GemmTNArgs) * (size_t)n);
+      std::memcpy(&g.meta, &tmp.meta, mixed_meta_bytes(tmp.meta));
+      g.n = n; g.blocks = tmp.blocks; g.x2 = tmp.x2; g.flops = tmp.flops; g.dirty = true;
+    }
+    if (g.dirty) {
+      if (capturing) tn_upload_pending = true;
+      else {
+        const int r = stage_upload(g.dev_probs, g.probs, sizeof(GemmTNArgs) * (size_t)g.n, g.dev_meta, &g.meta, mixed_meta_bytes(g.meta), st);
+        if (r) return r;
+        g.dirty = false;
+      }
+    }
+    const int r = leaf ? sln_launch_vae_tail(g.dev_probs, g.dev_meta, g.blocks, g.x2, g.flops, *leaf, st)
+                       : sln_launch_gemm_tn_mixed(g.dev_probs, g.dev_meta, g.blocks, g.x2, g.flops, st);
+    if (r == 0) { ++tail_launches; if (leaf) ++leaf_launches; }
+    return r;
+  }
   hipStream_t tn_eager_stream = nullptr;
-  int flush_deferred(int which, hipStream_t st) {
+  int flush_deferred(int which, hipStream_t st, const VaeLeaf* leaf = nullptr) {
     if (rec) { rec_push(SK_TN_FLUSH); return 0; }
+    if (leaf && (deferred.empty() || !(which == 2 && it_tail && tail_leaf))) {
+      const int r = sln_launch_vae_leaf(*leaf, st);
+      if (r) { deferred.clear(); return r; }
+      ++leaf_launches;
+      leaf = nullptr;
+    }
     if (deferred.empty()) return 0;
     const int set = capturing ? 0 : 1;
     if (set == 1 && tn_eager_stream != st) {
@@ -185,6 +245,15 @@
         if (tn_eager_stream != nullptr && hipStreamIsCapturing(tn_eager_stream, &cs_old) == hipSuccess && cs_old == hipStreamCaptureStatusNone)
           (void)hipStreamSynchronize(tn_eager_stream);
         tn_eager_stream = st;
+      }
+    }
+    if (which == 2 && it_tail) {
+      int r = flush_mixed(set, leaf, st);
+      if (r != TN_MIXED_NO_FIT) { deferred.clear(); return r; }
+      if (leaf) {
+        r = sln_launch_vae_leaf(*leaf, st);
+        if (r) { deferred.clear(); return r; }
+        ++leaf_launches;
       }
     }
     static thread_local TnGroup tmp;
@@ -551,8 +620,15 @@
           tg.dev_probs = dp; tg.dev_meta = dm; tg.dirty = true; tg.n = 0;
         }
       }
+  if (tn_mixed_store)
+    for (int set = 0; set < 2; ++set) {
+      GemmTNArgs* dp = b.take<GemmTNArgs>(SLN_TN_MIXED_MAX);
+      TnMixedMeta* dm = b.take<TnMixedMeta>(1);
+      if (!b.dry) { TnMixedGroup& tg = tn_mixed_store[set]; tg.dev_probs = dp; tg.dev_meta = dm; tg.dirty = true; tg.n = 0; }
+    }
   dG[0] = b.take<float>(Tm * 3 * Dm); dG[1] = b.take<float>(Tm * 3 * Dm);
   dG[2] = (gconv_only || !leaf_merge || no_merge || n_attr_e == 0 || !cfg.decoder_cat) ? nullptr : b.take<float>(Tm * 3 * (size_t)Ddc);
+  dX0_dc = (!tail_merge || gconv_only || !leaf_merge || no_merge || n_attr_e == 0 || !cfg.decoder_cat) ? nullptr : b.take<float>(Om * (size_t)Ddc);
   dX0 = b.take<float>(Om * Dm); dz = b.take<float>(Om * E); dmu = b.take<float>(Om * E); dlv = b.take<float>(Om * E);
   g_h2 = b.take<float>(Om * W); g_h1 = b.take<float>(Om * H); d_xb = b.take<float>(Om * W); d_xa = b.take<float>(Om * W);
   tmp_d = b.take<float>(Om * W);
@@ -584,6 +660,13 @@
   for (auto& bi : bns) maxc = bi.C > maxc ? bi.C : maxc;
   v.bn_tab = bn_table_dev; v.bn_n = (int)bns.size(); v.bn_max_c = maxc; v.bn_independent = cfg.recurrent ? 0 : 1;
   v.bn_update = step_training ? 1 : 0; v.bn_momentum = kBnMomentum;
+  if (it_dec_leaf) {
+    DecAssembleBwd& db = v.dec;
+    db.objs = batch.objs; db.attrs = batch.attributes; db.dx0 = dX0_dc; db.O = O; db.n_obj = n_obj_e; db.n_attr = n_attr_e; db.n_z = E;
+    db.d_obj_emb = t.d_obj_emb_dc; db.d_attr_emb = t.d_attr_emb_dc; db.dz = nullptr; db.z_in_x0 = 1;
+    db.rows_obj = cfg.num_objs; db.rows_attr = cfg.num_attrs;
+    v.dec_ld = Ddc;
+  }
   return v;
 }
 
@@ -765,7 +848,7 @@
                           v.mode != SLN_BN_NONE ? bns[pv.bn[3]].gsums : nullptr, W, st));
     } else {
       BnView none = view(-1, 0, tr);
-      RET_IF(k_gather_bwd(dG[slot], 3 * W, W, g, O, nullptr, 0, nullptr, 0, none, 0, dX0, W, nullptr, 0, st));
+      RET_IF(k_gather_bwd(dG[slot], 3 * W, W, g, O, nullptr, 0, nullptr, 0, none, 0, it_dec_leaf ? dX0_dc : dX0, W, nullptr, 0, st));
       if (!it_leaf) RET_IF(k_embed_bwd(g.p, 0, dG[slot], 3 * W, W, T, W, cfg.num_preds, t.d_pred_emb_dc, st));
     }
   }
@@ -773,7 +856,7 @@
   db.objs = batch.objs; db.attrs = batch.attributes; db.dx0 = dX0; db.O = O; db.n_obj = n_obj_e; db.n_attr = n_attr_e; db.n_z = E;
   db.d_obj_emb = t.d_obj_emb_dc; db.d_attr_emb = t.d_attr_emb_dc; db.dz = dz; db.z_in_x0 = cfg.decoder_cat ? 1 : 0;
   db.rows_obj = cfg.num_objs; db.rows_attr = cfg.num_attrs;
-  RET_IF(k_dec_assemble_bwd(db, st));
+  if (!it_dec_leaf) RET_IF(k_dec_assemble_bwd(db, st));
   const int nb = (int)bns.size() - n_bn_enc;
   if (nb > 0 && !it_merge_bn && !rec) {
     int maxc = 0;
@@ -850,9 +933,8 @@
     }
   }
   if (it_leaf) {
-    RET_IF(sln_launch_vae_leaf(leaf_args(), st));
-    ++leaf_launches;
-    RET_IF(flush_deferred(it_one_flush ? 2 : 1, st));
+    const VaeLeaf lf = leaf_args();
+    RET_IF(flush_deferred(it_one_flush ? 2 : 1, st, &lf));
     return 0;
   }
   EncAssembleBwd eb; std::memset(&eb, 0, sizeof(eb));
@@ -886,7 +968,10 @@
     bulk_zeroed = true;
     it_merge_bn = !no_merge && (mode == TRAIN_BACKWARD || mode == TRAIN_FULL);
     it_one_flush = one_flush && !tn_per_layer && (mode == TRAIN_BACKWARD || mode == TRAIN_FULL);
+    it_tail = it_one_flush && tail_merge && tn_mixed_store != nullptr && !g_sln_deterministic && !cfg.recurrent && !rec;
+    it_dec_leaf = it_tail && tail_leaf && tail_dec && it_merge_bn && dG[2] != nullptr && dX0_dc != nullptr && T > 0;
     it_leaf = it_merge_bn && dG[2] != nullptr && T > 0 && sln_vae_leaf_fits(leaf_args()) != 0;
+    it_dec_leaf = it_dec_leaf && it_leaf;
     it_wt_prologue = it_prologue && leaf_merge && (mode == TRAIN_BACKWARD || mode == TRAIN_FULL);
     if (!it_prologue && draw_eps) r = sln_launch_randn(eps_buf, (long)O * E, scalars, st);
     in_iteration = true;
@@ -897,14 +982,15 @@
     if (!r && grad_guard && mode != TRAIN_FULL)
       r = (int)hipMemcpyAsync(grad_guard, losses + 3, sizeof(float), hipMemcpyDeviceToDevice, st);
     if (!r) r = decoder_backward(st);
-    if (!r) r = sln_launch_latent_bwd(mu, logvar, eps, dz, &scalars->kl_weight, O, E, cfg.use_ae, dmu, dlv, st);
+    if (!r) r = it_dec_leaf ? sln_launch_latent_bwd(mu, logvar, eps, dX0_dc + n_obj_e + n_attr_e, &scalars->kl_weight, O, E, cfg.use_ae, dmu, dlv, st, Ddc)
+                            : sln_launch_latent_bwd(mu, logvar, eps, dz, &scalars->kl_weight, O, E, cfg.use_ae, dmu, dlv, st);
   }
   if (mode != TRAIN_UPTO_DECODER) {
     bulk_zeroed = true;
     if (!r) r = encoder_backward(st);
   }
   bulk_zeroed = false;
-  it_prologue = it_fused_loss = it_merge_bn = it_zero_in_prologue = it_one_flush = it_leaf = it_wt_prologue = false;
+  it_prologue = it_fused_loss = it_merge_bn = it_zero_in_prologue = it_one_flush = it_tail = it_leaf = it_dec_leaf = it_wt_prologue = false;
   RET_IF(r);
   if (mode == TRAIN_FULL) {
     RET_IF(sln_launch_adam(t.flat_params, t.flat_grads, t.adam_m, t.adam_v, (long)t.n_flat, scalars, losses + 3, st));
@@ -914,6 +1000,7 @@
 }
 
 long sln_vae_engine_leaf_launches(const SlnVae* h) { return h->leaf_launches; }
+long sln_vae_engine_tail_launches(const SlnVae* h) { return h->tail_launches; }
 long sln_vae_engine_half_launches(const SlnVae* h) { return h->half_launches; }
 
 extern "C" {
@@ -953,7 +1040,15 @@
   h->leaf_merge = !is("SLN_LEAF_MERGE", '0');
   h->tn_slots = 3 * (2 * h->L + 8 > 16 ? 2 * h->L + 8 : 16);
   h->tn_groups_store = new (std::nothrow) SlnVae::TnGroup[2 * (size_t)h->tn_slots * 2];
-  return h->tn_groups_store ? 0 : SLN_E_BADARG;
+  if (!h->tn_groups_store) return SLN_E_BADARG;
+  h->tail_merge = !is("SLN_TN_MIXED", '0') && !h->no_merge && h->leaf_merge && h->one_flush && !h->tn_per_layer && !h->cfg.recurrent && !h->gconv_only;
+  h->tail_leaf = !is("SLN_TN_MIXED", '1');
+  h->tail_dec = !is("SLN_TN_MIXED", '2');
+  if (h->tail_merge) {
+    h->tn_mixed_store = new (std::nothrow) SlnVae::TnMixedGroup[3];
+    if (!h->tn_mixed_store) return SLN_E_BADARG;
+  }
+  return 0;
 }
 
 int sln_vae_create(const SlnVaeConfig* c, SlnVae** out) {
@@ -1009,6 +1104,7 @@
   if (!h) return;
   h->drop_graphs();
   delete[] h->tn_groups_store;
+  delete[] h->tn_mixed_store;
   for (auto& sl : h->tn_stage) {
     if (sl.done) { (void)hipEventSynchronize(sl.done); (void)hipEventDestroy(sl.done); }
     if (sl.host) (void)hipHostFree(sl.host);
diff --git a/3d_sln_amd/csrc/vae_kernels.h b/3d_sln_amd/csrc/vae_kernels.h
--- a/3d_sln_amd/csrc/vae_kernels.h
+++ b/3d_sln_amd/csrc/vae_kernels.h
@@ -98,7 +98,7 @@
 int sln_launch_loss(LossArgs a, hipStream_t st);
 int sln_launch_latent_bwd(const float* mu, const float* logvar, const float* eps, const float* dz,
                           const float* kl_weight, int O, int n_z, int use_ae, float* dmu, float* dlogvar,
-                          hipStream_t st);
+                          hipStream_t st, int ld_dz = 0);
 
 struct BnTableEntry {
   const double* sums; const double* gsums; int cstride; int C; int rows;
@@ -139,7 +139,12 @@
   const int64_t* attr_idx; const float* d_attr; int ld_attr, col0_attr, n_attr_dc, attr_table_rows; float* d_attr_dc;
   const BnTableEntry* bn_tab; int bn_n, bn_max_c, bn_independent;
   int bn_update; float bn_momentum;
+  DecAssembleBwd dec; int dec_ld;
 };
 int sln_vae_leaf_fits(const VaeLeaf& a);
 int sln_launch_vae_leaf(const VaeLeaf& a, hipStream_t st);
+struct GemmTNArgs; struct TnMixedMeta;
+int sln_launch_vae_tail(const GemmTNArgs* dev_probs, const TnMixedMeta* dev_meta, int blocks, bool x2, double flops, const VaeLeaf& a,
+                        hipStream_t st);
+int sln_vae_tail_init();
 int sln_launch_layout_heatmap(const float* boxes, long n_trials, int O, int cs, int clip, float* counts, hipStream_t st);
diff --git a/3d_sln_amd/csrc/vae_kernels.hip b/3d_sln_amd/csrc/vae_kernels.hip
--- a/3d_sln_amd/csrc/vae_kernels.hip
+++ b/3d_sln_amd/csrc/vae_kernels.hip
@@ -1,6 +1,7 @@
 #include <cstring>
 #include "vae_kernels.h"
 #include "sln_prof.h"
+#include "gemm_bodies.h"
 
 namespace {
 
@@ -689,10 +690,10 @@
 __global__ void latent_bwd_kernel(const float* __restrict__ mu, const float* __restrict__ lv,
                                   const float* __restrict__ eps, const float* __restrict__ dz,
                                   const float* __restrict__ klw, int O, int nz, int use_ae, float* __restrict__ dmu,
-                                  float* __restrict__ dlv) {
+                                  float* __restrict__ dlv, int ld_dz) {
   const long i = (long)blockIdx.x * blockDim.x + threadIdx.x;
   if (i >= (long)O * nz) return;
-  const float g = dz[i];
+  const float g = ld_dz == nz ? dz[i] : dz[(i / nz) * ld_dz + (i % nz)];
   if (use_ae) { dmu[i] = g; dlv[i] = 0.f; return; }
   const float w = klw[0] / (float)O;
   const float l = lv[i];
@@ -1243,11 +1244,12 @@
 }
 
 int sln_launch_latent_bwd(const float* mu, const float* logvar, const float* eps, const float* dz, const float* kl_weight,
-                          int O, int n_z, int use_ae, float* dmu, float* dlogvar, hipStream_t st) {
+                          int O, int n_z, int use_ae, float* dmu, float* dlogvar, hipStream_t st, int ld_dz) {
   const long n = (long)O * n_z;
   if (n <= 0) return 0;
+  if (ld_dz != 0 && ld_dz < n_z) return -1;
   hipLaunchKernelGGL(latent_bwd_kernel, dim3((unsigned)((n + 255) / 256)), dim3(256), 0, st, mu, logvar, eps, dz,
-                     kl_weight, O, n_z, use_ae, dmu, dlogvar);
+                     kl_weight, O, n_z, use_ae, dmu, dlogvar, ld_dz ? ld_dz : n_z);
   SLN_CHECK_LAUNCH();
   return 0;
 }
@@ -1312,15 +1314,14 @@
 
 struct LeafEmbedJob { const void* idx; const float* d; float* d_emb; int ld, col0, rows, n, table_rows, rpb; };
 struct LeafArgs {
-  AssembleBwdLds asmb;
+  AssembleBwdLds asmb, asmb_dc;
   EncAssembleBwd box; int box_gx;
   LeafEmbedJob pdc, pec, attr;
   const BnTableEntry* bn_tab; int bn_n, bn_per_entry, bn_gx, rows_t, rows_o; float mom;
 };
-__global__ __launch_bounds__(256) void vae_leaf_kernel(unsigned int b0, unsigned int b1, unsigned int b2, unsigned int b3, unsigned int b4,
-                                                       unsigned int b5, LeafArgs a) {
+__device__ __forceinline__ void vae_leaf_dispatch(const unsigned int b, unsigned int b0, unsigned int b1, unsigned int b2, unsigned int b3,
+                                                  unsigned int b4, unsigned int b5, unsigned int b6, const LeafArgs& a) {
   extern __shared__ float tab[];
-  const unsigned int b = blockIdx.x;
   if (b < b0) assemble_bwd_lds_body(a.asmb, (int)b);
   else if (b < b1) {
     const int q = (int)(b - b0);
@@ -1338,10 +1339,23 @@
   else if (b < b5) {
     const int q = (int)(b - b4);
     bn_param_grads_body(a.bn_tab, a.bn_n, a.bn_per_entry, (q % a.bn_gx) * 256 + (int)threadIdx.x, q / a.bn_gx);
-  } else {
+  } else if (b < b6) {
     const int q = (int)(b - b5);
     bn_running_update_body(a.bn_tab, a.bn_n, a.mom, a.bn_per_entry, a.rows_t, a.rows_o, (q % a.bn_gx) * 256 + (int)threadIdx.x, q / a.bn_gx);
-  }
+  } else assemble_bwd_lds_body(a.asmb_dc, (int)(b - b6));
+}
+__global__ __launch_bounds__(256) void vae_leaf_kernel(unsigned int b0, unsigned int b1, unsigned int b2, unsigned int b3, unsigned int b4,
+                                                       unsigned int b5, unsigned int b6, LeafArgs a) {
+  vae_leaf_dispatch(blockIdx.x, b0, b1, b2, b3, b4, b5, b6, a);
+}
+
+struct LeafRanges { unsigned int b0, b1, b2, b3, b4, b5, b6; };
+template <bool G_X2>
+__global__ __launch_bounds__(256) void vae_tail_kernel(const GemmTNArgs* __restrict__ probs, const TnMixedMeta* __restrict__ meta,
+                                                       const unsigned int nwg, const LeafRanges r, const LeafArgs a) {
+  extern __shared__ __attribute__((aligned(16))) char smem[];
+  if (blockIdx.x >= nwg) { vae_leaf_dispatch(blockIdx.x - nwg, r.b0, r.b1, r.b2, r.b3, r.b4, r.b5, r.b6, a); return; }
+  gemm_tn_mixed_item<G_X2>(probs, meta->item[blockIdx.x], smem);
 }
 
 int sln_vae_leaf_fits(const VaeLeaf& a) {
@@ -1354,12 +1368,16 @@
     return 0;
   if (a.n_attr_dc > 0 && (a.attr_table_rows <= 0 || (long)a.attr_table_rows * a.n_attr_dc > EMBED_LDS_MAX_FLOATS)) return 0;
   if (a.n_pdc <= 0 || a.n_pec <= 0 || e.n_box <= 0) return 0;
+  if (a.dec.dx0) {
+    const DecAssembleBwd& d = a.dec;
+    if (d.dz || d.O != e.O || d.n_obj <= 0 || !(d.rows_obj > 0 && (d.n_attr == 0 || d.rows_attr > 0)) || a.dec_ld < d.n_obj + d.n_attr) return 0;
+    if ((long)d.rows_obj * d.n_obj + (long)d.rows_attr * d.n_attr > ASSEMBLE_LDS_MAX_FLOATS) return 0;
+  }
   return 1;
 }
 
-int sln_launch_vae_leaf(const VaeLeaf& v, hipStream_t st) {
-  if (!sln_vae_leaf_fits(v)) return -1;
-  LeafArgs a; std::memset(&a, 0, sizeof(a));
+static unsigned int leaf_build(const VaeLeaf& v, LeafArgs& a, LeafRanges& rg, size_t& lds_out) {
+  std::memset(&a, 0, sizeof(a));
   const EncAssembleBwd& e = v.enc;
   AssembleBwdLds& l = a.asmb;
   l.dx0 = e.dx0; l.ld = e.n_obj + e.n_attr + e.n_box + e.n_angle; l.O = e.O;
@@ -1385,12 +1403,58 @@
   const unsigned int n_pred = (unsigned int)sln_cdiv(v.pred_rows, rpb);
   const unsigned int n_attr = v.n_attr_dc > 0 ? (unsigned int)sln_cdiv(e.O, rpb) : 0;
   const unsigned int b0 = n_asm, b1 = b0 + n_box, b2 = b1 + n_pred, b3 = b2 + n_pred, b4 = b3 + n_attr, b5 = b4 + n_bn;
-  const unsigned int tot = b5 + (v.bn_update ? n_bn : 0);
+  const unsigned int b6 = b5 + (v.bn_update ? n_bn : 0);
+  unsigned int n_dasm = 0;
+  if (v.dec.dx0) {
+    AssembleBwdLds& d = a.asmb_dc;
+    d.dx0 = v.dec.dx0; d.ld = v.dec_ld; d.O = v.dec.O;
+    int kd = 0;
+    d.seg[kd++] = EmbSeg{v.dec.objs, v.dec.d_obj_emb, v.dec.n_obj, v.dec.rows_obj, 0, 0};
+    if (v.dec.n_attr > 0) d.seg[kd++] = EmbSeg{v.dec.attrs, v.dec.d_attr_emb, v.dec.n_attr, v.dec.rows_attr, v.dec.n_obj, 0};
+    d.nseg = kd;
+    int offd = 0;
+    for (int s = 0; s < d.nseg; ++s) { d.seg[s].lds0 = offd; offd += d.seg[s].rows * d.seg[s].n; }
+    d.lds_floats = offd;
+    d.rows_per_block = d.O <= 8192 ? 16 : 64;
+    n_dasm = (unsigned int)sln_cdiv(d.O, d.rows_per_block);
+  }
+  const unsigned int tot = b6 + n_dasm;
   size_t lds = sizeof(float) * 7 * RL * CB;
   auto grow = [&lds](long floats) { if (sizeof(float) * (size_t)floats > lds) lds = sizeof(float) * (size_t)floats; };
   grow(l.lds_floats); grow((long)v.pred_table_rows * v.n_pdc); grow((long)v.pred_table_rows * v.n_pec);
   if (v.n_attr_dc > 0) grow((long)v.attr_table_rows * v.n_attr_dc);
-  hipLaunchKernelGGL(vae_leaf_kernel, dim3(tot), dim3(256), lds, st, b0, b1, b2, b3, b4, b5, a);
+  grow(a.asmb_dc.lds_floats);
+  rg = LeafRanges{b0, b1, b2, b3, b4, b5, b6};
+  lds_out = lds;
+  return tot;
+}
+
+int sln_launch_vae_leaf(const VaeLeaf& v, hipStream_t st) {
+  if (!sln_vae_leaf_fits(v)) return -1;
+  LeafArgs a; LeafRanges r; size_t lds = 0;
+  const unsigned int tot = leaf_build(v, a, r, lds);
+  hipLaunchKernelGGL(vae_leaf_kernel, dim3(tot), dim3(256), lds, st, r.b0, r.b1, r.b2, r.b3, r.b4, r.b5, r.b6, a);
+  SLN_CHECK_LAUNCH();
+  return 0;
+}
+
+int sln_vae_tail_init() {
+  int r = (int)hipFuncSetAttribute(reinterpret_cast<const void*>(&vae_tail_kernel<true>), hipFuncAttributeMaxDynamicSharedMemorySize, 160 * 1024);
+  if (!r) r = (int)hipFuncSetAttribute(reinterpret_cast<const void*>(&vae_tail_kernel<false>), hipFuncAttributeMaxDynamicSharedMemorySize, 160 * 1024);
+  return r;
+}
+
+int sln_launch_vae_tail(const GemmTNArgs* dev_probs, const TnMixedMeta* dev_meta, int blocks, bool x2, double flops, const VaeLeaf& v,
+                        hipStream_t st) {
+  if (blocks < 0 || !sln_vae_leaf_fits(v)) return -1;
+  LeafArgs a; LeafRanges r; size_t lds = 0;
+  const unsigned int tot = leaf_build(v, a, r, lds);
+  const size_t smem = tn_smem_bytes(64, 64);
+  if (lds > smem) return -1;
+  { const int e = sln_gemm_init(); if (e) return e; }
+  SlnProfScope prof(SLN_FAM_GEMM_TN, flops, st);
+  if (x2) hipLaunchKernelGGL((vae_tail_kernel<true>), dim3((unsigned int)blocks + tot), dim3(256), smem, st, dev_probs, dev_meta, (unsigned int)blocks, r, a);
+  else hipLaunchKernelGGL((vae_tail_kernel<false>), dim3((unsigned int)blocks + tot), dim3(256), smem, st, dev_probs, dev_meta, (unsigned int)blocks, r, a);
   SLN_CHECK_LAUNCH();
   return 0;
 }
diff --git a/include/sln_hip.h b/include/sln_hip.h
--- a/include/sln_hip.h
+++ b/include/sln_hip.h
@@ -135,6 +135,8 @@
 int sln_set_deterministic(int on);
 int sln_get_deterministic(void);
 int sln_debug_tn_plan(const int* R, const int* Nout, const int* Kin, int n, int* rows_per_block, int* items, int max_items);
+int sln_debug_tn_plan_mixed(const int* R, const int* Nout, const int* Kin, const int* gathers, int n, int* rows_per_block, int* items,
+                            int max_items);
 int sln_prof_read(double* ms_by_family, double* work_by_family, int64_t* launches_by_family, int n_families);
 
 int64_t sln_vae_tap(SlnVae* h, int layer, int what, float* dst, void* stream);
@@ -201,6 +203,7 @@
 typedef struct SlnDbgNTRoute { int body, multi, amode, threads; } SlnDbgNTRoute;
 int sln_debug_gemm_nt(const SlnDbgGemmNT* desc, int n, int* grouped, void* stream);
 int sln_debug_gemm_tn(const SlnDbgGemmTN* desc, int n, int multi, void* stream);
+int sln_debug_gemm_tn_mixed(const SlnDbgGemmTN* desc, int n, void* stream);
 int sln_debug_gemm_nt_route(const SlnDbgGemmNT* desc, SlnDbgNTRoute* out);
 int sln_debug_gemm_nt_half(const SlnDbgGemmNT* desc, int terms, void* stream);
 int sln_debug_gemm_nt_half_takes(const SlnDbgGemmNT* desc);
@@ -258,6 +261,7 @@
 int sln_debug_vae_opt(SlnDbgOpt* desc, void* stream);
 int sln_debug_vae_sizes(int* out, int max);
 int64_t sln_debug_vae_leaf_launches(const SlnVae* h);
+int64_t sln_debug_vae_tail_launches(const SlnVae* h);
 int64_t sln_debug_vae_half_launches(const SlnVae* h);
 
 
```

Result: faster. 36300 graphs/s (scene-graph VAE fwd+loss+bwd+Adam), median of 6 (+2.1%).
